# KatherLab/STAMP

Hardware: AMD Instinct MI355X
Metric: tiles/sec encoded (224x224, ViT-L/14) (higher is better)
Workload: dtype f16

## Files before the change

include/amdstamp.h:

```cpp
#ifndef AMDSTAMP_H
#define AMDSTAMP_H

#include <stddef.h>
#include <stdint.h>

#ifdef __cplusplus
extern "C" {
#endif

#define AMDS_VERSION_MAJOR 0
#define AMDS_VERSION_MINOR 2

typedef enum {
    AMDS_OK = 0,
    AMDS_ERR_INVALID = -1,
    AMDS_ERR_WORKSPACE = -2,
    AMDS_ERR_HIP = -3,
    AMDS_ERR_NODEVICE = -4,
    AMDS_ERR_RANGE = -5
} amds_status;

typedef enum { AMDS_F16 = 0, AMDS_BF16 = 1, AMDS_F32 = 2 } amds_dtype;

typedef enum {
    AMDS_EPI_BIAS = 0,
    AMDS_EPI_BIAS_GELU = 1,
    AMDS_EPI_BIAS_RELU = 2,
    AMDS_EPI_RESIDUAL = 3,
    AMDS_EPI_BIAS_F32 = 4,
    AMDS_EPI_SWIGLU = 5,
    AMDS_EPI_PATCH = 6,
    AMDS_EPI_BIAS_GELU_F32 = 7,
    AMDS_EPI_BIAS_RELU_F32 = 8
} amds_epilogue;


int amds_version(void);
const char* amds_last_error(void);
int amds_device_info(int device, char* name_host, int n, int* cu_count_host, size_t* hbm_bytes_host);

typedef struct amds_ctx amds_ctx;
amds_ctx* amds_create(int device);
void amds_destroy(amds_ctx* ctx);
int amds_ctx_device(const amds_ctx* ctx);

int amds_profile_enable(amds_ctx* ctx, int on);
int amds_profile_reset(amds_ctx* ctx);
int amds_profile_read(amds_ctx* ctx, int kind, double* total_ms_host, long* launches_host, double* total_work_host);


int amds_cast_pad(const float* src, int ld_src, void* dst, int ld_dst, int rows, int cols,
                  int dtype, void* stream);

int amds_layernorm(const float* x, long x_row_stride, const float* gamma, const float* beta,
                   void* y, long y_row_stride, int rows, int cols, float eps, int out_dtype,
                   void* stream);

int amds_gemm(const void* A, long lda, const void* W, long ldw, int M, int N, int K,
              int dtype, int epi, void* out, long ldo, const float* bias, const float* scale,
              const float* pos, int np, int T, int P, float acc_scale, void* stream);

int amds_quick_gelu_inplace(void* u, long ld, long rows, int cols, int dtype, void* stream);

int amds_gemm_rowstream(const void* A, long lda, const float* ln_gamma, const float* ln_beta, float ln_eps,
                        const void* W, long ldw, int M, int N, int K, int dtype, int epi, void* out, long ldo,
                        const float* bias, void* stream);

int amds_swin_mlp96(float* x, int M, const void* fc1_w, const float* fc1_b, const void* fc2_w, const float* fc2_b,
                    const float* ln_gamma, const float* ln_beta, float ln_eps, int dtype, void* stream);

int amds_swin_mlp192_pack(const void* fc1_w, const void* fc2_w, void* packed, int dtype, void* stream);
int amds_swin_mlp192(float* x, int M, const void* packed_w, const float* fc1_b, const float* fc2_b, const float* ln_gamma,
                     const float* ln_beta, float ln_eps, int dtype, void* stream);

int amds_gemm_ex(int cfg, const void* A, long lda, const void* W, long ldw, int M, int N, int K,
                 int dtype, int epi, void* out, long ldo, const float* bias, const float* scale,
                 const float* pos, int np, int T, int P, float acc_scale, void* stream);
long amds_gemm_persist_launches(void);

int amds_gemm_fp8(const void* A8, long lda, const void* W8, long ldw, int M, int N, int K, int epi, void* out, long ldo, const float* bias,
                  const float* colscale, const float* rowscale, void* stream);
int amds_quantize_rows_e4m3(const void* x, long ldx, void* q, long ldq, float* scale, int rows, int cols, int in_dtype, void* stream);
int amds_layernorm_quant_e4m3(const float* x, long ldx, const float* gamma, const float* beta, float eps, void* q, long ldq, float* scale,
                              float* rownorm, int rows, int cols, void* stream);
int amds_row_bound_scale(const float* rownorm, float c0, float c1, float* us, int rows, void* stream);
int amds_gemm_fp8_out8(const void* A8, long lda, const void* W8, long ldw, int M, int N, int K, int epi, void* out8, long ldo8,
                       const float* out_rowscale, const float* bias, const float* colscale, const float* rowscale, void* stream);

int amds_gemm_lnfold(const void* A, long lda, const void* W, long ldw, int M, int N, int K, int dtype, int epi, void* out,
                     long ldo, const float* bias, const float* scale, void* xh, float* rowpart, const float* rowstat,
                     const float* colsum, void* stream);

int amds_gemm_lnfold_planes(const void* A, long lda, const void* W, long ldw, int M, int N, int K, void* hi, void* lo, long ld,
                            const float* bias, const float* scale, float* rowpart, void* stream);
int amds_ln_stats_split(const float* x, long ldx, int M, int D, float eps, void* hi, void* lo, long ld, float* rowstat, void* stream);
int amds_planes_to_f32(const void* hi, const void* lo, long ld, long row_stride, float* out, long ldo, long rows, int D, void* stream);

int amds_ln_rowstat(const float* rowpart, int M, int NP, int D, float eps, float* rowstat, void* stream);
int amds_ln_rowstat_diag(const float* rowpart, int M, int NP, int D, float eps, float* rowstat, int* diag, int dtype, void* stream);
int amds_ln_stats_cast(const float* x, long ldx, int M, int D, float eps, void* xh, long ldxh, float* rowstat, int dtype, void* stream);

int amds_pack_swiglu_rows(const float* src, float* dst, int H, int cols, void* stream);

int amds_attention_vit(const void* qkv, void* out, int B, int T, int H, int dtype, void* stream);

int amds_attention_vit_hd(const void* qkv, void* out, int B, int T, int H, int head_dim, int dtype, void* stream);

int amds_attention(const void* qkv, void* out, int B, int T, int H, int dtype, void* stream);
int amds_attention_row(const void* q, long ldq, const void* qkv, void* out, long ldo, int B, int T, int H, int dtype, void* stream);
int amds_attention_row_fwd_train(const void* qkv, void* out, float* lse, int B, int T, int H, int qrow, int dtype, float p, uint64_t seed,
                                 uint32_t stream_id, void* stream);
int amds_attention_row_alibi_fwd_train(const void* qkv, const float* coords, const float* inv_running_mean, const float* bias_scale, void* out, void* u, void* osm,
                                       float* lse, int B, int T, int H, int qrow, int dtype, void* stream);
int amds_attention_row_alibi_bwd_train(const void* qkv, const void* osm, const void* u, const void* dout, const float* lse, const float* coords, const float* bias_scale,
                                       const float* inv_running_mean, void* dqkv, float* dbs, int B, int T, int H, int qrow, int dtype, void* stream);
int amds_attention_row_bwd_train(const void* qkv, const void* out, const void* dout, const float* lse, void* dqkv, int B, int T, int H, int qrow,
                                 int dtype, float p, uint64_t seed, uint32_t stream_id, void* stream);
int amds_set_mil_cls_tail(amds_ctx* ctx, int on);
int amds_get_mil_cls_tail(amds_ctx* ctx);

int amds_attention_alibi(const void* qkv, const float* coords, const float* head_scale, void* out, int B, int T, int H,
                         int dtype, void* stream);

int amds_attention_masked(const void* qkv, const uint8_t* pad, void* out, int B, int T, int H, int mask_heads, int dtype, void* stream);
int amds_attention_alibi_masked(const void* qkv, const float* coords, const float* head_scale, const uint8_t* pad, void* out,
                                int B, int T, int H, int dtype, void* stream);


typedef struct {
    int img;
    int patch;
    int dim;
    int depth;
    int heads;
    int hidden;
    int n_prefix;
    int mlp_kind;
    int layerscale;
    int dtype;
    float ln_eps;
} amds_vit_cfg;

typedef struct {
    const float* ln1_w; const float* ln1_b;
    const void*  qkv_w; const float* qkv_b;
    const void*  proj_w; const float* proj_b;
    const float* ls1;
    const float* ln2_w; const float* ln2_b;
    const void*  fc1_w; const float* fc1_b;
    const void*  fc2_w; const float* fc2_b;
    const float* ls2;
    const float* qkv_colsum;
    const float* fc1_colsum;
} amds_vit_block;

typedef struct {
    const float* q_w;    const float* q_b;
    const float* proj_w; const float* proj_b;
    const float* fc1_w;  const float* fc1_b;
    const float* fc2_w;  const float* fc2_b;
} amds_vit_exact_block;

typedef struct {
    const void* qkv_w8;  const float* qkv_cs;
    const void* proj_w8; const float* proj_cs; const float* proj_b;
    const void* fc1_w8;  const float* fc1_cs;
    float fc1_wnorm_max; float fc1_babs_max;
    const void* fc2_w8;  const float* fc2_cs;  const float* fc2_b;
} amds_vit_fp8_block;

typedef struct {
    const void*  patch_w;
    const float* patch_b;
    const float* prefix;
    const float* pos_patch;
    const amds_vit_block* blocks_host;
    const float* norm_w; const float* norm_b;
    int patch_lo_shift;
    const amds_vit_exact_block* exact_host;
    int exact_hidden;
    const amds_vit_fp8_block* fp8_host;
    const float* pre_norm_w;
    const float* pre_norm_b;
    const amds_vit_exact_block* cls_tail;
} amds_vit_weights;

typedef struct {
    const float* norm1_w; const float* norm1_b;
    const float* qkv_w;   const float* qkv_b;
    const float* proj_w;  const float* proj_b;
    const float* ls1;
    const float* norm2_w; const float* norm2_b;
    const float* fc1_w;   const float* fc1_b;
    const float* fc2_w;   const float* fc2_b;
    const float* ls2;
} amds_vit_host_block;
typedef struct {
    const float* patch_w;
    const float* patch_b;
    const float* cls_token;
    const float* reg_token;
    const float* pos_embed;
    const amds_vit_host_block* blocks;
    const float* norm_w; const float* norm_b;
    int hidden;
    int no_embed_class;
    double mean[3]; double std[3];
} amds_vit_host_weights;
#define AMDS_PACK_LNFOLD      1
#define AMDS_PACK_PATCH_SPLIT 2
#define AMDS_PACK_EXACT       4
#define AMDS_PACK_CLS_TAIL    8
size_t amds_vit_pack_bytes(const amds_vit_cfg* cfg_host, const amds_vit_host_weights* src_host, int flags);
int amds_vit_pack(const amds_vit_cfg* cfg_host, const amds_vit_host_weights* src_host, int flags, void* dev_image, size_t bytes,
                  amds_vit_weights* out_w_host, amds_vit_block* out_blocks_host, amds_vit_exact_block* out_exact_host, void* stream);
int amds_vit_pack_host(const amds_vit_cfg* cfg_host, const amds_vit_host_weights* src_host, int flags, void* image_host, size_t bytes,
                       const void* target_base, amds_vit_weights* out_w_host, amds_vit_block* out_blocks_host,
                       amds_vit_exact_block* out_exact_host);

size_t amds_vit_workspace_bytes(const amds_vit_cfg* cfg_host, int batch);

size_t amds_vit_workspace_diag_offset(const amds_vit_cfg* cfg_host, int batch);

int amds_vit_forward(const amds_vit_cfg* cfg_host, const amds_vit_weights* w_host,
                     const uint8_t* tiles, void* feats_f16, int B, int chunk,
                     void* ws, size_t ws_bytes, void* stream);

int amds_check_finite(const void* x, long n, int dtype, int* count_dev, int* count_host, void* stream);

int amds_vit_forward_tokens(const amds_vit_cfg* cfg_host, const amds_vit_weights* w_host,
                            const uint8_t* tiles, void* feats_f16, float* tokens_f32, int B, int chunk,
                            void* ws, size_t ws_bytes, void* stream);

int amds_vit_forward_overlapped(amds_ctx* ctx, const amds_vit_cfg* cfg_host, const amds_vit_weights* w_host, const uint8_t* tiles,
                                void* feats_f16, int B, int chunk, void* ws, size_t ws_bytes, void* stream);

int amds_attention_cls_f32(const float* q, long ldq, const void* qkv, float* out, long ldo, int B, int T, int H, int head_dim,
                           int dtype, void* stream);
int amds_vit_cls_gather(const float* x, float* xc, int B, int T, int D, void* stream);
int amds_vit_cls_scatter(const float* xc, float* x, void* xh, float* rowstat, int B, int T, int D, float eps, int dtype, void* stream);
int amds_mlp_act_f32(float* u, long ld, int rows, int hidden, int kind, void* stream);

int amds_tile_im2col_u8(const uint8_t* tiles, void* out, int B, int img, int patch, int kp,
                        int dtype, void* stream);
int amds_tile_im2col_u8_ex(const uint8_t* tiles, void* out, int B, int img, int patch, int kp,
                           int dtype, int lo_shift, void* stream);

int amds_tile_normalize_u8(const uint8_t* hwc, float* chw, int B, int H, int W,
                           const float mean_host[3], const float std_host[3], void* stream);

int amds_tile_edge_fraction_u8(const uint8_t* tiles, float* frac, uint8_t* edges, uint8_t* gray, int B, int S, int low, int high,
                               void* stream);

typedef struct {
    int img;
    int embed;
    int n_stages;
    int depths[4];
    int heads[4];
    int dtype;
    float ln_eps;
} amds_swin_cfg;

typedef struct {
    const float* ln1_w; const float* ln1_b;
    const void*  qkv_w; const float* qkv_b;
    const float* bias_lane;
    const void*  proj_w; const float* proj_b;
    const float* ln2_w; const float* ln2_b;
    const void*  fc1_w; const float* fc1_b;
    const void*  fc2_w; const float* fc2_b;
    const void*  mlp_pack;
} amds_swin_block;

typedef struct {
    const float* ln_w; const float* ln_b;
    const void*  red_w;
} amds_swin_merge;

typedef struct {
    const float* stem;
    const amds_swin_block* blocks_host;
    int n_blocks;
    amds_swin_merge merges[3];
    const float* norm_w; const float* norm_b;
    const uint64_t* mask_bits;
} amds_swin_weights;

size_t amds_swin_workspace_bytes(const amds_swin_cfg* cfg_host, int batch);

int amds_swin_forward(const amds_swin_cfg* cfg_host, const amds_swin_weights* w_host, const uint8_t* tiles,
                      void* feats_f16, float* feats_f32, int B, int chunk, void* ws, size_t ws_bytes, void* stream);

int amds_swin_stem(const uint8_t* tiles, float* x, const float* params, int B, int img, int embed, float eps, void* stream);

int amds_window_attention(const void* qkv, long ldq, void* out, long ldo, const float* bias_lane, const uint64_t* mask_bits,
                          int B, int grid, int dim, int heads, int shift, int dtype, void* stream);

int amds_swin_attn96(float* x, const void* qkv_w, const float* qkv_b, const void* proj_w, const float* proj_b,
                     const float* ln_gamma, const float* ln_beta, const float* bias_lane, const uint64_t* mask_bits, int B,
                     int grid, int shift, float ln_eps, int dtype, void* stream);

int amds_patch_merge_ln(const float* x, void* y, const float* gamma, const float* beta, int B, int grid, int dim, float eps,
                        int dtype, void* stream);

int amds_layernorm_meanpool(const float* x, void* out_f16, float* out_f32, const float* gamma, const float* beta, int B,
                            int L, int dim, float eps, void* stream);

int amds_macenko_normalize_u8(const uint8_t* tiles, uint8_t* out, float* fit_out, int B, int H, int W, float Io, float alpha, float beta, void* stream);

size_t amds_supertiles_to_tiles_workspace_bytes(int n, int S, int k, int t);
int amds_supertiles_to_tiles_u8(const uint8_t* rgba, uint8_t* tiles, int n, int S, int k, int t, const int* bounds, const int* coef,
                                int ksize, void* ws, size_t ws_bytes, void* stream);

size_t amds_tile_resize_crop_workspace_bytes(int n, int S, int t);
int amds_tile_resize_crop_u8(const uint8_t* tiles, uint8_t* out, int n, int S, int O, int t, const int* bounds, const int* coef, int ksize, void* ws,
                             size_t ws_bytes, void* stream);

int amds_compact_rows_u8(const uint8_t* src, long row_bytes, const float* score, float cutoff, uint8_t* dst, int capacity_rows,
                         int* count_dev, int* slot_out, int n, void* stream);
int amds_compact_shift_u8(const uint8_t* src, uint8_t* dst, long row_bytes, int m, int max_rows, int* count_dev, void* stream);
// ... 495 lines not shown
```

stamp_amd/_lib.py:

```python
from __future__ import annotations

import ctypes as C
import os
from pathlib import Path

LIB_PATH = Path(__file__).resolve().parent / "lib" / "libamdstamp.so"

F16, BF16, F32 = 0, 1, 2
ERR_RANGE = -5
(EPI_BIAS, EPI_BIAS_GELU, EPI_BIAS_RELU, EPI_RESIDUAL, EPI_BIAS_F32, EPI_SWIGLU, EPI_PATCH,
 EPI_BIAS_GELU_F32, EPI_BIAS_RELU_F32) = range(9)


class VitCfg(C.Structure):
    _fields_ = [("img", C.c_int), ("patch", C.c_int), ("dim", C.c_int), ("depth", C.c_int),
                ("heads", C.c_int), ("hidden", C.c_int), ("n_prefix", C.c_int), ("mlp_kind", C.c_int),
                ("layerscale", C.c_int), ("dtype", C.c_int), ("ln_eps", C.c_float)]


class VitBlock(C.Structure):
    _fields_ = [(n, C.c_void_p) for n in (
        "ln1_w", "ln1_b", "qkv_w", "qkv_b", "proj_w", "proj_b", "ls1",
        "ln2_w", "ln2_b", "fc1_w", "fc1_b", "fc2_w", "fc2_b", "ls2", "qkv_colsum", "fc1_colsum")]

# ... 127 lines not shown
class BarspoonGrads(C.Structure):
    _fields_ = [("proj_w", C.c_void_p), ("proj_b", C.c_void_p), ("enc_layers_host", C.POINTER(MilVitLayerGrads)), ("class_tokens", C.c_void_p),
                ("dec_layers_host", C.POINTER(BarspoonDecLayerGrads)), ("head_w_host", C.POINTER(C.c_void_p)), ("head_b_host", C.POINTER(C.c_void_p))]


class TiconBlock(C.Structure):
    _fields_ = [(n, C.c_void_p) for n in ("ln1_w", "ln1_b", "v_w", "v_b", "proj_w", "proj_b", "ln2_w", "ln2_b", "fc1_w", "fc1_b", "fc2_w", "fc2_b")]


class TiconWeights(C.Structure):
    _fields_ = [("in_dim", C.c_int), ("dim", C.c_int), ("hidden", C.c_int), ("depth", C.c_int)] + \
               [(n, C.c_void_p) for n in ("in_fc1_w", "in_fc1_b", "in_fc2_w", "in_fc2_b", "in_norm_w", "in_norm_b")] + \
               [("blocks_host", C.POINTER(TiconBlock)), ("norm_w", C.c_void_p), ("norm_b", C.c_void_p)]


class SwinCfg(C.Structure):
    _fields_ = [("img", C.c_int), ("embed", C.c_int), ("n_stages", C.c_int), ("depths", C.c_int * 4),
                ("heads", C.c_int * 4), ("dtype", C.c_int), ("ln_eps", C.c_float)]


class SwinBlock(C.Structure):
    _fields_ = [(n, C.c_void_p) for n in (
        "ln1_w", "ln1_b", "qkv_w", "qkv_b", "bias_lane", "proj_w", "proj_b",
        "ln2_w", "ln2_b", "fc1_w", "fc1_b", "fc2_w", "fc2_b", "mlp_pack")]


class SwinMerge(C.Structure):
    _fields_ = [(n, C.c_void_p) for n in ("ln_w", "ln_b", "red_w")]


class SwinWeights(C.Structure):
    _fields_ = [("stem", C.c_void_p), ("blocks_host", C.POINTER(SwinBlock)), ("n_blocks", C.c_int),
                ("merges", SwinMerge * 3), ("norm_w", C.c_void_p), ("norm_b", C.c_void_p), ("mask_bits", C.c_void_p)]


class GapWeights(C.Structure):
    _fields_ = [(n, C.c_void_p) for n in ("fc_w", "fc_b", "a_w", "a_b", "b_w", "b_b", "c_w", "c_b", "packed")]


_vp, _i, _l, _f, _sz = C.c_void_p, C.c_int, C.c_long, C.c_float, C.c_size_t
_u64, _u32 = C.c_uint64, C.c_uint32

class TiconSlideCfg(C.Structure):
    _fields_ = [(n, C.c_int) for n in ("in_dim", "dim", "heads", "hidden", "depth", "dtype")]


class TiconSlideBlock(C.Structure):
    _fields_ = [(n, C.c_void_p) for n in ("ln1_w", "ln1_b", "in_w", "in_b", "proj_w", "proj_b", "g1", "ln2_w", "ln2_b", "fc1_w", "fc1_b", "fc2_w", "fc2_b", "g2")]


class TiconSlideWeights(C.Structure):
    _fields_ = [(n, C.c_void_p) for n in ("in_fc1_w", "in_fc1_b", "in_fc2_w", "in_fc2_b", "in_norm_w", "in_norm_b", "slopes")] + \
               [("blocks_host", C.POINTER(TiconSlideBlock)), ("norm_w", C.c_void_p), ("norm_b", C.c_void_p)]


PROTOTYPES = {
    "amds_version": (_i, []),
    "amds_last_error": (C.c_char_p, []),
    "amds_device_info": (_i, [_i, C.c_char_p, _i, C.POINTER(_i), C.POINTER(_sz)]),
    "amds_create": (_vp, [_i]),
    "amds_destroy": (None, [_vp]),
    "amds_ctx_device": (_i, [_vp]),
    "amds_profile_enable": (_i, [_vp, _i]),
    "amds_profile_reset": (_i, [_vp]),
    "amds_profile_read": (_i, [_vp, _i, C.POINTER(C.c_double), C.POINTER(C.c_long), C.POINTER(C.c_double)]),
    "amds_cast_pad": (_i, [_vp, _i, _vp, _i, _i, _i, _i, _vp]),
    "amds_layernorm": (_i, [_vp, _l, _vp, _vp, _vp, _l, _i, _i, _f, _i, _vp]),
    "amds_gemm": (_i, [_vp, _l, _vp, _l, _i, _i, _i, _i, _i, _vp, _l, _vp, _vp, _vp, _i, _i, _i, _f, _vp]),
    "amds_gemm_ex": (_i, [_i, _vp, _l, _vp, _l, _i, _i, _i, _i, _i, _vp, _l, _vp, _vp, _vp, _i, _i, _i, _f, _vp]),
    "amds_gemm_persist_launches": (_l, []),
    "amds_gemm_fp8": (_i, [_vp, _l, _vp, _l, _i, _i, _i, _i, _vp, _l, _vp, _vp, _vp, _vp]),
    "amds_layernorm_quant_e4m3": (_i, [_vp, _l, _vp, _vp, _f, _vp, _l, _vp, _vp, _i, _i, _vp]),
    "amds_row_bound_scale": (_i, [_vp, _f, _f, _vp, _i, _vp]),
    "amds_gemm_fp8_out8": (_i, [_vp, _l, _vp, _l, _i, _i, _i, _i, _vp, _l, _vp, _vp, _vp, _vp, _vp]),
    "amds_quantize_rows_e4m3": (_i, [_vp, _l, _vp, _l, _vp, _i, _i, _i, _vp]),
    "amds_gemm_lnfold": (_i, [_vp, _l, _vp, _l, _i, _i, _i, _i, _i, _vp, _l, _vp, _vp, _vp, _vp, _vp, _vp, _vp]),
    "amds_ln_rowstat": (_i, [_vp, _i, _i, _i, _f, _vp, _vp]),
    "amds_ln_rowstat_diag": (_i, [_vp, _i, _i, _i, _f, _vp, _vp, _i, _vp]),
    "amds_vit_workspace_diag_offset": (_sz, [_vp, _i]),
    "amds_check_finite": (_i, [_vp, _l, _i, _vp, _vp, _vp]),
    "amds_export_words": (_i, [_vp, _vp, _l, _i, _vp]),
    "amds_ln_stats_cast": (_i, [_vp, _l, _i, _i, _f, _vp, _l, _vp, _i, _vp]),
    "amds_gemm_lnfold_planes": (_i, [_vp, _l, _vp, _l, _i, _i, _i, _vp, _vp, _l, _vp, _vp, _vp, _vp]),
    "amds_ln_stats_split": (_i, [_vp, _l, _i, _i, _f, _vp, _vp, _l, _vp, _vp]),
    "amds_planes_to_f32": (_i, [_vp, _vp, _l, _l, _vp, _l, _l, _i, _vp]),
    "amds_gemm_rowstream": (_i, [_vp, _l, _vp, _vp, _f, _vp, _l, _i, _i, _i, _i, _i, _vp, _l, _vp, _vp]),
    "amds_swin_mlp96": (_i, [_vp, _i, _vp, _vp, _vp, _vp, _vp, _vp, _f, _i, _vp]),
    "amds_swin_mlp192_pack": (_i, [_vp, _vp, _vp, _i, _vp]),
    "amds_swin_mlp192": (_i, [_vp, _i, _vp, _vp, _vp, _vp, _vp, _f, _i, _vp]),
    "amds_pack_swiglu_rows": (_i, [_vp, _vp, _i, _i, _vp]),
    "amds_attention_vit": (_i, [_vp, _vp, _i, _i, _i, _i, _vp]),
    "amds_attention_row": (_i, [_vp, _l, _vp, _vp, _l, _i, _i, _i, _i, _vp]),
    "amds_attention_row_fwd_train": (_i, [_vp, _vp, _vp, _i, _i, _i, _i, _i, _f, C.c_uint64, C.c_uint32, _vp]),
    "amds_attention_row_bwd_train": (_i, [_vp, _vp, _vp, _vp, _vp, _i, _i, _i, _i, _i, _f, C.c_uint64, C.c_uint32, _vp]),
    "amds_set_mil_cls_tail": (_i, [_vp, _i]),
    "amds_get_mil_cls_tail": (_i, [_vp]),
    "amds_attention": (_i, [_vp, _vp, _i, _i, _i, _i, _vp]),
    "amds_attention_vit_hd": (_i, [_vp, _vp, _i, _i, _i, _i, _i, _vp]),
    "amds_attention_alibi": (_i, [_vp, _vp, _vp, _vp, _i, _i, _i, _i, _vp]),
    "amds_vit_workspace_bytes": (_sz, [C.POINTER(VitCfg), _i]),
    "amds_vit_forward": (_i, [C.POINTER(VitCfg), C.POINTER(VitWeights), _vp, _vp, _i, _i, _vp, _sz, _vp]),
    "amds_vit_forward_overlapped": (_i, [_vp, C.POINTER(VitCfg), C.POINTER(VitWeights), _vp, _vp, _i, _i, _vp, _sz, _vp]),
    "amds_vit_forward_tokens": (_i, [C.POINTER(VitCfg), C.POINTER(VitWeights), _vp, _vp, _vp, _i, _i, _vp, _sz, _vp]),
    "amds_swin_workspace_bytes": (_sz, [C.POINTER(SwinCfg), _i]),
    "amds_swin_forward": (_i, [C.POINTER(SwinCfg), C.POINTER(SwinWeights), _vp, _vp, _vp, _i, _i, _vp, _sz, _vp]),
    "amds_swin_stem": (_i, [_vp, _vp, _vp, _i, _i, _i, _f, _vp]),
    "amds_window_attention": (_i, [_vp, _l, _vp, _l, _vp, _vp, _i, _i, _i, _i, _i, _i, _vp]),
    "amds_swin_attn96": (_i, [_vp, _vp, _vp, _vp, _vp, _vp, _vp, _vp, _vp, _i, _i, _i, _f, _i, _vp]),
    "amds_patch_merge_ln": (_i, [_vp, _vp, _vp, _vp, _i, _i, _i, _f, _i, _vp]),
    "amds_layernorm_meanpool": (_i, [_vp, _vp, _vp, _vp, _vp, _i, _i, _i, _f, _vp]),
    "amds_tile_edge_fraction_u8": (_i, [_vp, _vp, _vp, _vp, _i, _i, _i, _i, _vp]),
    "amds_tile_im2col_u8": (_i, [_vp, _vp, _i, _i, _i, _i, _i, _vp]),
    "amds_tile_im2col_u8_ex": (_i, [_vp, _vp, _i, _i, _i, _i, _i, _i, _vp]),
    "amds_vit_pack_bytes": (_sz, [_vp, _vp, _i]),
    "amds_vit_pack": (_i, [_vp, _vp, _i, _vp, _sz, _vp, _vp, _vp, _vp]),
    "amds_vit_pack_host": (_i, [_vp, _vp, _i, _vp, _sz, _vp, _vp, _vp, _vp]),
    "amds_compact_shift_u8": (_i, [_vp, _vp, _l, _i, _i, _vp, _vp]),
    "amds_compact_rows_u8": (_i, [_vp, _l, _vp, _f, _vp, _i, _vp, _vp, _i, _vp]),
    "amds_attention_cls_f32": (_i, [_vp, _l, _vp, _vp, _l, _i, _i, _i, _i, _i, _vp]),
    "amds_vit_cls_gather": (_i, [_vp, _vp, _i, _i, _i, _vp]),
    "amds_vit_cls_scatter": (_i, [_vp, _vp, _vp, _vp, _i, _i, _i, _f, _i, _vp]),
    "amds_mlp_act_f32": (_i, [_vp, _l, _i, _i, _i, _vp]),
    "amds_tile_normalize_u8": (_i, [_vp, _vp, _i, _i, _i, C.POINTER(_f), C.POINTER(_f), _vp]),
    "amds_macenko_normalize_u8": (_i, [_vp, _vp, _vp, _i, _i, _i, _f, _f, _f, _vp]),
    "amds_supertiles_to_tiles_workspace_bytes": (_sz, [_i, _i, _i, _i]),
    "amds_supertiles_to_tiles_u8": (_i, [_vp, _vp, _i, _i, _i, _i, _vp, _vp, _i, _vp, _sz, _vp]),
    "amds_gather_rows": (_i, [_vp, _l, _vp, _i, _vp, _l, _i, _i, _i, _i, _vp]),
    "amds_vary_precision": (_i, [_vp, _vp, _vp, _l, _i, _vp]),
    "amds_bag_batch_gather": (_i, [_vp, _l, _i, _vp, _vp, _vp, _l, _i, _vp, _i, _i, _i, _i, _u64, _u32, _vp]),
    "amds_bag_batch_shifts": (_i, [_vp, _i, _i, _i, _i, _u64, _u32, _vp]),
    "amds_mean_pool": (_i, [_vp, _vp, _i, _i, _i, _i, _vp]),
    "amds_linear_f32": (_i, [_vp, _vp, _vp, _vp, _i, _i, _i, _i, _vp]),
    "amds_mil_vit_workspace_bytes": (_sz, [_vp, _i, _i]),
    "amds_mil_vit_forward": (_i, [_vp, _vp, _vp, _i, _vp, _vp, _vp, _i, _i, _vp, _sz, _vp]),
    "amds_mil_vit_ragged_workspace_bytes": (_sz, [_vp, _i, _l, _i]),
    "amds_mil_vit_forward_ragged": (_i, [_vp, _vp, _vp, _i, _vp, _vp, _vp, _i, _l, _i, _vp, _sz, _vp]),
    "amds_mil_vit_ragged_max_shared_tiles": (_i, [_vp]),
    "amds_attention_varlen_workspace_bytes": (_sz, [_i, _l]),
    "amds_attention_varlen": (_i, [_vp, _vp, _vp, _i, _l, _i, _i, _i, _vp, _sz, _vp]),
    "amds_attention_varlen_rows": (_i, [_vp, _vp, _vp, _i, _l, _i, _i, _i, _vp, _sz, _vp]),
    "amds_attention_alibi_varlen": (_i, [_vp, _vp, _vp, _vp, _vp, _i, _l, _i, _i, _i, _vp, _sz, _vp]),
    "amds_attention_row_varlen": (_i, [_vp, _l, _vp, _vp, _vp, _l, _i, _l, _i, _i, _i, _vp, _sz, _vp]),
    "amds_barspoon_workspace_bytes": (_sz, [_vp, _i, _i]),
    "amds_barspoon_forward": (_i, [_vp, _vp, _vp, _i, _vp, _vp, _i, _i, _vp, _sz, _vp]),
    "amds_barspoon_ragged_workspace_bytes": (_sz, [_vp, _i, _l, _i]),
    "amds_barspoon_forward_ragged": (_i, [_vp, _vp, _vp, _i, _vp, _vp, _vp, _i, _l, _i, _vp, _sz, _vp]),
    "amds_barspoon_ragged_max_shared_tiles": (_i, [_vp]),
    "amds_barspoon_train_saved_bytes": (_sz, [_vp, _i, _i]),
    "amds_barspoon_train_workspace_bytes": (_sz, [_vp, _i, _i, _i]),
    "amds_barspoon_train_forward": (_i, [_vp, _vp, _vp, _i, _vp, _vp, _vp, _i, _i, _vp, _sz, _vp]),
    "amds_barspoon_train_backward": (_i, [_vp, _vp, _vp, _vp, _i, _i, _vp, _sz, _vp, _i, _vp, _sz, _vp]),
    "amds_cross_attention_fwd_train": (_i, [_vp, _vp, _vp, _vp, _i, _i, _i, _i, _i, _i, _f, _u64, _u32, _vp]),
    "amds_cross_attention_bwd_workspace_bytes": (_sz, [_i, _i, _i, _i]),
    "amds_cross_attention_bwd_train": (_i, [_vp, _vp, _vp, _vp, _vp, _vp, _vp, _l, _i, _i, _i, _i, _i, _i, _f, _u64, _u32, _vp, _sz, _vp]),
    "amds_ticon_tile_workspace_bytes": (_sz, [_vp, _i]),
    "amds_ticon_tile_forward": (_i, [_vp, _vp, _i, _vp, _i, _i, _vp, _sz, _vp]),
    "amds_attention_distbias": (_i, [_vp, _vp, _vp, _vp, _i, _i, _i, _i, _vp]),
    "amds_ticon_slide_workspace_bytes": (_sz, [_vp, _i, _i]),
    "amds_ticon_slide_forward": (_i, [_vp, _vp, _vp, _i, _vp, _vp, _i, _i, _i, _vp, _sz, _vp]),
    "amds_tile_resize_crop_workspace_bytes": (_sz, [_i, _i, _i]),
    "amds_tile_resize_crop_u8": (_i, [_vp, _vp, _i, _i, _i, _i, _vp, _vp, _i, _vp, _sz, _vp]),
    "amds_proj_head_l2norm_workspace_bytes": (_sz, [_i, _i, _i]),
    "amds_proj_head_l2norm": (_i, [_vp, _i, _vp, _vp, _vp, _vp, _vp, _i, _i, _i, _vp, _sz, _vp]),
    "amds_quick_gelu_inplace": (_i, [_vp, _l, _l, _i, _i, _vp]),
    "amds_transmil_workspace_bytes": (_sz, [_vp, _i, _i]),
    "amds_transmil_train_saved_bytes": (_sz, [_vp, _i, _i]),
    "amds_transmil_train_workspace_bytes": (_sz, [_vp, _i, _i]),
    "amds_transmil_train_forward": (_i, [_vp, _vp, _vp, _i, _f, C.c_uint64, _vp, _i, _i, _vp, _sz, _vp]),
    "amds_transmil_train_backward": (_i, [_vp, _vp, _vp, _f, C.c_uint64, _i, _i, _vp, _sz, _vp, _vp, _vp, _sz, _vp]),
    "amds_nystrom_attn_saved_bytes": (_sz, [_i, _i, _i]),
    "amds_nystrom_attn_workspace_bytes": (_sz, [_i, _i, _i]),
    "amds_nystrom_attn_fwd": (_i, [_vp, _i, _vp, _vp, _i, _i, _f, C.c_uint64, C.c_uint32, _vp, _sz, _vp]),
    "amds_nystrom_attn_bwd": (_i, [_vp, _i, _vp, _vp, _vp, _i, _i, _f, C.c_uint64, C.c_uint32, _vp, _sz, _vp, _sz, _vp]),
    "amds_transmil_forward": (_i, [_vp, _vp, _vp, _i, _vp, _i, _i, _vp, _sz, _vp]),
    "amds_transmil_ragged_plan": (_i, [_vp, _i, _vp, _vp]),
    "amds_transmil_ragged_workspace_bytes": (_sz, [_vp, _i, _vp]),
    "amds_transmil_forward_ragged": (_i, [_vp, _vp, _vp, _i, _vp, _vp, _vp, _i, _vp, _sz, _vp]),
    "amds_mil_vit_train_saved_bytes": (_sz, [_vp, _i, _i]),
    "amds_mil_vit_train_workspace_bytes": (_sz, [_vp, _i, _i, _i]),
    "amds_mil_vit_train_forward": (_i, [_vp, _vp, _vp, _i, _vp, _vp, _vp, _i, _i, _vp, _sz, _vp]),
    "amds_mil_vit_train_backward": (_i, [_vp, _vp, _vp, _vp, _i, _i, _vp, _sz, _vp, _vp, _i, _vp, _sz, _vp]),
    "amds_mil_vit_gradcam_workspace_bytes": (_sz, [_vp, _i, _i]),
    "amds_mil_vit_gradcam": (_i, [_vp, _vp, _vp, _i, _i, _vp, _sz, _f, _vp, _vp, _sz, _vp]),
    "amds_softmax_over_tiles": (_i, [_vp, _vp, _i, _l, _vp]),
    "amds_scatter_grid": (_i, [_vp, _vp, _vp, _vp, _l, _i, _i, _i, _vp]),
    "amds_concordance_workspace_bytes": (_sz, [_l, _i]),
    "amds_concordance_counts": (_i, [_vp, _l, _l, _vp, _l, _vp, _l, _vp, _l, _l, _i, _vp, _vp, _sz, _vp]),
    "amds_bgemm_f32": (_i, [_vp, _i, _l, _l, _vp, _i, _l, _l, _i, _vp, _i, _l, _l, _i, _i, _i, _i, _i, _f, _f, _vp, _i, _vp]),
    "amds_bgemm_f32_dual": (_i, [_vp, _i, _l, _l, _vp, _i, _l, _l, _i, _vp, _vp, _i, _l, _l, _i, _i, _i, _i, _i, _f, _f, _f, _f, _vp]),
    "amds_softmax_rows": (_i, [_vp, _l, _i, _vp]),
    "amds_landmark_mean": (_i, [_vp, _l, _l, _i, _vp, _i, _i, _i, _i, _i, _f, _vp]),
    "amds_pinv_init": (_i, [_vp, _vp, _i, _i, _vp, _vp]),
    "amds_pinv_init_grouped": (_i, [_vp, _vp, _i, _i, _i, _vp, _vp]),
    "amds_dwconv_seq_row": (_i, [_vp, _l, _l, _i, _vp, _vp, _l, _l, _i, _i, _i, _i, _i, _i, _vp]),
    "amds_dwconv_seq": (_i, [_vp, _l, _l, _i, _vp, _vp, _l, _l, _i, _i, _i, _i, _i, _i, _vp]),
    "amds_ppeg": (_i, [_vp, _vp, _vp, _vp, _vp, _vp, _vp, _vp, _i, _i, _i, _i, _vp]),
    "amds_softmax_rows_bwd": (_i, [_vp, _vp, _l, _i, _vp]),
    "amds_landmark_mean_bwd": (_i, [_vp, _vp, _l, _l, _i, _i, _i, _i, _i, _i, _f, _i, _vp]),
    "amds_dwconv_seq_wgrad_workspace_bytes": (_sz, [_i, _i, _i]),
    "amds_dwconv_seq_wgrad": (_i, [_vp, _l, _l, _i, _vp, _l, _l, _i, _vp, _i, _i, _i, _i, _i, _vp, _sz, _vp]),
    "amds_ppeg_wgrad_workspace_bytes": (_sz, [_i, _i]),
    "amds_ppeg_wgrad": (_i, [_vp, _vp, _vp, _i, _i, _i, _i, _vp, _sz, _vp]),
# ... 119 lines not shown
```

stamp_amd/csrc/api.hip:

```cpp
#include "gemm_kernel.h"
#include <stdlib.h>
#include <atomic>
#include <mutex>

namespace amds {

static thread_local char g_err[512] = "";

void set_error(const char* fmt, ...) {
    va_list ap;
    va_start(ap, fmt);
    vsnprintf(g_err, sizeof(g_err), fmt, ap);
    va_end(ap);
}

int hip_fail(hipError_t e, const char* what) {
    set_error("HIP error %d (%s) in %s", (int)e, hipGetErrorString(e), what);
    return AMDS_ERR_HIP;
}

}
struct amds_ctx {
    int device = -1;
    int refs = 0;
// ... 289 lines not shown
        const char* e = getenv("AMDS_GEMM_CFG");
        bcfg = (e && *e && atoi(e) == 8) ? 8 : 12;
    }
    if (dtype == AMDS_F16) return gemm_dispatch<f16>(bcfg, epi, A, lda, W, ldw, M, N, K, ep, st);
    if (dtype == AMDS_BF16) return gemm_dispatch<bf16>(bcfg, epi, A, lda, W, ldw, M, N, K, ep, st);
    set_error("amds_gemm_batched: bad dtype %d", dtype);
    return AMDS_ERR_INVALID;
}

extern "C" int amds_wgrad_tn(const void* dy, long ld_dy, const void* x, long ld_x, long tokens, int N, int K, int split_k, int dtype, float* part,
                             void* stream) {
    AMDS_REQUIRE(dy && x && part, "amds_wgrad_tn: null pointer");
    AMDS_REQUIRE(tokens > 0 && N > 0 && K > 0 && split_k > 0 && split_k <= 65535, "amds_wgrad_tn: bad shape");
    AMDS_REQUIRE(N % 256 == 0 && K % 256 == 0, "amds_wgrad_tn: needs N %% 256 == 0 and K %% 256 == 0 (N=%d K=%d)", N, K);
    AMDS_REQUIRE(ld_dy % 8 == 0 && ld_x % 8 == 0 && ld_dy >= N && ld_x >= K, "amds_wgrad_tn: bad pitches");
    AMDS_REQUIRE(((uintptr_t)dy & 15) == 0 && ((uintptr_t)x & 15) == 0 && ((uintptr_t)part & 15) == 0, "amds_wgrad_tn: pointers must be 16-byte aligned");
    const long unit = 64L * split_k;
    const long chunk = (tokens + unit - 1) / unit * 64;
    AMDS_REQUIRE((chunk + 63) * std::max(ld_dy, ld_x) * 2 < (1L << 31), "amds_wgrad_tn: one split's operand span is beyond the 2 GB a buffer descriptor addresses (raise split_k)");
    EpiArgs ep;
    ep.out = part; ep.ldo = K; ep.bias = nullptr; ep.scale = nullptr; ep.pos = nullptr; ep.np = ep.T = ep.P = 0; ep.acc_scale = 1.0f;
    ep.bsA = chunk * ld_dy; ep.bsW = chunk * ld_x; ep.bsOut = (long)N * K; ep.nbatch = split_k; ep.ktot = tokens;
    hipStream_t st = (hipStream_t)stream;
    ProfScope prof(PROF_GEMM, 2.0 * tokens * (double)N * K, st);
    if (dtype == AMDS_F16) return gemm_dispatch<f16>(15, AMDS_EPI_BIAS_F32, dy, ld_dy, x, ld_x, N, K, (int)chunk, ep, st);
    if (dtype == AMDS_BF16) return gemm_dispatch<bf16>(15, AMDS_EPI_BIAS_F32, dy, ld_dy, x, ld_x, N, K, (int)chunk, ep, st);
    set_error("amds_wgrad_tn: bad dtype %d", dtype);
    return AMDS_ERR_INVALID;
}

extern "C" int amds_gemm_lnfold(const void* A, long lda, const void* W, long ldw, int M, int N, int K, int dtype, int epi, void* out,
                                long ldo, const float* bias, const float* scale, void* xh, float* rowpart, const float* rowstat,
                                const float* colsum, void* stream) {
    AMDS_REQUIRE(A && W && out, "amds_gemm_lnfold: null pointer");
    AMDS_REQUIRE(M >= 0 && N > 0 && K > 0 && K % 64 == 0 && N % 256 == 0, "amds_gemm_lnfold: needs K %% 64 == 0 and N %% 256 == 0 (M=%d N=%d K=%d)", M, N, K);
    AMDS_REQUIRE(lda % 8 == 0 && ldw % 8 == 0 && lda >= K && ldw >= K && ldo % 4 == 0, "amds_gemm_lnfold: bad pitches");
    AMDS_REQUIRE(((uintptr_t)A & 15) == 0 && ((uintptr_t)W & 15) == 0 && ((uintptr_t)out & 15) == 0 && ((uintptr_t)xh & 15) == 0,
                 "amds_gemm_lnfold: pointers must be 16-byte aligned");
    const bool producer = xh || rowpart, consumer = rowstat || colsum;
    AMDS_REQUIRE(producer != consumer, "amds_gemm_lnfold: either (xh, rowpart) [RESIDUAL] or (rowstat, colsum) [BIAS / BIAS_GELU / SWIGLU]");
    if (producer) {
        AMDS_REQUIRE(epi == AMDS_EPI_RESIDUAL && xh && rowpart, "amds_gemm_lnfold: the producer form is the RESIDUAL epilogue with xh AND rowpart");
    } else {
        AMDS_REQUIRE((epi == AMDS_EPI_BIAS || epi == AMDS_EPI_BIAS_GELU || epi == AMDS_EPI_SWIGLU) && rowstat && colsum && bias,
                     "amds_gemm_lnfold: the consumer form is BIAS / BIAS_GELU / SWIGLU with rowstat, colsum AND bias");
    }
    if (M == 0) return AMDS_OK;
    EpiArgs ep;
    ep.out = out; ep.ldo = ldo; ep.bias = bias; ep.scale = scale; ep.pos = nullptr; ep.np = ep.T = ep.P = 0; ep.acc_scale = 1.0f;
    ep.xh = xh; ep.rowpart = rowpart; ep.rowstat = rowstat; ep.colsum = colsum;
    hipStream_t st = (hipStream_t)stream;
    ProfScope prof(PROF_GEMM, 2.0 * M * (double)N * K, st);
    if (dtype == AMDS_F16) return gemm_dispatch<f16>(12, epi, A, lda, W, ldw, M, N, K, ep, st);
    if (dtype == AMDS_BF16) return gemm_dispatch<bf16>(12, epi, A, lda, W, ldw, M, N, K, ep, st);
    set_error("amds_gemm_lnfold: bad dtype %d", dtype);
    return AMDS_ERR_INVALID;
}

#ifdef AMDS_GEMM_TRACE
static const float* g_gemm_trace_buffer = nullptr;
extern "C" void amds_gemm_trace_buffer(void* p) { g_gemm_trace_buffer = reinterpret_cast<const float*>(p); }
#endif

extern "C" int amds_gemm_lnfold_planes(const void* A, long lda, const void* W, long ldw, int M, int N, int K, void* hi, void* lo, long ld,
                                       const float* bias, const float* scale, float* rowpart, void* stream) {
    AMDS_REQUIRE(A && W && hi && lo && rowpart, "amds_gemm_lnfold_planes: null pointer");
    AMDS_REQUIRE(M >= 0 && N > 0 && K > 0 && K % 64 == 0 && N % 256 == 0, "amds_gemm_lnfold_planes: needs K %% 64 == 0 and N %% 256 == 0 (M=%d N=%d K=%d)", M, N, K);
    AMDS_REQUIRE(lda % 8 == 0 && ldw % 8 == 0 && lda >= K && ldw >= K && ld % 4 == 0 && ld >= N, "amds_gemm_lnfold_planes: bad pitches");
    AMDS_REQUIRE(((uintptr_t)A & 15) == 0 && ((uintptr_t)W & 15) == 0 && ((uintptr_t)hi & 15) == 0 && ((uintptr_t)lo & 15) == 0,
                 "amds_gemm_lnfold_planes: pointers must be 16-byte aligned");
    AMDS_REQUIRE(hi != lo && A != hi && A != lo, "amds_gemm_lnfold_planes: the planes are updated in place and must not alias each other or A");
    if (M == 0) return AMDS_OK;
    EpiArgs ep;
    ep.out = hi; ep.ldo = ld; ep.bias = bias; ep.scale = scale; ep.pos = nullptr; ep.np = ep.T = ep.P = 0; ep.acc_scale = 1.0f;
    ep.xh = hi; ep.xl = lo; ep.rowpart = rowpart;
#ifdef AMDS_GEMM_TRACE
    ep.pos = g_gemm_trace_buffer;
#endif
    hipStream_t st = (hipStream_t)stream;
    ProfScope prof(PROF_GEMM, 2.0 * M * (double)N * K, st);
    return gemm_dispatch<f16>(12, AMDS_EPI_RESIDUAL, A, lda, W, ldw, M, N, K, ep, st);
}

extern "C" long amds_gemm_persist_launches(void) { return g_gemm_persist_launches.load(std::memory_order_relaxed); }

extern "C" int amds_gemm_ex(int cfg, const void* A, long lda, const void* W, long ldw, int M, int N, int K, int dtype,
                            int epi, void* out, long ldo, const float* bias, const float* scale, const float* pos,
                            int np, int T, int P, float acc_scale, void* stream) {
    return gemm_impl(cfg, A, lda, W, ldw, M, N, K, dtype, epi, out, ldo, bias, scale, pos, np, T, P, acc_scale, stream);
}
```

stamp_amd/csrc/elementwise.hip:

```cpp
#include "launch.h"

namespace amds {

template <typename TO, int MAXV>
__global__ void __launch_bounds__(256) layernorm_kernel(const float* __restrict__ x, long xs,
                                                        const float* __restrict__ gamma,
                                                        const float* __restrict__ beta, TO* __restrict__ y,
                                                        long ys, int rows, int cols, float eps) {
    const int lane = threadIdx.x & 63;
    const int row = blockIdx.x * 4 + (threadIdx.x >> 6);
    if (row >= rows) return;
    const float* xr = x + (long)row * xs;
    const int nv = cols >> 2;
    f32x4 v[MAXV];
    float s = 0.f;
#pragma unroll
    for (int i = 0; i < MAXV; ++i) {
        const int c = i * 64 + lane;
        if (c < nv) {
            v[i] = *reinterpret_cast<const f32x4*>(xr + c * 4);
            s += (v[i][0] + v[i][1]) + (v[i][2] + v[i][3]);
        }
    }
    const float mean = wave_sum(s) / (float)cols;
// ... 241 lines not shown

struct Norm3 { float mean[3], inv_std[3]; };
__global__ void __launch_bounds__(256) tile_normalize_kernel(const uint8_t* __restrict__ hwc, float* __restrict__ chw,
                                                             long npix_total, int hw, Norm3 nm) {
    long q = (long)blockIdx.x * blockDim.x + threadIdx.x;
    const long nq = npix_total >> 2;
    const long stride = (long)gridDim.x * blockDim.x;
    for (; q < nq; q += stride) {
        const long p = q << 2;
        const long b = p / hw;
        const int off = (int)(p - b * hw);
        const uint32_t* s = reinterpret_cast<const uint32_t*>(hwc + p * 3);
        const uint32_t w0 = s[0], w1 = s[1], w2 = s[2];
        uint8_t px[12];
#pragma unroll
        for (int k = 0; k < 4; ++k) { px[k] = (w0 >> (8 * k)) & 255; px[4 + k] = (w1 >> (8 * k)) & 255; px[8 + k] = (w2 >> (8 * k)) & 255; }
#pragma unroll
        for (int c = 0; c < 3; ++c) {
            f32x4 o;
#pragma unroll
            for (int k = 0; k < 4; ++k) o[k] = ((float)px[k * 3 + c] / 255.0f - nm.mean[c]) * nm.inv_std[c];
            *reinterpret_cast<f32x4*>(chw + (b * 3 + c) * hw + off) = o;
        }
    }
}

constexpr int IM2COL_KMAX = 4096;
template <typename TO>
__global__ void __launch_bounds__(256) im2col_u8_kernel(const uint8_t* __restrict__ tiles, TO* __restrict__ out,
                                                        int img, int p, int kp, float lo_scale) {
    extern __shared__ __attribute__((aligned(16))) uint8_t srow[];
    const int g = img / p;
    const int b = blockIdx.x / g, py = blockIdx.x - b * g;
    const int nbytes = p * img * 3;
    const uint8_t* src = tiles + ((long)b * img + (long)py * p) * img * 3;
    for (int i = threadIdx.x * 16; i < nbytes; i += 256 * 16)
        *reinterpret_cast<u32x4*>(srow + i) = *reinterpret_cast<const u32x4*>(src + i);
    __shared__ int koff[IM2COL_KMAX];
    const int pp = p * p, k_real = 3 * pp;
    for (int k = threadIdx.x; k < kp; k += 256) {
        const int c = k / pp, r = k - c * pp, i = r / p, j = r - i * p;
        koff[k] = k < k_real ? (i * img + j) * 3 + c : -1;
    }
    __syncthreads();
    const int ld = lo_scale != 0.f ? 2 * kp : kp;
    const int chunks = ld >> 3, half = kp >> 3;
    TO* orow = out + ((long)b * g * g + (long)py * g) * ld;
    typedef TO vec8 __attribute__((ext_vector_type(8)));
    for (int w = threadIdx.x; w < g * chunks; w += 256) {
        const int px = w / chunks, ch = w - px * chunks;
        const int ch0 = ch >= half ? ch - half : ch;
        const float sc = ch >= half ? lo_scale : 1.0f;
        const uint8_t* pbase = srow + px * p * 3;
        vec8 o;
#pragma unroll
        for (int e = 0; e < 8; ++e) {
            const int off = koff[ch0 * 8 + e];
            o[e] = (TO)(off >= 0 ? (float)pbase[off] * sc : 0.f);
        }
        *reinterpret_cast<vec8*>(orow + (long)px * ld + ch * 8) = o;
    }
}

__global__ void prefix_init_kernel(const float* __restrict__ prefix, float* __restrict__ x, int B, int T, int P, int dim) {
    const long total = (long)B * P * (dim >> 2);
    long i = (long)blockIdx.x * blockDim.x + threadIdx.x;
    const long stride = (long)gridDim.x * blockDim.x;
    const int dv = dim >> 2;
    for (; i < total; i += stride) {
        const long bt = i / dv;
        const int c = (int)(i - bt * dv);
        const long b = bt / P;
        const int t = (int)(bt - b * P);
        *reinterpret_cast<f32x4*>(x + ((b * T + t) * (long)dim) + c * 4) =
            *reinterpret_cast<const f32x4*>(prefix + (long)t * dim + c * 4);
    }
}

int prefix_init(const float* prefix, float* x, int B, int T, int P, int dim, hipStream_t st) {
    const long total = (long)B * P * (dim / 4);
    const int grid = (int)min((long)2048, (total + 255) / 256);
    hipLaunchKernelGGL(prefix_init_kernel, dim3(grid), dim3(256), 0, st, prefix, x, B, T, P, dim);
    AMDS_LAUNCH_CHECK("prefix_init_kernel");
    return AMDS_OK;
}

template <typename T>
__global__ void __launch_bounds__(256) quick_gelu_inplace_kernel(T* __restrict__ u, long ld, long rows, int cols) {
    typedef T vec8 __attribute__((ext_vector_type(8)));
    const int c8 = cols >> 3;
    const long total = rows * c8;
    long i = (long)blockIdx.x * blockDim.x + threadIdx.x;
    const long stride = (long)gridDim.x * blockDim.x;
    for (; i < total; i += stride) {
        const long r = i / c8;
        const int c = (int)(i - r * c8);
        vec8* p = reinterpret_cast<vec8*>(u + r * ld) + c;
        vec8 v = *p;
#pragma unroll
        for (int e = 0; e < 8; ++e) {
            const float x = (float)v[e];
            v[e] = (T)(x * __builtin_amdgcn_rcpf(1.0f + __expf(-1.702f * x)));
        }
        *p = v;
    }
}

}

using namespace amds;

extern "C" int amds_layernorm(const float* x, long x_row_stride, const float* gamma, const float* beta, void* y,
                              long y_row_stride, int rows, int cols, float eps, int out_dtype, void* stream) {
    AMDS_REQUIRE(x && gamma && beta && y, "amds_layernorm: null pointer");
    AMDS_REQUIRE(rows >= 0 && cols > 0 && cols % 4 == 0 && cols <= 8192, "amds_layernorm: cols=%d must be a multiple of 4 and <= 8192", cols);
    AMDS_REQUIRE(x_row_stride % 4 == 0 && y_row_stride % 4 == 0, "amds_layernorm: row strides must be multiples of 4");
    if (rows == 0) return AMDS_OK;
    hipStream_t st = (hipStream_t)stream;
    ProfScope prof(PROF_LN, (double)rows * cols * (4 + (out_dtype == AMDS_F32 ? 4 : 2)), st);
    int rc = AMDS_ERR_INVALID;
    if (!dispatch_16_32(out_dtype, [&](auto t) { rc = launch_ln<AMDS_TAG_T(t)>(x, x_row_stride, gamma, beta, y, y_row_stride, rows, cols, eps, st); }))
        set_error("amds_layernorm: bad out_dtype %d", out_dtype);
    return rc;
}

extern "C" int amds_cast_pad(const float* src, int ld_src, void* dst, int ld_dst, int rows, int cols, int dtype,
                             void* stream) {
    AMDS_REQUIRE(src && dst, "amds_cast_pad: null pointer");
    AMDS_REQUIRE(rows >= 0 && cols >= 0 && ld_dst >= cols && ld_src >= cols, "amds_cast_pad: bad shape");
    const long total = (long)rows * ld_dst;
    if (total == 0) return AMDS_OK;
    const int grid = (int)min((long)4096, (total + 255) / 256);
    hipStream_t st = (hipStream_t)stream;
    const bool ok = dispatch_16_32(dtype, [&](auto t) {
        typedef AMDS_TAG_T(t) T;
        hipLaunchKernelGGL((cast_pad_kernel<T>), dim3(grid), dim3(256), 0, st, src, ld_src, (T*)dst, ld_dst, total, cols);
    });
    if (!ok) { set_error("amds_cast_pad: bad dtype %d", dtype); return AMDS_ERR_INVALID; }
    AMDS_LAUNCH_CHECK("cast_pad_kernel");
    return AMDS_OK;
}

extern "C" int amds_pack_swiglu_rows(const float* src, float* dst, int H, int cols, void* stream) {
    AMDS_REQUIRE(src && dst && src != dst, "amds_pack_swiglu_rows: null/aliased pointer");
    AMDS_REQUIRE(H > 0 && H % 32 == 0 && cols > 0, "amds_pack_swiglu_rows: H=%d must be a positive multiple of 32", H);
    const long total = 2L * H * cols;
    const int grid = (int)min((long)4096, (total + 255) / 256);
    hipLaunchKernelGGL(pack_swiglu_rows_kernel, dim3(grid), dim3(256), 0, (hipStream_t)stream, src, dst, H, cols);
    AMDS_LAUNCH_CHECK("pack_swiglu_rows_kernel");
    return AMDS_OK;
}

extern "C" int amds_tile_normalize_u8(const uint8_t* hwc, float* chw, int B, int H, int W, const float mean_host[3],
                                      const float std_host[3], void* stream) {
    AMDS_REQUIRE(hwc && chw && mean_host && std_host, "amds_tile_normalize_u8: null pointer");
    AMDS_REQUIRE(B >= 0 && H > 0 && W > 0 && (H * W) % 4 == 0, "amds_tile_normalize_u8: H*W must be a multiple of 4");
    if (B == 0) return AMDS_OK;
    Norm3 nm;
    for (int c = 0; c < 3; ++c) {
        AMDS_REQUIRE(std_host[c] != 0.f, "amds_tile_normalize_u8: std[%d] == 0", c);
        nm.mean[c] = mean_host[c];
        nm.inv_std[c] = 1.0f / std_host[c];
    }
    const long npix = (long)B * H * W;
    const int grid = (int)min((long)4096, (npix / 4 + 255) / 256);
    hipLaunchKernelGGL(tile_normalize_kernel, dim3(grid), dim3(256), 0, (hipStream_t)stream, hwc, chw, npix, H * W, nm);
// ... 164 lines not shown
```

stamp_amd/csrc/gemm_4w16.h:

```cpp
#pragma once
#include <algorithm>
#include <type_traits>
#include "gemm_kernel.h"

namespace amds {

__device__ __forceinline__ f32x4 agpr_read(const f32x4& a) {
    f32x4 v;
    asm("v_accvgpr_read_b32 %0, %1" : "=v"(v[0]) : "a"(a[0]));
    asm("v_accvgpr_read_b32 %0, %1" : "=v"(v[1]) : "a"(a[1]));
    asm("v_accvgpr_read_b32 %0, %1" : "=v"(v[2]) : "a"(a[2]));
    asm("v_accvgpr_read_b32 %0, %1" : "=v"(v[3]) : "a"(a[3]));
    return v;
}

template <int N> struct NextTilePieces : std::integral_constant<int, N> {};
template <typename C> struct is_next_tile : std::false_type {};
template <int N> struct is_next_tile<NextTilePieces<N>> : std::true_type {};

template <typename T, int EPI, int P3 = 6, int P0 = 6, bool SPREAD = true, int PRL = 0, int PRS = 0, bool STREAM = false, bool PERSIST = false, bool TN = false>
__global__ void __launch_bounds__(256) __attribute__((amdgpu_waves_per_eu(1, 1)))
gemm_4w16_kernel(const T* __restrict__ A, long lda, const T* __restrict__ W, long ldw, int M, int N, int K,
                 EpiArgs ep, int tiles_m, int tiles_n) {
    typedef typename Act<T>::vec8 vec8;
    typedef typename Act<T>::vec4 vec4;
    constexpr int BM = 256, BN = 256, BK = 64, NT = 256;
    constexpr int ROWB = BK * 2;
    constexpr int A_BYTES = BM * ROWB, STAGE = (BM + BN) * ROWB;
    constexpr int FI = 8, FJ = 8;
    constexpr int GROUP_M = 8;

    extern __shared__ __attribute__((aligned(16))) char smem[];
#ifdef AMDS_GEMM_TRACE
    unsigned long long tr_t[4] = {0, 0, 0, 0}, tr_rt0 = __builtin_amdgcn_s_memrealtime();
    int tr_round = 0;
#define AMDS_GEMM_STAMP(k)                             \
    do {                                               \
        __builtin_amdgcn_sched_barrier(0);             \
        tr_t[k] = __builtin_amdgcn_s_memtime();        \
        __builtin_amdgcn_sched_barrier(0);             \
    } while (0)
#define AMDS_GEMM_TRACE_WRITE()                                                                                                            \
    do {                                                                                                                                   \
        if (ep.pos != nullptr && threadIdx.x == 0) {                                                                                       \
            unsigned long long* rec = reinterpret_cast<unsigned long long*>(const_cast<float*>(ep.pos)) +                                  \
                                      ((long)blockIdx.x * ((ntiles + (int)gridDim.x - 1) / (int)gridDim.x) + tr_round) * 8;                \
            rec[0] = tr_t[0]; rec[1] = tr_t[1]; rec[2] = tr_t[2]; rec[3] = tr_t[3];                                                        \
            rec[4] = (unsigned long long)__builtin_amdgcn_s_getreg(63492) | ((unsigned long long)__builtin_amdgcn_s_getreg(63508) << 32);  \
            rec[5] = (unsigned long long)ti;                                                                                               \
            rec[6] = tr_rt0; rec[7] = __builtin_amdgcn_s_memrealtime();                                                                    \
        }                                                                                                                                  \
        ++tr_round;                                                                                                                        \
    } while (0)
    AMDS_GEMM_STAMP(0);
#else
#define AMDS_GEMM_STAMP(k) do { } while (0)
#define AMDS_GEMM_TRACE_WRITE() do { } while (0)
#endif

    const int tid = threadIdx.x;
    const int lane = tid & 63;
    const int wave = __builtin_amdgcn_readfirstlane(tid >> 6);
    const int wm = wave >> 1, wn = wave & 1;
    const int l15 = lane & 15, kb = lane >> 4;
    const int l31 = lane & 31, hi = lane >> 5;

    static_assert(!PERSIST || (STREAM && !TN && P3 >= 0 && PRL + PRS == 0 &&
                               (EPI == AMDS_EPI_BIAS || EPI == AMDS_EPI_BIAS_GELU || EPI == AMDS_EPI_BIAS_RELU || EPI == AMDS_EPI_RESIDUAL)),
                  "gemm_4w16: the persistent form is a streamed epilogue on SCHED 0");
    int tm, tn;
    auto tile_of = [&](int bid, int nwg, int& tm_, int& tn_) {
        const int xcd = bid & 7, q = nwg >> 3, r = nwg & 7;
        const int t = (xcd < r ? xcd * (q + 1) : r * (q + 1) + (xcd - r) * q) + (bid >> 3);
        const int group = GROUP_M * tiles_n;
        const int g = t / group, first_m = g * GROUP_M;
        const int gm = min(tiles_m - first_m, GROUP_M);
        const int rr = t - g * group;
        tm_ = first_m + rr % gm;
        tn_ = rr / gm;
    };
    const int ntiles = PERSIST ? tiles_m * tiles_n : (int)gridDim.x;
    int ti = blockIdx.x;
    tile_of(ti, ntiles, tm, tn);
    int m0 = tm * BM, n0 = tn * BN;
    int par = 0;
    if (ep.nbatch > 1) {
        const long by = blockIdx.y;
        A += by * ep.bsA;
        W += by * ep.bsW;
        constexpr bool F32O = (EPI == AMDS_EPI_RESIDUAL || EPI == AMDS_EPI_BIAS_F32 || EPI == AMDS_EPI_BIAS_GELU_F32 || EPI == AMDS_EPI_BIAS_RELU_F32);
        if (F32O) ep.out = reinterpret_cast<float*>(ep.out) + by * ep.bsOut;
        else ep.out = reinterpret_cast<T*>(ep.out) + by * ep.bsOut;
    }

    int rows_a = min(BM, M - m0);
    const long tn_valid = TN ? (ep.ktot > 0 ? min((long)K, ep.ktot - (long)blockIdx.y * K) : (long)K) : 0;
    __amdgpu_buffer_rsrc_t rsrc_a = TN ? __builtin_amdgcn_make_buffer_rsrc(const_cast<T*>(A + m0), 0, tn_valid > 0 ? (int)(((tn_valid - 1) * lda + BM) * 2) : 0, 0x00020000)
                                             : __builtin_amdgcn_make_buffer_rsrc(const_cast<T*>(A + (long)m0 * lda), 0, (int)((((long)rows_a - 1) * lda + K) * 2), 0x00020000);
    __amdgpu_buffer_rsrc_t rsrc_w = TN ? __builtin_amdgcn_make_buffer_rsrc(const_cast<T*>(W + n0), 0, tn_valid > 0 ? (int)(((tn_valid - 1) * ldw + BN) * 2) : 0, 0x00020000)
                                             : __builtin_amdgcn_make_buffer_rsrc(const_cast<T*>(W + (long)n0 * ldw), 0, (int)(((long)(BN - 1) * ldw + K) * 2), 0x00020000);
    int voff[16];
#pragma unroll
    for (int it = 0; it < 16; ++it) {
        if constexpr (TN) {
            const int c = (it & 7) * NT + tid, row = c >> 5, pos = c & 31, g = (row & 3) | ((row >> 1) & 4);
            voff[it] = (int)(((long)row * (it < 8 ? lda : ldw) + (pos ^ (g << 1)) * 8) * 2);
        } else {
            const int c = (it & 7) * NT + tid, row = c >> 3, cp = c & 7, sc = cp ^ ((row >> 1) & 7);
            voff[it] = (int)(((long)row * (it < 8 ? lda : ldw) + sc * 8) * 2);
        }
    }
    auto issue_to = [&](const __amdgpu_buffer_rsrc_t& ra, const __amdgpu_buffer_rsrc_t& rw, char* st, int koff, int koff_w, int lo, int hi_) {
#pragma unroll
        for (int it = 0; it < 16; ++it)
            if (it >= lo && it < hi_) {
                if (it < 8) {
                    __builtin_amdgcn_raw_ptr_buffer_load_lds(ra, (lptr_t)(st + ((it & 7) * NT + wave * 64) * 16), 16, voff[it], koff, 0, 0);
                } else {
                    __builtin_amdgcn_raw_ptr_buffer_load_lds(rw, (lptr_t)(st + A_BYTES + ((it & 7) * NT + wave * 64) * 16), 16, voff[it], koff_w,
                                                             0, 0);
                }
            }
    };
    auto issue_pieces = [&](int kt, int lo, int hi_) {
        char* st = smem + ((PERSIST ? kt + par : kt) & 1) * STAGE;
        const int koff = TN ? kt * BK * (int)lda * 2 : kt * BK * 2;
        const int koff_w = TN ? kt * BK * (int)ldw * 2 : koff;
        issue_to(rsrc_a, rsrc_w, st, koff, koff_w, lo, hi_);
    };
    int m0n = m0, n0n = n0;
    bool has_next = false;
    __amdgpu_buffer_rsrc_t rsrc_an = rsrc_a, rsrc_wn = rsrc_w;
    auto issue_next = [&](int lo, int hi_) { issue_to(rsrc_an, rsrc_wn, smem + ((K / BK + par) & 1) * STAGE, 0, 0, lo, hi_); };

    const int swz = (l15 >> 1) & 7;
    const int a_off = (wm * 128 + l15) * ROWB;
    const int w_off = A_BYTES + (wn * 128 + l15) * ROWB;

    const bool lnf = ep.rowstat != nullptr;
    const bool bias_in_acc = ep.bias != nullptr && ep.acc_scale == 1.0f && !lnf;
    f32x4 acc[FI][FJ];
    {
        f32x4 b0[FJ];
#pragma unroll
        for (int j = 0; j < FJ; ++j) b0[j] = f32x4{0.f, 0.f, 0.f, 0.f};
        if (bias_in_acc) {
#pragma unroll
            for (int j = 0; j < FJ; ++j) b0[j] = *reinterpret_cast<const f32x4*>(ep.bias + n0 + wn * 128 + j * 16 + 4 * kb);
        }
        __builtin_amdgcn_sched_barrier(0);
        issue_pieces(0, 0, 16);
        if constexpr (P3 < 0) {
            if (K / BK > 1) issue_pieces(1, 0, 16);
        }
        __builtin_amdgcn_sched_barrier(0);
#pragma unroll
        for (int i = 0; i < FI; ++i)
#pragma unroll
            for (int j = 0; j < FJ; ++j) acc[i][j] = b0[j];
    }
#pragma unroll
    for (int i = 0; i < FI; ++i) {
        if (i == FI - 1)
            asm volatile("s_nop 7" : "+a"(acc[i][0]), "+a"(acc[i][1]), "+a"(acc[i][2]), "+a"(acc[i][3]), "+a"(acc[i][4]), "+a"(acc[i][5]),
                         "+a"(acc[i][6]), "+a"(acc[i][7]));
        else
            asm volatile("" : "+a"(acc[i][0]), "+a"(acc[i][1]), "+a"(acc[i][2]), "+a"(acc[i][3]), "+a"(acc[i][4]), "+a"(acc[i][5]),
                         "+a"(acc[i][6]), "+a"(acc[i][7]));
    }
    __builtin_amdgcn_sched_barrier(0);

    vec8 af[2][FI], wf[2][FJ];
    const int tn_g = (l15 >> 2) | ((kb & 1) << 2);
    const int tn_row = (kb * 8 + (l15 >> 2)) * 512 + (l15 & 1) * 8 + ((l15 >> 1) & 1) * 16;
    auto load_frags = [&](int kt, int ks, int s, int lo, int hi_) {
        const char* sb = smem + ((PERSIST ? kt + par : kt) & 1) * STAGE;
        if constexpr (TN) {
            const unsigned base = (unsigned)(size_t)(sb + tn_row + ks * 32 * 512);
#pragma unroll
            for (int q = 0; q < 16; ++q)
                if (q >= lo && q < hi_) {
                    const int qq = q & 7;
                    const unsigned pq = base + (q < 8 ? 0 : A_BYTES) + ((q < 8 ? wm : wn) * 16 + 2 * (qq ^ tn_g)) * 16;
                    u32x2 a0, a1;
                    asm volatile("ds_read_b64_tr_b16 %0, %1" : "=v"(a0) : "v"(pq) : "memory");
                    asm volatile("ds_read_b64_tr_b16 %0, %1 offset:2048" : "=v"(a1) : "v"(pq) : "memory");
                    const vec8 f = __builtin_bit_cast(vec8, u32x4{a0[0], a0[1], a1[0], a1[1]});
                    if (q < 8) af[s][qq] = f; else wf[s][qq] = f;
                }
        } else {
            const int co = ((ks * 4 + kb) ^ swz) << 4;
#pragma unroll
            for (int q = 0; q < 16; ++q)
                if (q >= lo && q < hi_) {
                    if (q < 8) af[s][q] = *reinterpret_cast<const vec8*>(sb + a_off + q * 16 * ROWB + co);
                    else wf[s][q - 8] = *reinterpret_cast<const vec8*>(sb + w_off + (q - 8) * 16 * ROWB + co);
                }
        }
    };
    auto unit = [&](int s, int ih, auto nr_c, int rkt, int rks, int rs, int rlo, auto nc_c, int ckt, int clo) {
        constexpr int NR = decltype(nr_c)::value, NC = decltype(nc_c)::value;
        constexpr bool NXT = is_next_tile<decltype(nc_c)>::value;
        constexpr int R_SPAN = SPREAD ? (NR >= 16 ? 16 : 32) : (NR > 0 ? NR : 1), C_LO = SPREAD ? (NR >= 16 ? 16 : 0) : NR,
                      C_SPAN = SPREAD ? 32 - C_LO : (NC > 0 ? NC : 1);
#pragma unroll
        for (int m = 0; m < 32; ++m) {
            Act<T>::mfma16_agpr(wf[s][m & 7], af[s][ih * 4 + (m >> 3)], acc[ih * 4 + (m >> 3)][m & 7]);
            if (NR > 0 && m < R_SPAN) {
                const int r0 = m * NR / R_SPAN, r1 = (m + 1) * NR / R_SPAN;
                if (r1 > r0) load_frags(rkt, rks, rs, rlo + r0, rlo + r1);
            }
            if (NC > 0 && m >= C_LO && m < C_LO + C_SPAN) {
                const int c0 = (m - C_LO) * NC / C_SPAN, c1 = (m - C_LO + 1) * NC / C_SPAN;
                if (c1 > c0) {
                    if constexpr (NXT) issue_next(clo + c0, clo + c1); else issue_pieces(ckt, clo + c0, clo + c1);
                }
            }
            __builtin_amdgcn_sched_barrier(0);
        }
    };
    typedef std::integral_constant<int, 0> I0;
    typedef std::integral_constant<int, 8> I8;
    typedef std::integral_constant<int, 16> I16;
// ... 119 lines not shown
                AMDS_BARRIER();
                unit(1, 1, I16{}, kt + 1, 0, 0, 0, I0{}, 0, 0);
            } else {
                unit(1, 0, I0{}, 0, 0, 0, 0, I0{}, 0, 0);
                unit(1, 1, I0{}, 0, 0, 0, 0, I0{}, 0, 0);
            }
        }
    };
    auto k_tile_last_prefetch = [&](int kt) {
        unit(0, 0, I8{}, kt, 1, 1, 0, NextTilePieces<8>{}, 0, 0);
        unit(0, 1, I8{}, kt, 1, 1, 8, NextTilePieces<8>{}, 0, 8);
        unit(1, 0, I0{}, 0, 0, 0, 0, I0{}, 0, 0);
        asm volatile("s_waitcnt lgkmcnt(0)" ::: "memory");
        __builtin_amdgcn_sched_barrier(0);
        __builtin_amdgcn_s_waitcnt(0x0F70);
        AMDS_BARRIER();
    };
next_tile:
    int kt = 0;
    for (; kt < nk - 2; ++kt) k_tile(kt, std::true_type{}, std::true_type{});
    if (nk >= 2) k_tile(kt++, std::true_type{}, std::false_type{});
    if constexpr (PERSIST) {
        has_next = ti + (int)gridDim.x < ntiles;
        int tmn, tnn;
        tile_of(has_next ? ti + (int)gridDim.x : ti, ntiles, tmn, tnn);
        m0n = tmn * BM;
        n0n = tnn * BN;
        const int rows_an = min(BM, M - m0n);
        rsrc_an = __builtin_amdgcn_make_buffer_rsrc(const_cast<T*>(A + (long)m0n * lda), 0, has_next ? (int)((((long)rows_an - 1) * lda + K) * 2) : 0, 0x00020000);
        rsrc_wn = __builtin_amdgcn_make_buffer_rsrc(const_cast<T*>(W + (long)n0n * ldw), 0, has_next ? (int)(((long)(BN - 1) * ldw + K) * 2) : 0, 0x00020000);
    }
    constexpr bool LNC = (EPI == AMDS_EPI_BIAS || EPI == AMDS_EPI_BIAS_GELU || EPI == AMDS_EPI_SWIGLU);
    f32x2 rs[LNC ? FI : 1];
    f32x4 cb[LNC ? FJ : 1], cs[LNC ? FJ : 1];
    auto load_lnc = [&]() {
        if constexpr (LNC) {
            if (lnf) {
#pragma unroll
                for (int i = 0; i < FI; ++i)
                    rs[i] = *reinterpret_cast<const f32x2*>(ep.rowstat + 2 * (long)min(m0 + wm * 128 + i * 16 + l15, M - 1));
#pragma unroll
                for (int j = 0; j < FJ; ++j) {
                    cb[j] = *reinterpret_cast<const f32x4*>(ep.bias + n0 + wn * 128 + j * 16 + 4 * kb);
                    cs[j] = *reinterpret_cast<const f32x4*>(ep.colsum + n0 + wn * 128 + j * 16 + 4 * kb);
                }
            }
        }
    };
    if constexpr (PERSIST) {
        k_tile_last_prefetch(kt);
        if constexpr (LNC) {
#pragma unroll
            for (int i = 0; i < FI; ++i) asm volatile("" : "=v"(rs[i]));
#pragma unroll
            for (int j = 0; j < FJ; ++j) asm volatile("" : "=v"(cb[j]), "=v"(cs[j]));
        }
        load_lnc();
        __builtin_amdgcn_sched_barrier(0);
        unit(1, 1, I0{}, 0, 0, 0, 0, I0{}, 0, 0);
    } else {
        load_lnc();
        k_tile(kt, std::false_type{}, std::false_type{});
    }
    AMDS_GEMM_STAMP(2);
    if constexpr (PRN > 0) {
        asm volatile("s_waitcnt vmcnt(0)" ::: "memory");
#pragma unroll
        for (int q = 0; q < (PRL > 0 ? PRL : 1); ++q) asm volatile("" ::"v"(pd[q]));
    }
    if constexpr (!PERSIST) AMDS_BARRIER();

#pragma unroll
    for (int i = 0; i < FI; ++i) {
        if (i == 0)
            asm volatile("s_nop 15\n\ts_nop 15" : "+a"(acc[i][0]), "+a"(acc[i][1]), "+a"(acc[i][2]), "+a"(acc[i][3]), "+a"(acc[i][4]),
                         "+a"(acc[i][5]), "+a"(acc[i][6]), "+a"(acc[i][7]));
        else
            asm volatile("" : "+a"(acc[i][0]), "+a"(acc[i][1]), "+a"(acc[i][2]), "+a"(acc[i][3]), "+a"(acc[i][4]), "+a"(acc[i][5]),
                         "+a"(acc[i][6]), "+a"(acc[i][7]));
    }
    __builtin_amdgcn_sched_barrier(0);

    constexpr bool F16OUT = (EPI == AMDS_EPI_BIAS || EPI == AMDS_EPI_BIAS_GELU || EPI == AMDS_EPI_BIAS_RELU);
    static_assert(epi_is_staged<EPI>() || EPI == AMDS_EPI_SWIGLU, "gemm_4w16: staged epilogues and SWIGLU");
    if constexpr (EPI == AMDS_EPI_SWIGLU) {
        const float as = ep.acc_scale;
#pragma unroll
        for (int i = 0; i < FI; ++i) {
            const int row = wm * 128 + i * 16 + l15;
#pragma unroll
            for (int q = 0; q < 2; ++q)
#pragma unroll
                for (int t = 0; t < 2; ++t) {
                    f32x4 gt = agpr_read(acc[i][4 * q + t]), vl = agpr_read(acc[i][4 * q + 2 + t]);
                    if (lnf) {
                        gt = gt * rs[i][0] + (cs[4 * q + t] * rs[i][1] + cb[4 * q + t]);
                        vl = vl * rs[i][0] + (cs[4 * q + 2 + t] * rs[i][1] + cb[4 * q + 2 + t]);
                    } else if (!bias_in_acc) {
                        const f32x4 bg = *reinterpret_cast<const f32x4*>(ep.bias + n0 + wn * 128 + (4 * q + t) * 16 + 4 * kb);
                        const f32x4 bv = *reinterpret_cast<const f32x4*>(ep.bias + n0 + wn * 128 + (4 * q + 2 + t) * 16 + 4 * kb);
                        gt = gt * as + bg;
                        vl = vl * as + bv;
                    }
                    f32x4 o;
                    {
                        const f32x2 o01 = silu_mul2(f32x2{gt[0], gt[1]}, f32x2{vl[0], vl[1]}), o23 = silu_mul2(f32x2{gt[2], gt[3]}, f32x2{vl[2], vl[3]});
                        o = f32x4{o01[0], o01[1], o23[0], o23[1]};
                    }
                    const int hcol = wn * 64 + q * 32 + t * 16 + 4 * kb;
                    const int chunk = hcol >> 3, half = ((hcol >> 2) & 1) * 8;
                    *reinterpret_cast<vec4*>(smem + row * 256 + ((chunk ^ (row & 15)) << 4) + half) = Act<T>::from_f32x4(o);
                }
        }
        __syncthreads();
        const int l15r = lane & 15, rsub = lane >> 4;
#pragma unroll 4
        for (int it = 0; it < 16; ++it) {
            const int row = wave * 64 + it * 4 + rsub;
            const u32x4 v = *reinterpret_cast<const u32x4*>(smem + row * 256 + l15r * 16);
            const int chunk = l15r ^ (row & 15);
            if (m0 + row < M)
                *reinterpret_cast<u32x4*>(reinterpret_cast<T*>(ep.out) + (long)(m0 + row) * ep.ldo + n0 / 2 + chunk * 8) = v;
        }
        return;
    }
    if constexpr (EPI == AMDS_EPI_RESIDUAL && STREAM) {
        static_assert(std::is_same<T, f16>::value && !TN && PRL + PRS == 0, "gemm_4w16: the streamed residual epilogue is the fp16 planes producer");
        __builtin_amdgcn_sched_barrier(0);
        __builtin_amdgcn_s_waitcnt(0x0F70);
        __builtin_amdgcn_sched_barrier(0);
        const int rows_o = min(BM, M - m0);
        int ldo2 = (int)ep.ldo * 2;
        if constexpr (PERSIST) asm volatile("" : "+s"(ldo2));
        const __amdgpu_buffer_rsrc_t rsrc_h = __builtin_amdgcn_make_buffer_rsrc(reinterpret_cast<T*>(ep.xh) + (long)m0 * ep.ldo + n0, 0,
                                                                                (int)((((long)rows_o - 1) * ep.ldo + BN) * 2), 0x00020000);
        const __amdgpu_buffer_rsrc_t rsrc_l = __builtin_amdgcn_make_buffer_rsrc(reinterpret_cast<T*>(ep.xl) + (long)m0 * ep.ldo + n0, 0,
                                                                                (int)((((long)rows_o - 1) * ep.ldo + BN) * 2), 0x00020000);
        char* slab = smem + (PERSIST ? ((nk - 1 + par) & 1) * STAGE : 0) + wave * 16384;
        float* part = reinterpret_cast<float*>(smem + 2 * STAGE);
        int wr_base = l15 * 512;
        int rd_base = hi * 512 + l31 * 16;
        if constexpr (PERSIST) asm volatile("" : "+v"(wr_base), "+v"(rd_base));
        int offp[8];
#pragma unroll
        for (int u = 0; u < 8; ++u) offp[u] = (wm * 128 + 2 * u + hi) * ldo2 + wn * 256 + ((l31 ^ (2 * u + hi)) << 3);
        const int np_part = N / 128;
        auto run = [&](auto has_scale_c) {
            constexpr bool HS = decltype(has_scale_c)::value;
            f32x4 sc[HS ? FJ : 1];
            if constexpr (HS) {
#pragma unroll
                for (int j = 0; j < FJ; ++j) sc[j] = *reinterpret_cast<const f32x4*>(ep.scale + n0 + wn * 128 + j * 16 + 4 * kb);
            }
            f32x4 b0n[PERSIST ? FJ : 1];
            u32x4 prev[3][8];
            auto load_prev = [&](int s) {
                int rowoff = s * 16 * ldo2;
                asm volatile("" : "+s"(rowoff));
#pragma unroll
                for (int u = 0; u < 8; ++u) {
                    const u32x2 ph = __builtin_bit_cast(u32x2, __builtin_amdgcn_raw_buffer_load_b64(rsrc_h, offp[u] + rowoff, 0, 0));
                    const u32x2 pl = __builtin_bit_cast(u32x2, __builtin_amdgcn_raw_buffer_load_b64(rsrc_l, offp[u] + rowoff, 0, 0));
                    prev[s % 3][u] = u32x4{ph[0], ph[1], pl[0], pl[1]};
                }
            };
            load_prev(0);
            load_prev(1);
            f32x4 v[8];
#pragma unroll
            for (int s = 0; s <= FI; ++s) {
                if (s < FI) {
                    char* wp = slab + (s & 1) * 8192 + wr_base;
#pragma unroll
                    for (int j = 0; j < FJ; ++j) {
                        f32x4 a = agpr_read(acc[s][j]);
                        if constexpr (HS) a *= sc[j];
                        *reinterpret_cast<f32x4*>(wp + (((j * 4 + kb) ^ l15) << 4)) = a;
                    }
                    if (s >= 1 && s + 1 < FI) load_prev(s + 1);
                    if constexpr (PERSIST) {
                        if (s == FI - 1) {
#pragma unroll
                            for (int j = 0; j < FJ; ++j) b0n[j] = f32x4{0.f, 0.f, 0.f, 0.f};
                            if (bias_in_acc) {
#pragma unroll
                                for (int j = 0; j < FJ; ++j) b0n[j] = *reinterpret_cast<const f32x4*>(ep.bias + n0n + wn * 128 + j * 16 + 4 * kb);
                            }
                        }
                    }
                }
                __builtin_amdgcn_sched_barrier(0);
                if (s > 0) {
                    const int t = s - 1;
                    int rowoff = t * 16 * ldo2;
                    asm volatile("" : "+s"(rowoff));
                    f32x2 ss[8];
#pragma unroll
                    for (int u = 0; u < 8; ++u) {
                        const u32x4 o = prev[t % 3][u];
                        const f32x4 old4 = f32x4{mix_add_hh<0, 0>(o[0], o[2]), mix_add_hh<1, 1>(o[0], o[2]), mix_add_hh<0, 0>(o[1], o[3]), mix_add_hh<1, 1>(o[1], o[3])};
                        v[u] += old4;
                        const vec4 c = Act<T>::from_f32x4(v[u]);
                        __builtin_amdgcn_raw_buffer_store_b64(__builtin_bit_cast(u32x2, c), rsrc_h, offp[u] + rowoff, 0, 0);
                        const u32x2 cu = __builtin_bit_cast(u32x2, c);
                        const f32x4 rest = f32x4{mix_sub_fh<0>(v[u][0], cu[0]), mix_sub_fh<1>(v[u][1], cu[0]), mix_sub_fh<0>(v[u][2], cu[1]), mix_sub_fh<1>(v[u][3], cu[1])};
                        const vec4 cl = Act<T>::from_f32x4(rest);
                        __builtin_amdgcn_raw_buffer_store_b64(__builtin_bit_cast(u32x2, cl), rsrc_l, offp[u] + rowoff, 0, 0);
                        ss[u] = f32x2{(v[u][0] + v[u][1]) + (v[u][2] + v[u][3]),
                                      fmaf(v[u][0], v[u][0], v[u][1] * v[u][1]) + fmaf(v[u][2], v[u][2], v[u][3] * v[u][3])};
                    }
                    const f32x2 tot = row16_sum8(ss, lane);
                    const int urow = ((lane >> 3) & 1) * 4 + ((lane >> 2) & 1) * 2 + (lane & 1);
                    const int prow = wm * 128 + t * 16 + 2 * urow + hi;
                    if ((lane & 2) == 0) *reinterpret_cast<f32x2*>(part + ((prow * 2 + ((lane >> 4) & 1)) * 2 + wn) * 2) = tot;
                }
                if (s < FI) {
                    __builtin_amdgcn_fence(__ATOMIC_ACQ_REL, "wavefront");
                    __builtin_amdgcn_wave_barrier();
                    const char* rp = slab + (s & 1) * 8192 + rd_base;
#pragma unroll
                    for (int u = 0; u < 8; ++u) v[u] = *reinterpret_cast<const f32x4*>(rp + u * 1024);
                    __builtin_amdgcn_wave_barrier();
                }
                __builtin_amdgcn_sched_barrier(0);
            }
            if constexpr (PERSIST) {
#pragma unroll
                for (int i = 0; i < FI; ++i)
#pragma unroll
                    for (int j = 0; j < FJ; ++j) acc[i][j] = b0n[PERSIST ? j : 0];
            }
        };
        if (ep.scale) run(std::true_type{}); else run(std::false_type{});
        if constexpr (PERSIST) {
#pragma unroll
            for (int i = 0; i < FI; ++i) {
                if (i == FI - 1)
                    asm volatile("s_nop 7" : "+a"(acc[i][0]), "+a"(acc[i][1]), "+a"(acc[i][2]), "+a"(acc[i][3]), "+a"(acc[i][4]), "+a"(acc[i][5]),
                                 "+a"(acc[i][6]), "+a"(acc[i][7]));
                else
                    asm volatile("" : "+a"(acc[i][0]), "+a"(acc[i][1]), "+a"(acc[i][2]), "+a"(acc[i][3]), "+a"(acc[i][4]), "+a"(acc[i][5]),
                                 "+a"(acc[i][6]), "+a"(acc[i][7]));
            }
        }
        asm volatile("s_waitcnt lgkmcnt(0)" ::: "memory");
        __builtin_amdgcn_sched_barrier(0);
        __builtin_amdgcn_s_barrier();
        __builtin_amdgcn_sched_barrier(0);
#pragma unroll
        for (int e = 0; e < 2; ++e) {
            const int idx = e * NT + tid, row = idx >> 1;
            const f32x4 p4 = *reinterpret_cast<const f32x4*>(part + idx * 4);
            if (m0 + row < M)
                *reinterpret_cast<f32x2*>(ep.rowpart + ((long)(m0 + row) * np_part + tn * 2 + (idx & 1)) * 2) = f32x2{p4[0] + p4[2], p4[1] + p4[3]};
        }
        if constexpr (PERSIST) {
            AMDS_GEMM_STAMP(3);
            AMDS_GEMM_TRACE_WRITE();
            if (!has_next) return;
            ti += (int)gridDim.x;
            tn = n0n / BN;
            m0 = m0n;
            n0 = n0n;
            rsrc_a = rsrc_an;
            rsrc_w = rsrc_wn;
            par = (par + nk) & 1;
            AMDS_GEMM_STAMP(0);
            AMDS_GEMM_STAMP(1);
            load_frags(0, 0, 0, 0, 16);
            if (nk > 1) issue_pieces(1, 0, Q3);
            __builtin_amdgcn_sched_barrier(0);
            goto next_tile;
        }
#ifdef AMDS_GEMM_TRACE
        asm volatile("s_waitcnt vmcnt(0)" ::: "memory");
#endif
        AMDS_GEMM_STAMP(3);
        AMDS_GEMM_TRACE_WRITE();
        return;
    }
    if constexpr (EPI == AMDS_EPI_RESIDUAL) {
        if (rmw_fast) {
            const int rows_o = min(BM, M - m0);
            rsrc_o = __builtin_amdgcn_make_buffer_rsrc(reinterpret_cast<float*>(ep.out) + (long)m0 * ep.ldo + n0, 0,
                                                       (int)((((long)rows_o - 1) * ep.ldo + BN) * 4), 0x00020000);
#pragma unroll
            for (int h = 0; h < 2; ++h)
#pragma unroll
                for (int u = 0; u < 8; ++u)
                    offu[h][u] = (wave * 64 + 2 * u + hi) * ldo4 + (((l31 >> 4) ^ h) << 9) + (((l31 & 15) ^ (2 * u + hi)) << 4);
            const __amdgpu_buffer_rsrc_t rsrc_h = __builtin_amdgcn_make_buffer_rsrc(
                ep.xh ? reinterpret_cast<T*>(ep.xh) + (long)m0 * ep.ldo + n0 : reinterpret_cast<T*>(ep.out), 0,
                ep.xh ? (int)((((long)rows_o - 1) * ep.ldo + BN) * 2) : 0, 0x00020000);
            const __amdgpu_buffer_rsrc_t rsrc_l = __builtin_amdgcn_make_buffer_rsrc(
                ep.xl ? reinterpret_cast<T*>(ep.xl) + (long)m0 * ep.ldo + n0 : reinterpret_cast<T*>(ep.out), 0,
                ep.xl ? (int)((((long)rows_o - 1) * ep.ldo + BN) * 2) : 0, 0x00020000);
            const int np_part = N / 128;
            auto run = [&](auto has_scale_c, auto lnp_c, auto pl_c) {
                constexpr bool HS = decltype(has_scale_c)::value, LNP = decltype(lnp_c)::value, PL = decltype(pl_c)::value;
                auto load_prev = [&](int pass, int b8) {
                    if constexpr (PL) {
                        int rowoff = b8 * 16 * ldo4 + pass * 256;
                        asm volatile("" : "+s"(rowoff));
#pragma unroll
                        for (int u = 0; u < 8; ++u) {
                            const int o = (offu[b8 & 1][u] + rowoff) >> 1;
                            const u32x2 ph = __builtin_bit_cast(u32x2, __builtin_amdgcn_raw_buffer_load_b64(rsrc_h, o, 0, 0));
                            const u32x2 pl = __builtin_bit_cast(u32x2, __builtin_amdgcn_raw_buffer_load_b64(rsrc_l, o, 0, 0));
                            old[b8][u] = __builtin_bit_cast(f32x4, u32x4{ph[0], ph[1], pl[0], pl[1]});
                        }
                    } else {
                        load_old(pass, b8);
                    }
                };
                f32x4 sc[4];
                auto load_scale = [&](int pass) {
                    if constexpr (HS) {
#pragma unroll
                        for (int jj = 0; jj < 4; ++jj)
                            sc[jj] = *reinterpret_cast<const f32x4*>(ep.scale + n0 + wn * 128 + (pass * 4 + jj) * 16 + 4 * kb);
                    }
                };
                load_scale(0);
#pragma unroll
                for (int b8 = 0; b8 < 4; ++b8) load_prev(0, b8);
#pragma unroll
                for (int pass = 0; pass < 2; ++pass) {
#pragma unroll
                    for (int i = 0; i < FI; ++i) {
                        const int row = wm * 128 + i * 16 + l15;
#pragma unroll
                        for (int jj = 0; jj < 4; ++jj) {
                            f32x4 v = agpr_read(acc[i][pass * 4 + jj]);
                            if constexpr (HS) v *= sc[jj];
                            const int chunk = wn * 16 + jj * 4 + kb;
                            *reinterpret_cast<f32x4*>(smem + row * 512 + ((chunk ^ (row & 31)) << 4)) = v;
                        }
                        __builtin_amdgcn_sched_barrier(0);
                    }
                    asm volatile("s_waitcnt lgkmcnt(0)" ::: "memory");
                    __builtin_amdgcn_sched_barrier(0);
                    __builtin_amdgcn_s_barrier();
                    __builtin_amdgcn_sched_barrier(0);
                    if (pass == 0) load_scale(1);
#pragma unroll
                    for (int b8 = 0; b8 < 4; ++b8) {
                        f32x4 v[8];
#pragma unroll
                        for (int u = 0; u < 8; ++u) {
                            const int row = wave * 64 + (b8 * 8 + u) * 2 + hi;
                            v[u] = *reinterpret_cast<const f32x4*>(smem + row * 512 + l31 * 16);
                        }
                        int rowoff = b8 * 16 * ldo4 + pass * 256;
                        asm volatile("" : "+s"(rowoff));
#pragma unroll
                        for (int u = 0; u < 8; ++u) {
                            if constexpr (PL) {
                                const u32x4 o = __builtin_bit_cast(u32x4, old[b8][u]);
                                const vec4 h4 = __builtin_bit_cast(vec4, u32x2{o[0], o[1]}), l4 = __builtin_bit_cast(vec4, u32x2{o[2], o[3]});
                                f32x4 old4;
                                if constexpr (std::is_same<T, f16>::value) {
                                    old4 = f32x4{mix_add_hh<0, 0>(o[0], o[2]), mix_add_hh<1, 1>(o[0], o[2]), mix_add_hh<0, 0>(o[1], o[3]), mix_add_hh<1, 1>(o[1], o[3])};
                                } else {
// ... 196 lines not shown
#pragma unroll
                for (int jj = 0; jj < JP; jj += 2) {
                    const int j = pass * JP + jj;
                    f32x4 v0 = agpr_read(acc[i][j]), v1 = agpr_read(acc[i][j + 1]);
                    epi_value_pair<EPI, FAST, true>(epv, cols.bias[jj], cols.scale[jj], cols.bias[jj + 1], cols.scale[jj + 1], v0, v1);
                    if constexpr (F16OUT) {
                        const vec4 o0 = Act<T>::from_f32x4(v0), o1 = Act<T>::from_f32x4(v1);
                        const int chunk = wn * 16 + j * 2 + (kb >> 1);
                        const int half = ((kb & 1) ^ ((l15 >> 3) & 1)) * 8;
                        *reinterpret_cast<vec4*>(smem + row * 512 + ((chunk ^ (row & 31)) << 4) + half) = o0;
                        *reinterpret_cast<vec4*>(smem + row * 512 + (((chunk + 2) ^ (row & 31)) << 4) + half) = o1;
                    } else {
                        const int chunk = wn * 16 + jj * 4 + kb;
                        *reinterpret_cast<f32x4*>(smem + row * 512 + ((chunk ^ (row & 31)) << 4)) = v0;
                        *reinterpret_cast<f32x4*>(smem + row * 512 + (((chunk + 4) ^ (row & 31)) << 4)) = v1;
                    }
                }
            }
        };
        auto values_ln = [&]() {
            if constexpr (LNC && F16OUT) {
#pragma unroll
                for (int i = 0; i < FI; ++i) {
                    const int row = wm * 128 + i * 16 + l15;
#pragma unroll
                    for (int j = 0; j < FJ; j += 2) {
                        f32x4 v0 = agpr_read(acc[i][j]), v1 = agpr_read(acc[i][j + 1]);
                        v0 = v0 * rs[i][0] + (cs[j] * rs[i][1] + cb[j]);
                        v1 = v1 * rs[i][0] + (cs[j + 1] * rs[i][1] + cb[j + 1]);
                        epi_value_pair<EPI, true, true>(epv, cb[j], cb[j], cb[j + 1], cb[j + 1], v0, v1);
                        const vec4 o0 = Act<T>::from_f32x4(v0), o1 = Act<T>::from_f32x4(v1);
                        const int chunk = wn * 16 + j * 2 + (kb >> 1);
                        const int half = ((kb & 1) ^ ((l15 >> 3) & 1)) * 8;
                        *reinterpret_cast<vec4*>(smem + row * 512 + ((chunk ^ (row & 31)) << 4) + half) = o0;
                        *reinterpret_cast<vec4*>(smem + row * 512 + (((chunk + 2) ^ (row & 31)) << 4) + half) = o1;
                    }
                }
            }
        };
        if (LNC && F16OUT && lnf) values_ln();
        else if (F16OUT && (bias_in_acc || (ep.bias == nullptr && ep.acc_scale == 1.0f))) values(std::true_type{}); else values(std::false_type{});
        __syncthreads();
#pragma unroll 1
        for (int b8 = 0; b8 < 4; ++b8) {
            if constexpr (F16OUT) {
                u32x4 v[8];
#pragma unroll
                for (int u = 0; u < 8; ++u) {
                    const int row = wave * 64 + (b8 * 8 + u) * 2 + hi;
                    v[u] = *reinterpret_cast<const u32x4*>(smem + row * 512 + l31 * 16);
                    if ((u >> 2) & 1) v[u] = u32x4{v[u][2], v[u][3], v[u][0], v[u][1]};
                }
#pragma unroll
                for (int u = 0; u < 8; ++u) {
                    const int row = wave * 64 + (b8 * 8 + u) * 2 + hi;
                    const int chunk = l31 ^ (row & 31);
                    if (m0 + row < M)
                        *reinterpret_cast<u32x4*>(reinterpret_cast<T*>(ep.out) + (long)(m0 + row) * ep.ldo + n0 + chunk * 8) = v[u];
                }
            } else {
                f32x4 v[8], o[8];
#pragma unroll
                for (int u = 0; u < 8; ++u) {
                    const int row = wave * 64 + (b8 * 8 + u) * 2 + hi;
                    const int chunk = l31 ^ (row & 31);
                    const int n = n0 + (chunk >> 4) * 128 + pass * 64 + (chunk & 15) * 4;
                    v[u] = *reinterpret_cast<const f32x4*>(smem + row * 512 + l31 * 16);
                    if constexpr (EPI == AMDS_EPI_RESIDUAL)
                        o[u] = *reinterpret_cast<const f32x4*>(reinterpret_cast<const float*>(ep.out) +
                                                               (long)min(m0 + row, M - 1) * ep.ldo + n);
                }
#pragma unroll
                for (int u = 0; u < 8; ++u) {
                    const int row = wave * 64 + (b8 * 8 + u) * 2 + hi;
                    const int chunk = l31 ^ (row & 31);
                    const int n = n0 + (chunk >> 4) * 128 + pass * 64 + (chunk & 15) * 4;
                    if constexpr (EPI == AMDS_EPI_RESIDUAL) v[u] += o[u];
                    if (m0 + row < M)
                        *reinterpret_cast<f32x4*>(reinterpret_cast<float*>(ep.out) + (long)(m0 + row) * ep.ldo + n) = v[u];
                }
            }
        }
    }
}

static inline int gemm_persist_grid(int tiles) {
    int g = device_cu_count() & ~7;
    const char* e = getenv("AMDS_GEMM_PERSIST_WGS");
    if (e && *e) g = std::min(g, atoi(e) & ~7);
    return std::min(tiles, std::max(g, 8));
}

template <typename T, int EPI, bool SPREAD = true, int P3 = 6, int P0 = 6, int PRL = 0, int PRS = 0, bool STREAM = false, bool PERSIST = false, bool TN = false>
static int launch_gemm_4w16(const void* A, long lda, const void* W, long ldw, int M, int N, int K, const EpiArgs& ep,
                            hipStream_t st) {
    if constexpr (!epi_is_staged<EPI>() && EPI != AMDS_EPI_SWIGLU) {
        return launch_gemm_4w64<T, EPI>(A, lda, W, ldw, M, N, K, ep, st);
    } else {
        constexpr bool STR = STREAM && (EPI == AMDS_EPI_BIAS || EPI == AMDS_EPI_BIAS_GELU || EPI == AMDS_EPI_BIAS_RELU);
        constexpr bool RSTR = STREAM && EPI == AMDS_EPI_RESIDUAL && std::is_same<T, f16>::value && !TN && P3 >= 0 && PRL + PRS == 0;
        constexpr int LDS = 2 * (256 + 256) * 128 + (RSTR ? 8192 : 0);
        if constexpr (RSTR) {
            if (!(ep.xh && ep.xl && ep.rowpart && ep.acc_scale == 1.0f && ep.rowstat == nullptr && ep.nbatch == 1 && ep.ldo * 512 < (1L << 31)))
                return launch_gemm_4w16<T, EPI, SPREAD, P3, P0, PRL, PRS, false, false, TN>(A, lda, W, ldw, M, N, K, ep, st);
        }
        if constexpr (STR) {
            if (ep.ldo * 512 >= (1L << 31)) return launch_gemm_4w16<T, EPI, SPREAD, P3, P0, PRL, PRS, false, false, TN>(A, lda, W, ldw, M, N, K, ep, st);
        }
        constexpr bool PER = PERSIST && (STR || RSTR) && !TN && P3 >= 0 && PRL + PRS == 0;
        if constexpr (PER) {
            if (ep.nbatch != 1) return launch_gemm_4w16<T, EPI, SPREAD, P3, P0, PRL, PRS, STREAM, false, TN>(A, lda, W, ldw, M, N, K, ep, st);
        }
        constexpr auto kern = gemm_4w16_kernel<T, EPI, P3, P0, SPREAD, PRL, PRS, STR || RSTR, PER, TN>;
        EpiArgs epp = ep;
        if constexpr (PRL + PRS > 0) {
            static char* scratch = nullptr;
            static size_t scratch_bytes = 0;
            const size_t need = (size_t)cdiv(M, 256) * (N / 256) * (K / 64) * 4096 * (PRL > PRS ? PRL : PRS);
            if (need > scratch_bytes) {
                if (scratch) AMDS_HIP(hipFree(scratch));
                AMDS_HIP(hipMalloc(reinterpret_cast<void**>(&scratch), need));
                scratch_bytes = need;
            }
            epp.pos = reinterpret_cast<const float*>(scratch);
        }
        AMDS_HIP(lds_opt_in<kern>(LDS));
        const int tiles_m = cdiv(M, 256), tiles_n = N / 256;
        int grid = tiles_m * tiles_n;
        if constexpr (PER) {
            grid = gemm_persist_grid(grid);
            g_gemm_persist_launches.fetch_add(1, std::memory_order_relaxed);
        }
        hipLaunchKernelGGL(kern, dim3(grid, ep.nbatch), dim3(256), LDS, st, reinterpret_cast<const T*>(A), lda,
                           reinterpret_cast<const T*>(W), ldw, M, N, K, epp, tiles_m, tiles_n);
        AMDS_LAUNCH_CHECK("gemm_4w16_kernel");
        return AMDS_OK;
    }
}

}
```

stamp_amd/csrc/gemm_f16.hip:

```cpp
#include "gemm_8p64.h"
#include "gemm_4w64.h"
#include "gemm_4w16.h"
namespace amds {
AMDS_GEMM_DISPATCH_IMPL(f16)
}
```

stamp_amd/csrc/gemm_kernel.h:

```cpp
#pragma once
#include <stdlib.h>
#include <atomic>
#include <type_traits>
#include "launch.h"

namespace amds {

struct EpiArgs {
    void* out;
    long ldo;
    const float* bias;
    const float* scale;
    const float* pos;
    int np, T, P;
    float acc_scale;
    long bsA = 0, bsW = 0, bsOut = 0;
    int nbatch = 1;
    void* xh = nullptr;
    void* xl = nullptr;
    float* rowpart = nullptr;
    const float* rowstat = nullptr;
    const float* colsum = nullptr;
    long ktot = 0;
};
// ... 333 lines not shown
    AMDS_LAUNCH_CHECK("gemm_tn_kernel");
    return AMDS_OK;
}

template <typename T, int EPI>
static int launch_gemm_8p64(const void* A, long lda, const void* W, long ldw, int M, int N, int K, const EpiArgs& ep,
                            hipStream_t st);
template <typename T, int EPI>
static int launch_gemm_4w64(const void* A, long lda, const void* W, long ldw, int M, int N, int K, const EpiArgs& ep,
                            hipStream_t st);
template <typename T, int EPI, bool SPREAD, int P3, int P0, int PRL, int PRS, bool STREAM, bool PERSIST, bool TN>
static int launch_gemm_4w16(const void* A, long lda, const void* W, long ldw, int M, int N, int K, const EpiArgs& ep,
                            hipStream_t st);

static inline bool gemm_epi_stream() {
    const char* e = getenv("AMDS_GEMM_EPI_STREAM");
    return !(e && *e && atoi(e) == 0);
}
static inline bool gemm_resid_stream() {
    const char* e = getenv("AMDS_GEMM_RESID_STREAM");
    return !(e && *e && atoi(e) == 0);
}
static inline bool gemm_resid_persist() {
    const char* e = getenv("AMDS_GEMM_RESID_PERSIST");
    return !(e && *e && atoi(e) == 0);
}
inline std::atomic<long> g_gemm_persist_launches{0};
static inline bool gemm_persist() {
    const char* e = getenv("AMDS_GEMM_PERSIST");
    return !(e && *e && atoi(e) == 0);
}

template <typename T, int EPI>
static int launch_gemm(int cfg, const void* A, long lda, const void* W, long ldw, int M, int N, int K,
                       const EpiArgs& ep, hipStream_t st) {
    if (cfg == 10 && N % 256 == 0 && ep.nbatch == 1) return launch_gemm_4w64<T, EPI>(A, lda, W, ldw, M, N, K, ep, st);
    if (cfg == 10) cfg = 8;
    if ((cfg == 12 || cfg == 13 || cfg == 14 || cfg == 16) && N % 256 == 0) {
        const bool stream = cfg != 14 && (EPI == AMDS_EPI_RESIDUAL ? gemm_resid_stream() : gemm_epi_stream());
        if (cfg == 13) {
            if (stream) return launch_gemm_4w16<T, EPI, true, -2, 0, 0, 0, true, false, false>(A, lda, W, ldw, M, N, K, ep, st);
            return launch_gemm_4w16<T, EPI, true, -2, 0, 0, 0, false, false, false>(A, lda, W, ldw, M, N, K, ep, st);
        }
        if constexpr (EPI == AMDS_EPI_BIAS || EPI == AMDS_EPI_BIAS_GELU || EPI == AMDS_EPI_BIAS_RELU || EPI == AMDS_EPI_RESIDUAL) {
            if (stream && (cfg == 16 || (gemm_persist() && (EPI != AMDS_EPI_RESIDUAL || gemm_resid_persist())))) return launch_gemm_4w16<T, EPI, true, 6, 6, 0, 0, true, true, false>(A, lda, W, ldw, M, N, K, ep, st);
        }
        if (stream) return launch_gemm_4w16<T, EPI, true, 6, 6, 0, 0, true, false, false>(A, lda, W, ldw, M, N, K, ep, st);
        return launch_gemm_4w16<T, EPI, true, 6, 6, 0, 0, false, false, false>(A, lda, W, ldw, M, N, K, ep, st);
    }
#ifdef AMDS_GEMM_PROBE
    if constexpr (EPI == AMDS_EPI_BIAS || EPI == AMDS_EPI_BIAS_GELU || EPI == AMDS_EPI_RESIDUAL) {
        if (cfg == 21 && N % 256 == 0) return launch_gemm_4w16<T, EPI, true, 6, 6, 0, 2, false, false, false>(A, lda, W, ldw, M, N, K, ep, st);
        if (cfg == 22 && N % 256 == 0) return launch_gemm_4w16<T, EPI, true, 6, 6, 1, 1, false, false, false>(A, lda, W, ldw, M, N, K, ep, st);
        if (cfg == 23 && N % 256 == 0) return launch_gemm_4w16<T, EPI, true, 6, 6, 4, 4, false, false, false>(A, lda, W, ldw, M, N, K, ep, st);
    }
#endif
    if constexpr (EPI == AMDS_EPI_BIAS_F32) {
        if (cfg == 15 && N % 256 == 0 && M % 256 == 0) return launch_gemm_4w16<T, EPI, true, 6, 6, 0, 0, false, false, true>(A, lda, W, ldw, M, N, K, ep, st);
    }
    if (cfg == 15) { set_error("amds_gemm: kernel 15 (token-major operands) takes the BIAS_F32 epilogue and M, N multiples of 256"); return AMDS_ERR_INVALID; }
    if (cfg == 12 || cfg == 13 || cfg == 14 || cfg == 16) cfg = 8;

    if (cfg == 8 && N % 256 == 0) return launch_gemm_8p64<T, EPI>(A, lda, W, ldw, M, N, K, ep, st);
    if (cfg == 8) cfg = 0;
    if (cfg == 0 && N % 128 != 0) cfg = 1;
    switch (cfg) {
        case 0: return launch_gemm_cfg<T, 128, 128, 2, 2, EPI>(A, lda, W, ldw, M, N, K, ep, st);
        case 1:
            if constexpr (EPI == AMDS_EPI_SWIGLU || EPI == AMDS_EPI_PATCH) {
                set_error("amds_gemm: the 128x96 tile has no SWIGLU / PATCH epilogue");
                return AMDS_ERR_INVALID;
            } else {
                if (N % 96 != 0) { set_error("amds_gemm: kernel 1 needs N %% 96 == 0 (N=%d)", N); return AMDS_ERR_INVALID; }
                return launch_gemm_cfg<T, 128, 96, 4, 1, EPI>(A, lda, W, ldw, M, N, K, ep, st);
            }
    }
    set_error("amds_gemm: unknown tile config %d", cfg);
    return AMDS_ERR_INVALID;
}

template <typename T>
int gemm_dispatch(int cfg, int epi, const void* A, long lda, const void* W, long ldw, int M, int N, int K,
                  const EpiArgs& ep, hipStream_t st);

#define AMDS_GEMM_DISPATCH_IMPL(T)                                                                        \
    template <>                                                                                           \
    int gemm_dispatch<T>(int cfg, int epi, const void* A, long lda, const void* W, long ldw, int M, int N, \
                         int K, const EpiArgs& ep, hipStream_t st) {                                      \
        switch (epi) {                                                                                    \
            case AMDS_EPI_BIAS: return launch_gemm<T, AMDS_EPI_BIAS>(cfg, A, lda, W, ldw, M, N, K, ep, st); \
            case AMDS_EPI_BIAS_GELU: return launch_gemm<T, AMDS_EPI_BIAS_GELU>(cfg, A, lda, W, ldw, M, N, K, ep, st); \
            case AMDS_EPI_BIAS_RELU: return launch_gemm<T, AMDS_EPI_BIAS_RELU>(cfg, A, lda, W, ldw, M, N, K, ep, st); \
            case AMDS_EPI_RESIDUAL: return launch_gemm<T, AMDS_EPI_RESIDUAL>(cfg, A, lda, W, ldw, M, N, K, ep, st); \
            case AMDS_EPI_BIAS_F32: return launch_gemm<T, AMDS_EPI_BIAS_F32>(cfg, A, lda, W, ldw, M, N, K, ep, st); \
            case AMDS_EPI_SWIGLU: return launch_gemm<T, AMDS_EPI_SWIGLU>(cfg, A, lda, W, ldw, M, N, K, ep, st); \
            case AMDS_EPI_PATCH: return launch_gemm<T, AMDS_EPI_PATCH>(cfg, A, lda, W, ldw, M, N, K, ep, st); \
            case AMDS_EPI_BIAS_GELU_F32: return launch_gemm<T, AMDS_EPI_BIAS_GELU_F32>(cfg, A, lda, W, ldw, M, N, K, ep, st); \
            case AMDS_EPI_BIAS_RELU_F32: return launch_gemm<T, AMDS_EPI_BIAS_RELU_F32>(cfg, A, lda, W, ldw, M, N, K, ep, st); \
        }                                                                                                 \
        set_error("amds_gemm: unknown epilogue %d", epi);                                                 \
        return AMDS_ERR_INVALID;                                                                          \
    }

}
```

stamp_amd/csrc/vit.hip:

```cpp
#include "common.h"

namespace amds {
int prefix_init(const float* prefix, float* x, int B, int T, int P, int dim, hipStream_t st);

struct VitPlan {
    int np, T, kp, dim, hidden;
    size_t off_x, off_h, off_qkv, off_mlp, off_h2, off_lo, off_rowpart, off_rowstat, off_xc, off_hc, off_qc, off_oc, off_uc, off_diag, off_q8, off_q8s, off_q8n, off_q8u, total;
};

static inline size_t align256(size_t v) { return (v + 255) & ~(size_t)255; }

static int make_plan(const amds_vit_cfg* c, int batch, VitPlan* p) {
    AMDS_REQUIRE(c != nullptr, "vit: null cfg");
    AMDS_REQUIRE(c->img > 0 && c->patch > 0 && c->img % c->patch == 0, "vit: img=%d not divisible by patch=%d", c->img, c->patch);
    AMDS_REQUIRE(c->dim % 128 == 0 && c->heads > 0 && (c->heads * 64 == c->dim || c->heads * 80 == c->dim),
                 "vit: dim=%d must be a multiple of 128 and heads*64 or heads*80", c->dim);
    AMDS_REQUIRE(c->hidden % 64 == 0 && c->hidden > 0, "vit: hidden=%d must be a multiple of 64 (zero-pad)", c->hidden);
    AMDS_REQUIRE(c->mlp_kind >= 0 && c->mlp_kind <= 2, "vit: bad mlp_kind");
    AMDS_REQUIRE(c->mlp_kind == 1 || c->hidden % 128 == 0, "vit: GELU hidden=%d must be a multiple of 128", c->hidden);
    AMDS_REQUIRE(c->dtype == AMDS_F16 || c->dtype == AMDS_BF16, "vit: bad act dtype");
    AMDS_REQUIRE(c->depth > 0 && c->n_prefix >= 0 && batch > 0, "vit: bad depth/prefix/batch");
    const int g = c->img / c->patch;
    p->np = g * g;
    p->T = p->np + c->n_prefix;
    AMDS_REQUIRE(p->T <= 288, "vit: %d tokens > 288 unsupported", p->T);
    p->kp = ((3 * c->patch * c->patch + 63) / 64) * 64;
    p->dim = c->dim;
    p->hidden = c->hidden;
    const size_t rows = (size_t)batch * p->T;
    size_t o = 0;
    p->off_x = o;   o += align256(rows * c->dim * 4);
    p->off_h = o;   o += align256(rows * c->dim * 2);
    p->off_qkv = o; o += align256(rows * 3 * c->dim * 2);
    const size_t mlp_b = rows * c->hidden * 2, pm_b = (size_t)batch * p->np * p->kp * 2 * 2;
    p->off_mlp = o; o += align256(mlp_b > pm_b ? mlp_b : pm_b);
    p->off_h2 = o;      o += align256(rows * c->dim * 2);
    p->off_lo = o;      o += align256(rows * c->dim * 2);
    p->off_rowpart = o; o += align256(rows * (size_t)(c->dim / 128) * 2 * 4);
    p->off_rowstat = o; o += align256(rows * 2 * 4);
    const size_t cls = (size_t)batch * c->dim * 4;
    p->off_xc = o; o += align256(cls);
    p->off_hc = o; o += align256(cls);
    p->off_qc = o; o += align256(cls);
    p->off_oc = o; o += align256(cls);
    p->off_uc = o; o += align256((size_t)batch * 2 * c->hidden * 4);
    p->off_diag = o; o += 256;
    p->off_q8 = o;  o += align256(rows * (size_t)(c->hidden > c->dim ? c->hidden : c->dim));
    p->off_q8s = o; o += align256(rows * 4);
    p->off_q8n = o; o += align256(rows * 4);
    p->off_q8u = o; o += align256(rows * 4);
    p->total = o;
    return AMDS_OK;
}

struct VitSide {
    hipStream_t side = nullptr;
    hipEvent_t ev_fork = nullptr, ev_join = nullptr;
};

static int vit_chunk(const amds_vit_cfg* c, const amds_vit_weights* w, const VitPlan& pl, const uint8_t* tiles,
                     void* feats_f16, float* tokens_f32, int Bc, char* ws, hipStream_t st, const VitSide& sd = VitSide()) {
    float* x = reinterpret_cast<float*>(ws + pl.off_x);
    char* h = ws + pl.off_h;
    char* qkv = ws + pl.off_qkv;
    char* mlp = ws + pl.off_mlp;
    char* h2 = ws + pl.off_h2;
    char* lo = ws + pl.off_lo;
    float* rowpart = reinterpret_cast<float*>(ws + pl.off_rowpart);
    float* rowstat = reinterpret_cast<float*>(ws + pl.off_rowstat);
    int* diag = reinterpret_cast<int*>(ws + pl.off_diag);
    const int D = c->dim, T = pl.T, M = Bc * T, dt = c->dtype, Hd = c->hidden, NP = D / 128;
    const int n_fc1 = c->mlp_kind == 1 ? 2 * Hd : Hd;
    int rc;
#define AMDS_TRY(call) do { rc = (call); if (rc != AMDS_OK) return rc; } while (0)
    static const int kcfg = (getenv("AMDS_GEMM_CFG") && *getenv("AMDS_GEMM_CFG")) ? -1 : 12;
    auto enc_gemm = [&](const void* A, long lda, const void* Wt, long ldw, int Mr, int N, int K, int epi, void* out, long ldo, const float* bias,
                        const float* scale, hipStream_t s) {
        return amds_gemm_ex(N % 256 == 0 ? kcfg : -1, A, lda, Wt, ldw, Mr, N, K, dt, epi, out, ldo, bias, scale, nullptr, 0, 0, 0, 1.0f, s);
    };
    const bool fold = w->blocks_host[0].qkv_colsum != nullptr;
    for (int l = 0; l < c->depth; ++l) {
        const amds_vit_block& b = w->blocks_host[l];
        AMDS_REQUIRE((b.qkv_colsum != nullptr) == fold && (b.fc1_colsum != nullptr) == fold, "vit: block %d: qkv_colsum / fc1_colsum must be set in all blocks or in none", l);
    }
    if (fold)
        AMDS_REQUIRE(D % 256 == 0 && n_fc1 % 256 == 0, "vit: the LayerNorm-folded path needs dim %% 256 == 0 and fc1 rows %% 256 == 0 (dim=%d, fc1 rows=%d)", D, n_fc1);
    AMDS_REQUIRE(c->mlp_kind != 2 || (!fold && !w->exact_host && !w->fp8_host), "vit: the quick-GELU MLP (CLIP) runs on the plain packing only (no LayerNorm fold, exact rows or fp8)");
    const amds_vit_exact_block* ex = w->exact_host;
    const int xh_ = w->exact_hidden, xf1 = c->mlp_kind == 1 ? 2 * xh_ : xh_, hd = D / c->heads;
    if (ex) {
        AMDS_REQUIRE(xh_ > 0 && xh_ <= Hd && xh_ % 4 == 0, "vit: exact_hidden=%d must be a multiple of 4 and <= hidden=%d", xh_, Hd);
        for (int l = 0; l < c->depth; ++l)
            AMDS_REQUIRE(ex[l].q_w && ex[l].q_b && ex[l].proj_w && ex[l].proj_b && ex[l].fc1_w && ex[l].fc1_b && ex[l].fc2_w && ex[l].fc2_b &&
                         w->blocks_host[l].ln1_w && w->blocks_host[l].ln1_b && w->blocks_host[l].ln2_w && w->blocks_host[l].ln2_b,
                         "vit: exact block %d: incomplete weights", l);
    }
    const bool tail_env = !(getenv("AMDS_VIT_CLS_TAIL") && atoi(getenv("AMDS_VIT_CLS_TAIL")) == 0);
    const amds_vit_exact_block* tl = (tail_env && tokens_f32 == nullptr && c->mlp_kind != 2) ? (ex ? &ex[c->depth - 1] : w->cls_tail) : nullptr;
    if (tl) {
        AMDS_REQUIRE(xh_ > 0 && xh_ <= Hd && xh_ % 4 == 0, "vit: exact_hidden=%d must be a multiple of 4 and <= hidden=%d", xh_, Hd);
        const amds_vit_block& lb = w->blocks_host[c->depth - 1];
        AMDS_REQUIRE(tl->q_w && tl->q_b && tl->proj_w && tl->proj_b && tl->fc1_w && tl->fc1_b && tl->fc2_w && tl->fc2_b && lb.ln1_w && lb.ln1_b && lb.ln2_w && lb.ln2_b,
                     "vit: cls_tail: incomplete weights");
    }
    const bool planes_env = !(getenv("AMDS_VIT_PLANES") && atoi(getenv("AMDS_VIT_PLANES")) == 0);
    const bool planes = planes_env && fold && !ex && dt == AMDS_F16;
    const amds_vit_fp8_block* f8 = w->fp8_host;
    if (f8) {
        AMDS_REQUIRE(!fold && !ex && dt == AMDS_F16, "vit: the fp8 path needs the plain packing (no LayerNorm fold, no exact rows) and fp16 activations");
        AMDS_REQUIRE(D % 256 == 0 && Hd % 256 == 0, "vit: the fp8 path needs dim %% 256 == 0 and hidden %% 256 == 0");
        for (int l = 0; l < c->depth; ++l)
            AMDS_REQUIRE(f8[l].qkv_w8 && f8[l].qkv_cs && f8[l].proj_w8 && f8[l].proj_cs && f8[l].proj_b && f8[l].fc1_w8 && f8[l].fc1_cs && f8[l].fc2_w8 && f8[l].fc2_cs && f8[l].fc2_b,
                         "vit: fp8 block %d: incomplete weights", l);
    }
    char* q8 = ws + pl.off_q8;
    float* q8s = reinterpret_cast<float*>(ws + pl.off_q8s);
    float* q8n = reinterpret_cast<float*>(ws + pl.off_q8n);
    float* q8u = reinterpret_cast<float*>(ws + pl.off_q8u);
    float* xc = reinterpret_cast<float*>(ws + pl.off_xc);
    float* hc = reinterpret_cast<float*>(ws + pl.off_hc);
    float* qc = reinterpret_cast<float*>(ws + pl.off_qc);
    float* oc = reinterpret_cast<float*>(ws + pl.off_oc);
    float* uc = reinterpret_cast<float*>(ws + pl.off_uc);

    const int kpe = w->patch_lo_shift > 0 ? 2 * pl.kp : pl.kp;
    AMDS_TRY(amds_tile_im2col_u8_ex(tiles, mlp, Bc, c->img, c->patch, pl.kp, dt, w->patch_lo_shift, st));
    if (c->n_prefix > 0) AMDS_TRY(prefix_init(w->prefix, x, Bc, T, c->n_prefix, D, st));
    AMDS_TRY(amds_gemm(mlp, kpe, w->patch_w, kpe, Bc * pl.np, D, kpe, dt, AMDS_EPI_PATCH, x, D, w->patch_b,
                       nullptr, w->pos_patch, pl.np, T, c->n_prefix, 1.0f / 255.0f, st));
    if (w->pre_norm_w) {
        AMDS_REQUIRE(w->pre_norm_b, "vit: pre_norm_b missing");
        AMDS_TRY(amds_layernorm(x, D, w->pre_norm_w, w->pre_norm_b, x, D, Bc * T, D, c->ln_eps, AMDS_F32, st));
    }

    auto block_units = [&](int tiles) {
        const long rt = ((long)tiles * T + 255) / 256;
        auto waves = [&](long tn) { return (rt * tn + 255) / 256; };
        const long kf = Hd / D > 0 ? Hd / D : 1;
        return waves(3 * D / 256) + waves(D / 256) + waves(n_fc1 / 256) + kf * waves(D / 256);
    };
    int n_tail = 0;
    if (sd.side != nullptr && D % 256 == 0 && n_fc1 % 256 == 0 && Bc >= 8) {
        long best = block_units(Bc);
        for (int t = 1; t <= 2; ++t) {
            const long u = block_units(Bc - t);
            if (u < best) { best = u; n_tail = t; }
        }
        if (n_tail > 0) n_tail = Bc / 8 < 4 ? (Bc / 8 > n_tail ? Bc / 8 : n_tail) : 4;
    }
    struct Part { int t0, nt; hipStream_t s; };
    const Part parts[2] = {{0, Bc - n_tail, st}, {Bc - n_tail, n_tail, sd.side}};
    const int nparts = n_tail > 0 ? 2 : 1;
    auto rows16 = [&](char* base, long r0, long pitch_elems) { return base + (size_t)r0 * pitch_elems * 2; };

    auto run_tiles = [&](const Part& q) -> int {
        const long r0 = (long)q.t0 * T;
        const int n = q.nt * T;
        hipStream_t s = q.s;
        float* xq = x + (size_t)r0 * D;
        float* rp = rowpart + (size_t)r0 * NP * 2;
        float* rs = rowstat + 2 * (size_t)r0;
        char *hq = rows16(h, r0, D), *h2q = rows16(h2, r0, D), *loq = rows16(lo, r0, D), *qkvq = rows16(qkv, r0, 3 * D), *mlpq = rows16(mlp, r0, Hd);
        const int epi1 = c->mlp_kind == 0 ? AMDS_EPI_BIAS_GELU : (c->mlp_kind == 1 ? AMDS_EPI_SWIGLU : AMDS_EPI_BIAS);
        float *xcq = xc + (size_t)q.t0 * D, *hcq = hc + (size_t)q.t0 * D, *qcq = qc + (size_t)q.t0 * D, *ocq = oc + (size_t)q.t0 * D;
        float* ucq = uc + (size_t)q.t0 * 2 * Hd;
        auto lin32 = [&](const float* A, int lda, const float* Wt, int K, float* Cm, int ldc, int N, const float* bias, int acc) {
            return bgemm_f32_exact(A, lda, 0, 0, Wt, K, 0, 0, 1, Cm, ldc, 0, 0, 1, 1, q.nt, N, K, 1.0f, 0.0f, bias, acc, s);
        };
        if (ex) AMDS_TRY(amds_vit_cls_gather(xq, xcq, q.nt, T, D, s));
        if (planes) AMDS_TRY(amds_ln_stats_split(xq, D, n, D, c->ln_eps, hq, loq, D, rs, s));
        else if (fold) AMDS_TRY(amds_ln_stats_cast(xq, D, n, D, c->ln_eps, hq, D, rs, dt, s));
        for (int l = 0; l < c->depth; ++l) {
            const amds_vit_block& b = w->blocks_host[l];
            const bool last = l + 1 == c->depth;
            const float* ls1 = c->layerscale ? b.ls1 : nullptr;
            const float* ls2 = c->layerscale ? b.ls2 : nullptr;
            if (last && tl) {
                const size_t wkv = (size_t)D * D;
                if (f8) {
                    char* a8 = q8 + (size_t)r0 * (Hd > D ? Hd : D);
                    float* as = q8s + r0;
                    AMDS_TRY(amds_layernorm_quant_e4m3(xq, D, b.ln1_w, b.ln1_b, c->ln_eps, a8, D, as, nullptr, n, D, s));
                    AMDS_TRY(amds_gemm_fp8(a8, D, (const char*)f8[l].qkv_w8 + wkv, D, n, 2 * D, D, AMDS_EPI_BIAS, qkvq + (size_t)D * 2, 3 * D, b.qkv_b + D,
                                           f8[l].qkv_cs + D, as, s));
                } else if (fold) {
                    AMDS_TRY(amds_gemm_lnfold(hq, D, (const char*)b.qkv_w + wkv * 2, D, n, 2 * D, D, dt, AMDS_EPI_BIAS, qkvq + (size_t)D * 2, 3 * D, b.qkv_b + D,
                                              nullptr, nullptr, nullptr, rs, b.qkv_colsum + D, s));
                } else {
                    AMDS_TRY(amds_layernorm(xq, D, b.ln1_w, b.ln1_b, hq, D, n, D, c->ln_eps, dt, s));
                    AMDS_TRY(amds_gemm_ex((3 * D) % 256 == 0 ? kcfg : -1, hq, D, (const char*)b.qkv_w + wkv * 2, D, n, 2 * D, D, dt, AMDS_EPI_BIAS, qkvq + (size_t)D * 2, 3 * D,
                                          b.qkv_b + D, nullptr, nullptr, 0, 0, 0, 1.0f, s));
                }
                if (planes) AMDS_TRY(amds_planes_to_f32(hq, loq, D, T, xcq, D, q.nt, D, s));
                else if (!ex) AMDS_TRY(amds_vit_cls_gather(xq, xcq, q.nt, T, D, s));
                AMDS_TRY(amds_layernorm(xcq, D, b.ln1_w, b.ln1_b, hcq, D, q.nt, D, c->ln_eps, AMDS_F32, s));
                AMDS_TRY(lin32(hcq, D, tl->q_w, D, qcq, D, D, tl->q_b, 0));
                AMDS_TRY(amds_attention_cls_f32(qcq, D, qkvq, ocq, D, q.nt, T, c->heads, hd, dt, s));
                AMDS_TRY(lin32(ocq, D, tl->proj_w, D, xcq, D, D, tl->proj_b, 1));
                AMDS_TRY(amds_layernorm(xcq, D, b.ln2_w, b.ln2_b, hcq, D, q.nt, D, c->ln_eps, AMDS_F32, s));
                AMDS_TRY(lin32(hcq, D, tl->fc1_w, D, ucq, xf1, xf1, tl->fc1_b, 0));
                AMDS_TRY(amds_mlp_act_f32(ucq, xf1, q.nt, xh_, c->mlp_kind, s));
                AMDS_TRY(lin32(ucq, xf1, tl->fc2_w, xh_, xcq, D, D, tl->fc2_b, 1));
                continue;
            }
            if (f8) {
                char* a8 = q8 + (size_t)r0 * (Hd > D ? Hd : D);
                float* as = q8s + r0;
                float *an = q8n + r0, *au = q8u + r0;
                char* u8 = mlp + (size_t)r0 * Hd;
                AMDS_TRY(amds_layernorm_quant_e4m3(xq, D, b.ln1_w, b.ln1_b, c->ln_eps, a8, D, as, nullptr, n, D, s));
                AMDS_TRY(amds_gemm_fp8(a8, D, f8[l].qkv_w8, D, n, 3 * D, D, AMDS_EPI_BIAS, qkvq, 3 * D, b.qkv_b, f8[l].qkv_cs, as, s));
                AMDS_TRY(amds_attention_vit_hd(qkvq, hq, q.nt, T, c->heads, D / c->heads, dt, s));
                AMDS_TRY(amds_quantize_rows_e4m3(hq, D, a8, D, as, n, D, AMDS_F16, s));
                AMDS_TRY(amds_gemm_fp8(a8, D, f8[l].proj_w8, D, n, D, D, AMDS_EPI_RESIDUAL, xq, D, f8[l].proj_b, f8[l].proj_cs, as, s));
                if (c->mlp_kind == 0) {
                    AMDS_TRY(amds_layernorm_quant_e4m3(xq, D, b.ln2_w, b.ln2_b, c->ln_eps, a8, D, as, an, n, D, s));
                    AMDS_TRY(amds_row_bound_scale(an, f8[l].fc1_wnorm_max, f8[l].fc1_babs_max, au, n, s));
                    AMDS_TRY(amds_gemm_fp8_out8(a8, D, f8[l].fc1_w8, D, n, Hd, D, AMDS_EPI_BIAS_GELU, u8, Hd, au, b.fc1_b, f8[l].fc1_cs, as, s));
                } else {
                    AMDS_TRY(amds_layernorm_quant_e4m3(xq, D, b.ln2_w, b.ln2_b, c->ln_eps, a8, D, as, nullptr, n, D, s));
                    AMDS_TRY(amds_gemm_fp8(a8, D, f8[l].fc1_w8, D, n, 2 * Hd, D, AMDS_EPI_SWIGLU, mlpq, Hd, b.fc1_b, f8[l].fc1_cs, as, s));
                    u8 = a8;
                    AMDS_TRY(amds_quantize_rows_e4m3(mlpq, Hd, u8, Hd, au, n, Hd, AMDS_F16, s));
                }
                AMDS_TRY(amds_gemm_fp8(u8, Hd, f8[l].fc2_w8, Hd, n, D, Hd, AMDS_EPI_RESIDUAL, xq, D, f8[l].fc2_b, f8[l].fc2_cs, au, s));
                continue;
            }
            if (planes) {
                AMDS_TRY(amds_gemm_lnfold(hq, D, b.qkv_w, D, n, 3 * D, D, dt, AMDS_EPI_BIAS, qkvq, 3 * D, b.qkv_b, nullptr, nullptr, nullptr, rs,
                                          b.qkv_colsum, s));
                AMDS_TRY(amds_attention_vit_hd(qkvq, h2q, q.nt, T, c->heads, D / c->heads, dt, s));
                AMDS_TRY(amds_gemm_lnfold_planes(h2q, D, b.proj_w, D, n, D, D, hq, loq, D, b.proj_b, ls1, rp, s));
                AMDS_TRY(amds_ln_rowstat_diag(rp, n, NP, D, c->ln_eps, rs, diag, dt, s));
                AMDS_TRY(amds_gemm_lnfold(hq, D, b.fc1_w, D, n, n_fc1, D, dt, epi1, mlpq, Hd, b.fc1_b, nullptr, nullptr, nullptr, rs, b.fc1_colsum, s));
                AMDS_TRY(amds_gemm_lnfold_planes(mlpq, Hd, b.fc2_w, Hd, n, D, Hd, hq, loq, D, b.fc2_b, ls2, rp, s));
                if (!last) AMDS_TRY(amds_ln_rowstat_diag(rp, n, NP, D, c->ln_eps, rs, diag, dt, s));
                continue;
            }
            if (fold) {
                AMDS_TRY(amds_gemm_lnfold(hq, D, b.qkv_w, D, n, 3 * D, D, dt, AMDS_EPI_BIAS, qkvq, 3 * D, b.qkv_b, nullptr, nullptr, nullptr, rs,
                                          b.qkv_colsum, s));
            } else {
                AMDS_TRY(amds_layernorm(xq, D, b.ln1_w, b.ln1_b, hq, D, n, D, c->ln_eps, dt, s));
                AMDS_TRY(enc_gemm(hq, D, b.qkv_w, D, n, 3 * D, D, AMDS_EPI_BIAS, qkvq, 3 * D, b.qkv_b, nullptr, s));
            }
            AMDS_TRY(amds_attention_vit_hd(qkvq, hq, q.nt, T, c->heads, D / c->heads, dt, s));
            if (ex) {
                AMDS_TRY(amds_layernorm(xcq, D, b.ln1_w, b.ln1_b, hcq, D, q.nt, D, c->ln_eps, AMDS_F32, s));
                AMDS_TRY(lin32(hcq, D, ex[l].q_w, D, qcq, D, D, ex[l].q_b, 0));
                AMDS_TRY(amds_attention_cls_f32(qcq, D, qkvq, ocq, D, q.nt, T, c->heads, hd, dt, s));
                AMDS_TRY(lin32(ocq, D, ex[l].proj_w, D, xcq, D, D, ex[l].proj_b, 1));
            }
            if (fold) {
                AMDS_TRY(amds_gemm_lnfold(hq, D, b.proj_w, D, n, D, D, dt, AMDS_EPI_RESIDUAL, xq, D, b.proj_b, ls1, h2q, rp, nullptr, nullptr, s));
                AMDS_TRY(amds_ln_rowstat_diag(rp, n, NP, D, c->ln_eps, rs, diag, dt, s));
                if (ex) AMDS_TRY(amds_vit_cls_scatter(xcq, xq, h2q, rs, q.nt, T, D, c->ln_eps, dt, s));
                AMDS_TRY(amds_gemm_lnfold(h2q, D, b.fc1_w, D, n, n_fc1, D, dt, epi1, mlpq, Hd, b.fc1_b, nullptr, nullptr, nullptr, rs, b.fc1_colsum, s));
                if (!last) {
                    AMDS_TRY(amds_gemm_lnfold(mlpq, Hd, b.fc2_w, Hd, n, D, Hd, dt, AMDS_EPI_RESIDUAL, xq, D, b.fc2_b, ls2, hq, rp, nullptr, nullptr, s));
                    AMDS_TRY(amds_ln_rowstat_diag(rp, n, NP, D, c->ln_eps, rs, diag, dt, s));
                } else {
                    AMDS_TRY(enc_gemm(mlpq, Hd, b.fc2_w, Hd, n, D, Hd, AMDS_EPI_RESIDUAL, xq, D, b.fc2_b, ls2, s));
                }
            } else {
                AMDS_TRY(enc_gemm(hq, D, b.proj_w, D, n, D, D, AMDS_EPI_RESIDUAL, xq, D, b.proj_b, ls1, s));
                if (ex) AMDS_TRY(amds_vit_cls_scatter(xcq, xq, nullptr, nullptr, q.nt, T, D, c->ln_eps, dt, s));
                AMDS_TRY(amds_layernorm(xq, D, b.ln2_w, b.ln2_b, hq, D, n, D, c->ln_eps, dt, s));
                AMDS_TRY(enc_gemm(hq, D, b.fc1_w, D, n, n_fc1, D, epi1, mlpq, Hd, b.fc1_b, nullptr, s));
                if (c->mlp_kind == 2) AMDS_TRY(amds_quick_gelu_inplace(mlpq, Hd, n, Hd, dt, s));
                AMDS_TRY(enc_gemm(mlpq, Hd, b.fc2_w, Hd, n, D, Hd, AMDS_EPI_RESIDUAL, xq, D, b.fc2_b, ls2, s));
            }
            if (ex) {
                AMDS_TRY(amds_layernorm(xcq, D, b.ln2_w, b.ln2_b, hcq, D, q.nt, D, c->ln_eps, AMDS_F32, s));
                AMDS_TRY(lin32(hcq, D, ex[l].fc1_w, D, ucq, xf1, xf1, ex[l].fc1_b, 0));
                AMDS_TRY(amds_mlp_act_f32(ucq, xf1, q.nt, xh_, c->mlp_kind, s));
                AMDS_TRY(lin32(ucq, xf1, ex[l].fc2_w, xh_, xcq, D, D, ex[l].fc2_b, 1));
                const bool copy16 = fold && !last;
                AMDS_TRY(amds_vit_cls_scatter(xcq, xq, copy16 ? hq : nullptr, copy16 ? rs : nullptr, q.nt, T, D, c->ln_eps, dt, s));
            }
        }
// ... 126 lines not shown
```

stamp_amd/ops.py:

```python
from __future__ import annotations

import ctypes as C

import torch

from . import _lib
from ._lib import BF16, F16, F32

_DT = {torch.float16: F16, torch.bfloat16: BF16, torch.float32: F32}


def _stream() -> int:
    return torch.cuda.current_stream().cuda_stream


def _dev(*ts: torch.Tensor) -> None:
    for t in ts:
        if t is not None and not t.is_cuda:
            raise RuntimeError("stamp_amd ops need tensors on the GPU (no CPU fallback)")


_SCRATCH: dict = {}


# ... 75 lines not shown


def gemm(a: torch.Tensor, w: torch.Tensor, epi: int, *, bias=None, scale=None, out=None, pos=None, np_=0, T=0, P=0,
         acc_scale: float = 1.0, cfg: int = -1, n_out: int | None = None) -> torch.Tensor:
    _dev(a, w, bias, scale, out, pos)
    M, K = a.shape
    N = w.shape[0]
    assert w.shape[1] == K and a.dtype == w.dtype
    dt = act_code(a.dtype)
    f32_out = epi in (_lib.EPI_RESIDUAL, _lib.EPI_BIAS_F32, _lib.EPI_PATCH, _lib.EPI_BIAS_GELU_F32, _lib.EPI_BIAS_RELU_F32)
    if out is None:
        cols = n_out if n_out is not None else (N // 2 if epi == _lib.EPI_SWIGLU else N)
        out = torch.empty(M, cols, dtype=torch.float32 if f32_out else a.dtype, device=a.device)
    ldo = out.stride(-2) if out.dim() >= 2 else out.shape[-1]
    _lib.check(_lib.lib().amds_gemm_ex(cfg, _p(a), a.stride(0), _p(w), w.stride(0), M, N, K, dt, epi, _p(out), ldo,
                                       _p(bias), _p(scale), _p(pos), np_, T, P, acc_scale, _stream()), "gemm")
    return out


def gemm_lnfold(a: torch.Tensor, w: torch.Tensor, epi: int, *, out=None, bias=None, scale=None, xh=None, rowpart=None, rowstat=None,
                colsum=None) -> torch.Tensor:
    _dev(a, w, out, bias, scale, xh, rowpart, rowstat, colsum)
    M, K = a.shape
    N = w.shape[0]
    assert w.shape[1] == K and a.dtype == w.dtype
    if out is None:
        assert epi != _lib.EPI_RESIDUAL
        out = torch.empty(M, N // 2 if epi == _lib.EPI_SWIGLU else N, dtype=a.dtype, device=a.device)
    if xh is not None:
        assert xh.dtype == a.dtype and xh.stride(0) == out.stride(0) and rowpart.shape == (M, N // 128, 2) and rowpart.is_contiguous()
    _lib.check(_lib.lib().amds_gemm_lnfold(_p(a), a.stride(0), _p(w), w.stride(0), M, N, K, act_code(a.dtype), epi, _p(out), out.stride(0),
                                           _p(bias), _p(scale), _p(xh), _p(rowpart), _p(rowstat), _p(colsum), _stream()), "gemm_lnfold")
    return out


def ln_rowstat(rowpart: torch.Tensor, D: int, eps: float) -> torch.Tensor:
    _dev(rowpart)
    assert rowpart.dtype == torch.float32 and rowpart.is_contiguous() and rowpart.dim() == 3 and rowpart.shape[2] == 2
    out = torch.empty(rowpart.shape[0], 2, dtype=torch.float32, device=rowpart.device)
    _lib.check(_lib.lib().amds_ln_rowstat(_p(rowpart), rowpart.shape[0], rowpart.shape[1], D, eps, _p(out), _stream()), "ln_rowstat")
    return out


def ln_stats_cast(x: torch.Tensor, eps: float, dtype: torch.dtype) -> tuple[torch.Tensor, torch.Tensor]:
    _dev(x)
    assert x.dtype == torch.float32 and x.dim() == 2 and x.stride(1) == 1
    M, D = x.shape
    xh = torch.empty(M, D, dtype=dtype, device=x.device)
    rs = torch.empty(M, 2, dtype=torch.float32, device=x.device)
    _lib.check(_lib.lib().amds_ln_stats_cast(_p(x), x.stride(0), M, D, eps, _p(xh), D, _p(rs), act_code(dtype), _stream()), "ln_stats_cast")
    return xh, rs


def ln_stats_split(x: torch.Tensor, eps: float) -> tuple[torch.Tensor, torch.Tensor, torch.Tensor]:
    _dev(x)
    assert x.dtype == torch.float32 and x.dim() == 2 and x.stride(1) == 1
    M, D = x.shape
    hi, lo = torch.empty(M, D, dtype=torch.float16, device=x.device), torch.empty(M, D, dtype=torch.float16, device=x.device)
    rs = torch.empty(M, 2, dtype=torch.float32, device=x.device)
    _lib.check(_lib.lib().amds_ln_stats_split(_p(x), x.stride(0), M, D, eps, _p(hi), _p(lo), D, _p(rs), _stream()), "ln_stats_split")
    return hi, lo, rs


def planes_to_f32(hi: torch.Tensor, lo: torch.Tensor, row_stride: int = 1) -> torch.Tensor:
    _dev(hi, lo)
    assert hi.dtype == lo.dtype == torch.float16 and hi.shape == lo.shape and hi.is_contiguous() and lo.is_contiguous()
    rows = (hi.shape[0] + row_stride - 1) // row_stride
    out = torch.empty(rows, hi.shape[1], dtype=torch.float32, device=hi.device)
    _lib.check(_lib.lib().amds_planes_to_f32(_p(hi), _p(lo), hi.stride(0), row_stride, _p(out), out.stride(0), rows, hi.shape[1], _stream()), "planes_to_f32")
    return out


def gemm_lnfold_planes(a: torch.Tensor, w: torch.Tensor, hi: torch.Tensor, lo: torch.Tensor, *, bias=None, scale=None) -> torch.Tensor:
    _dev(a, w, hi, lo, bias, scale)
    M, K = a.shape
    N = w.shape[0]
    assert a.dtype == w.dtype == hi.dtype == lo.dtype == torch.float16 and hi.shape == lo.shape == (M, N) and hi.stride(0) == lo.stride(0)
    rowpart = torch.empty(M, N // 128, 2, dtype=torch.float32, device=a.device)
    _lib.check(_lib.lib().amds_gemm_lnfold_planes(_p(a), a.stride(0), _p(w), w.stride(0), M, N, K, _p(hi), _p(lo), hi.stride(0), _p(bias), _p(scale),
                                                  _p(rowpart), _stream()), "gemm_lnfold_planes")
    return rowpart


def attention_vit(qkv: torch.Tensor, B: int, T: int, H: int, head_dim: int = 64) -> torch.Tensor:
    _dev(qkv)
    assert qkv.is_contiguous() and qkv.shape == (B * T, 3 * H * head_dim)
    out = torch.empty(B * T, H * head_dim, dtype=qkv.dtype, device=qkv.device)
    _lib.check(_lib.lib().amds_attention_vit_hd(_p(qkv), _p(out), B, T, H, head_dim, act_code(qkv.dtype), _stream()), "attention_vit")
    return out


def attention(qkv: torch.Tensor, B: int, T: int, H: int) -> torch.Tensor:
    _dev(qkv)
    assert qkv.is_contiguous() and qkv.shape == (B * T, 3 * H * 64)
    out = torch.empty(B * T, H * 64, dtype=qkv.dtype, device=qkv.device)
    _lib.check(_lib.lib().amds_attention(_p(qkv), _p(out), B, T, H, act_code(qkv.dtype), _stream()), "attention")
    return out


def set_mil_cls_tail(on: bool, device: int | None = None) -> bool:
    lib = _lib.lib()
    cx = _lib.ctx_of(device)
    prev = bool(lib.amds_get_mil_cls_tail(cx))
    _lib.check(lib.amds_set_mil_cls_tail(cx, 1 if on else 0), "set_mil_cls_tail")
    return prev


def attention_row(q: torch.Tensor, qkv: torch.Tensor, B: int, T: int, H: int) -> torch.Tensor:
    _dev(q, qkv)
    assert qkv.is_contiguous() and qkv.shape == (B * T, 3 * H * 64) and q.shape == (B, H * 64) and q.dtype == qkv.dtype and q.stride(1) == 1
    out = torch.empty(B, H * 64, dtype=qkv.dtype, device=qkv.device)
    _lib.check(_lib.lib().amds_attention_row(_p(q), q.stride(0), _p(qkv), _p(out), H * 64, B, T, H, act_code(qkv.dtype), _stream()), "attention_row")
    return out


def attention_alibi(qkv: torch.Tensor, coords: torch.Tensor, head_scale: torch.Tensor, B: int, T: int, H: int) -> torch.Tensor:
    _dev(qkv, coords, head_scale)
    assert qkv.is_contiguous() and qkv.shape == (B * T, 3 * H * 64)
    assert coords.dtype == torch.float32 and coords.is_contiguous() and coords.shape == (B, T, 2)
    assert head_scale.dtype == torch.float32 and head_scale.numel() == H
    out = torch.empty(B * T, H * 64, dtype=torch.bfloat16, device=qkv.device)
    _lib.check(_lib.lib().amds_attention_alibi(_p(qkv), _p(coords), _p(head_scale), _p(out), B, T, H, act_code(qkv.dtype),
                                               _stream()), "attention_alibi")
    return out


def quantize_rows_e4m3(x: torch.Tensor) -> tuple[torch.Tensor, torch.Tensor]:
    _dev(x)
    assert x.dim() == 2 and x.stride(1) == 1 and x.dtype in (torch.float16, torch.float32)
    rows, cols = x.shape
    q = torch.empty(rows, cols, dtype=torch.uint8, device=x.device)
    sc = torch.empty(rows, dtype=torch.float32, device=x.device)
    _lib.check(_lib.lib().amds_quantize_rows_e4m3(_p(x), x.stride(0), _p(q), cols, _p(sc), rows, cols, _DT[x.dtype], _stream()), "quantize_rows_e4m3")
    return q, sc


def layernorm_quant_e4m3(x: torch.Tensor, gamma: torch.Tensor, beta: torch.Tensor, eps: float, want_norm: bool = False):
    _dev(x, gamma, beta)
    assert x.dtype == torch.float32 and x.dim() == 2 and x.stride(1) == 1
    rows, cols = x.shape
    q = torch.empty(rows, cols, dtype=torch.uint8, device=x.device)
    sc = torch.empty(rows, dtype=torch.float32, device=x.device)
    nrm = torch.empty(rows, dtype=torch.float32, device=x.device) if want_norm else None
    _lib.check(_lib.lib().amds_layernorm_quant_e4m3(_p(x), x.stride(0), _p(gamma), _p(beta), eps, _p(q), cols, _p(sc), _p(nrm), rows, cols, _stream()), "layernorm_quant_e4m3")
    return (q, sc, nrm) if want_norm else (q, sc)


def row_bound_scale(rownorm: torch.Tensor, c0: float, c1: float) -> torch.Tensor:
    _dev(rownorm)
    us = torch.empty_like(rownorm)
    _lib.check(_lib.lib().amds_row_bound_scale(_p(rownorm), float(c0), float(c1), _p(us), rownorm.numel(), _stream()), "row_bound_scale")
    return us


def gemm_fp8_out8(a8: torch.Tensor, w8: torch.Tensor, epi: int, out_rowscale: torch.Tensor, *, rowscale=None, colscale=None, bias=None) -> torch.Tensor:
    _dev(a8, w8, out_rowscale, rowscale, colscale, bias)
    M, K = a8.shape
    N = w8.shape[0]
    out8 = torch.empty(M, N, dtype=torch.uint8, device=a8.device)
    _lib.check(_lib.lib().amds_gemm_fp8_out8(_p(a8), a8.stride(0), _p(w8), w8.stride(0), M, N, K, epi, _p(out8), N, _p(out_rowscale), _p(bias), _p(colscale), _p(rowscale),
                                             _stream()), "gemm_fp8_out8")
    return out8


def gemm_fp8(a8: torch.Tensor, w8: torch.Tensor, epi: int, *, rowscale=None, colscale=None, bias=None, out=None) -> torch.Tensor:
    _dev(a8, w8, rowscale, colscale, bias, out)
    assert a8.dtype == torch.uint8 and w8.dtype == torch.uint8 and a8.stride(1) == 1 and w8.stride(1) == 1
    M, K = a8.shape
    N = w8.shape[0]
    if epi == _lib.EPI_RESIDUAL:
        assert out is not None and out.dtype == torch.float32 and out.shape == (M, N)
    elif out is None:
        out = torch.empty(M, N // 2 if epi == _lib.EPI_SWIGLU else N, dtype=torch.float16, device=a8.device)
    _lib.check(_lib.lib().amds_gemm_fp8(_p(a8), a8.stride(0), _p(w8), w8.stride(0), M, N, K, epi, _p(out), out.stride(0), _p(bias), _p(colscale), _p(rowscale),
                                        _stream()), "gemm_fp8")
    return out


def attention_cls_f32(q: torch.Tensor, qkv: torch.Tensor, B: int, T: int, H: int, head_dim: int = 64) -> torch.Tensor:
    _dev(q, qkv)
    assert q.dtype == torch.float32 and q.is_contiguous() and qkv.is_contiguous() and q.shape == (B, H * head_dim)
    out = torch.empty(B, H * head_dim, dtype=torch.float32, device=q.device)
    _lib.check(_lib.lib().amds_attention_cls_f32(_p(q), H * head_dim, _p(qkv), _p(out), H * head_dim, B, T, H, head_dim, act_code(qkv.dtype), _stream()),
               "attention_cls_f32")
    return out


def vit_cls_gather(x: torch.Tensor, B: int, T: int) -> torch.Tensor:
    _dev(x)
    assert x.dtype == torch.float32 and x.is_contiguous()
    D = x.shape[-1]
    xc = torch.empty(B, D, dtype=torch.float32, device=x.device)
    _lib.check(_lib.lib().amds_vit_cls_gather(_p(x), _p(xc), B, T, D, _stream()), "vit_cls_gather")
    return xc


def vit_cls_scatter(xc: torch.Tensor, x: torch.Tensor, T: int, eps: float, xh: torch.Tensor | None = None, rowstat: torch.Tensor | None = None) -> None:
    _dev(xc, x, xh, rowstat)
    B, D = xc.shape
    code = act_code(xh.dtype) if xh is not None else F16
    _lib.check(_lib.lib().amds_vit_cls_scatter(_p(xc), _p(x), _p(xh), _p(rowstat), B, T, D, eps, code, _stream()), "vit_cls_scatter")


def mlp_act_f32(u: torch.Tensor, hidden: int, kind: int) -> None:
    _dev(u)
    assert u.dtype == torch.float32 and u.is_contiguous() and u.dim() == 2
    _lib.check(_lib.lib().amds_mlp_act_f32(_p(u), u.shape[1], u.shape[0], hidden, kind, _stream()), "mlp_act_f32")


def pack_swiglu_rows(w: torch.Tensor) -> torch.Tensor:
    _dev(w)
    w2 = w.contiguous().float().reshape(w.shape[0], -1)
    H, cols = w2.shape[0] // 2, w2.shape[1]
    dst = torch.empty_like(w2)
    _lib.check(_lib.lib().amds_pack_swiglu_rows(_p(w2), _p(dst), H, cols, _stream()), "pack_swiglu_rows")
    return dst.reshape(w.shape)


def tile_im2col_u8(tiles: torch.Tensor, patch: int, kp: int, dtype: torch.dtype, lo_shift: int = 0) -> torch.Tensor:
    _dev(tiles)
    assert tiles.dtype == torch.uint8 and tiles.is_contiguous() and tiles.shape[-1] == 3
    B, img = tiles.shape[0], tiles.shape[1]
    g = img // patch
    out = torch.empty(B * g * g, kp * (2 if lo_shift else 1), dtype=dtype, device=tiles.device)
    _lib.check(_lib.lib().amds_tile_im2col_u8_ex(_p(tiles), _p(out), B, img, patch, kp, act_code(dtype), int(lo_shift), _stream()), "im2col")
    return out


def tile_normalize_u8(tiles: torch.Tensor, mean, std) -> torch.Tensor:
    _dev(tiles)
    assert tiles.dtype == torch.uint8 and tiles.is_contiguous() and tiles.shape[-1] == 3
    B, H, W, _ = tiles.shape
    out = torch.empty(B, 3, H, W, dtype=torch.float32, device=tiles.device)
    m = (C.c_float * 3)(*[float(v) for v in mean])
    s = (C.c_float * 3)(*[float(v) for v in std])
    _lib.check(_lib.lib().amds_tile_normalize_u8(_p(tiles), _p(out), B, H, W, m, s, _stream()), "tile_normalize")
    return out


_GAP_KEYS = ("fc_w", "fc_b", "a_w", "a_b", "b_w", "b_b", "c_w", "c_b")
_gap_ws: dict = {}


def _gap_workspace(device: torch.device, nbytes: int) -> torch.Tensor:
    key = (device.index, torch.cuda.current_stream(device).cuda_stream)
    ws = _gap_ws.get(key)
    if ws is None or ws.numel() < nbytes:
        ws = _gap_ws[key] = torch.empty(max(nbytes, 1 << 16), dtype=torch.uint8, device=device)
    return ws


_gap_packed: dict = {}


def _gap_weights(weights: dict[str, torch.Tensor], pack: bool = True):
    for k in _GAP_KEYS:
        assert weights[k].dtype == torch.float32 and weights[k].is_contiguous(), k
    gw = _lib.GapWeights(**{k: _p(weights[k]) for k in _GAP_KEYS})
    F, L, D = weights["fc_w"].shape[1], weights["fc_w"].shape[0], weights["a_w"].shape[0]
    n = _lib.lib().amds_gated_attn_packed_floats(F, L, D) if pack else 0
    if n:
        big = [weights[k] for k in ("fc_w", "a_w", "b_w")]
        key = tuple(t.data_ptr() for t in big)
        ver = tuple(t._version for t in big)
        hit = _gap_packed.get(key)
        if hit is None or hit[0] != ver:
            pk = torch.empty(n, dtype=torch.float32, device=big[0].device)
            _lib.check(_lib.lib().amds_gated_attn_pack(C.byref(gw), _p(pk), F, L, D, _stream()), "gated_attn_pack")
            if len(_gap_packed) > 16:
                _gap_packed.clear()
            hit = _gap_packed[key] = (ver, pk, big)
        gw.packed = _p(hit[1])
    return gw


GAP_MODES = {"auto": 0, "slab": 1, "split": 2}

# ... 242 lines not shown
```

Measured before the change: 6426.

## Stream CLS-only last-layer attention from LN-folded planes and fuse patch embed into planes

Adds a CLS-only attention kernel for the last block. It computes the query-key scores by projecting q through Wk (r = q·Wk) and reading the normalized hidden planes directly, which avoids computing the full K/V projection for all tokens in the final layer. Values are recovered as a softmax-weighted sum of the hidden rows multiplied by Wv, using colsum and rowstat corrections for the LayerNorm fold. A second kernel fuses the patch-embedding GEMM epilogue so it writes hi/lo fp16 planes and per-row partial statistics directly, removing the separate f32 write and the stats-split pass. Both paths are on by default behind env switches; the reordered arithmetic may change numerics slightly.

```diff
diff --git a/include/amdstamp.h b/include/amdstamp.h
--- a/include/amdstamp.h
+++ b/include/amdstamp.h
@@ -93,6 +93,8 @@
 
 int amds_gemm_lnfold_planes(const void* A, long lda, const void* W, long ldw, int M, int N, int K, void* hi, void* lo, long ld,
                             const float* bias, const float* scale, float* rowpart, void* stream);
+int amds_gemm_patch_planes(const void* A, long lda, const void* W, long ldw, int M, int N, int K, void* hi, void* lo, long ld,
+                           const float* bias, const float* pos, int np, int T, int P, float acc_scale, float* rowpart, void* stream);
 int amds_ln_stats_split(const float* x, long ldx, int M, int D, float eps, void* hi, void* lo, long ld, float* rowstat, void* stream);
 int amds_planes_to_f32(const void* hi, const void* lo, long ld, long row_stride, float* out, long ldo, long rows, int D, void* stream);
 
@@ -237,6 +239,10 @@
 
 int amds_attention_cls_f32(const float* q, long ldq, const void* qkv, float* out, long ldo, int B, int T, int H, int head_dim,
                            int dtype, void* stream);
+size_t amds_attention_cls_stream_scratch_bytes(int nt, int H, int D);
+int amds_attention_cls_stream(const float* q, long ldq, const void* hi, long ld, const float* rowstat, const void* wk, const void* wv,
+                              const float* colsum_k, const float* colsum_v, const float* bias_v, void* scratch, float* out, long ldo, int nt, int T,
+                              int H, void* stream);
 int amds_vit_cls_gather(const float* x, float* xc, int B, int T, int D, void* stream);
 int amds_vit_cls_scatter(const float* xc, float* x, void* xh, float* rowstat, int B, int T, int D, float eps, int dtype, void* stream);
 int amds_mlp_act_f32(float* u, long ld, int rows, int hidden, int kind, void* stream);
diff --git a/stamp_amd/_lib.py b/stamp_amd/_lib.py
--- a/stamp_amd/_lib.py
+++ b/stamp_amd/_lib.py
@@ -233,6 +233,7 @@
     "amds_export_words": (_i, [_vp, _vp, _l, _i, _vp]),
     "amds_ln_stats_cast": (_i, [_vp, _l, _i, _i, _f, _vp, _l, _vp, _i, _vp]),
     "amds_gemm_lnfold_planes": (_i, [_vp, _l, _vp, _l, _i, _i, _i, _vp, _vp, _l, _vp, _vp, _vp, _vp]),
+    "amds_gemm_patch_planes": (_i, [_vp, _l, _vp, _l, _i, _i, _i, _vp, _vp, _l, _vp, _vp, _i, _i, _i, _f, _vp, _vp]),
     "amds_ln_stats_split": (_i, [_vp, _l, _i, _i, _f, _vp, _vp, _l, _vp, _vp]),
     "amds_planes_to_f32": (_i, [_vp, _vp, _l, _l, _vp, _l, _l, _i, _vp]),
     "amds_gemm_rowstream": (_i, [_vp, _l, _vp, _vp, _f, _vp, _l, _i, _i, _i, _i, _i, _vp, _l, _vp, _vp]),
@@ -269,6 +270,8 @@
     "amds_compact_shift_u8": (_i, [_vp, _vp, _l, _i, _i, _vp, _vp]),
     "amds_compact_rows_u8": (_i, [_vp, _l, _vp, _f, _vp, _i, _vp, _vp, _i, _vp]),
     "amds_attention_cls_f32": (_i, [_vp, _l, _vp, _vp, _l, _i, _i, _i, _i, _i, _vp]),
+    "amds_attention_cls_stream_scratch_bytes": (_sz, [_i, _i, _i]),
+    "amds_attention_cls_stream": (_i, [_vp, _l, _vp, _l, _vp, _vp, _vp, _vp, _vp, _vp, _vp, _vp, _l, _i, _i, _i, _vp]),
     "amds_vit_cls_gather": (_i, [_vp, _vp, _i, _i, _i, _vp]),
     "amds_vit_cls_scatter": (_i, [_vp, _vp, _vp, _vp, _i, _i, _i, _f, _i, _vp]),
     "amds_mlp_act_f32": (_i, [_vp, _l, _i, _i, _i, _vp]),
diff --git a/stamp_amd/csrc/api.hip b/stamp_amd/csrc/api.hip
--- a/stamp_amd/csrc/api.hip
+++ b/stamp_amd/csrc/api.hip
@@ -395,6 +395,25 @@
     return gemm_dispatch<f16>(12, AMDS_EPI_RESIDUAL, A, lda, W, ldw, M, N, K, ep, st);
 }
 
+extern "C" int amds_gemm_patch_planes(const void* A, long lda, const void* W, long ldw, int M, int N, int K, void* hi, void* lo, long ld,
+                                      const float* bias, const float* pos, int np, int T, int P, float acc_scale, float* rowpart, void* stream) {
+    AMDS_REQUIRE(A && W && hi && lo && rowpart && bias && pos, "amds_gemm_patch_planes: null pointer");
+    AMDS_REQUIRE(M >= 0 && N > 0 && K > 0 && K % 64 == 0 && N % 256 == 0, "amds_gemm_patch_planes: needs K %% 64 == 0 and N %% 256 == 0 (M=%d N=%d K=%d)", M, N, K);
+    AMDS_REQUIRE(np > 0 && np % 256 == 0 && M % np == 0 && P >= 0 && T >= np + P, "amds_gemm_patch_planes: needs np %% 256 == 0, M %% np == 0, T >= np + P (M=%d np=%d T=%d P=%d)",
+                 M, np, T, P);
+    AMDS_REQUIRE(lda % 8 == 0 && ldw % 8 == 0 && lda >= K && ldw >= K && ld % 4 == 0 && ld >= N && ld * 1024 < (1L << 31), "amds_gemm_patch_planes: bad pitches");
+    AMDS_REQUIRE(((uintptr_t)A & 15) == 0 && ((uintptr_t)W & 15) == 0 && ((uintptr_t)hi & 15) == 0 && ((uintptr_t)lo & 15) == 0 && ((uintptr_t)pos & 15) == 0 &&
+                 ((uintptr_t)bias & 15) == 0, "amds_gemm_patch_planes: pointers must be 16-byte aligned");
+    AMDS_REQUIRE(hi != lo && A != hi && A != lo, "amds_gemm_patch_planes: the planes must not alias each other or A");
+    if (M == 0) return AMDS_OK;
+    EpiArgs ep;
+    ep.out = hi; ep.ldo = ld; ep.bias = bias; ep.scale = nullptr; ep.pos = pos; ep.np = np; ep.T = T; ep.P = P; ep.acc_scale = acc_scale;
+    ep.xh = hi; ep.xl = lo; ep.rowpart = rowpart;
+    hipStream_t st = (hipStream_t)stream;
+    ProfScope prof(PROF_GEMM, 2.0 * M * (double)N * K, st);
+    return gemm_patch_planes_f16(A, lda, W, ldw, M, N, K, ep, st);
+}
+
 extern "C" long amds_gemm_persist_launches(void) { return g_gemm_persist_launches.load(std::memory_order_relaxed); }
 
 extern "C" int amds_gemm_ex(int cfg, const void* A, long lda, const void* W, long ldw, int M, int N, int K, int dtype,
diff --git a/stamp_amd/csrc/attention_cls_stream.hip b/stamp_amd/csrc/attention_cls_stream.hip
--- /dev/null
+++ b/stamp_amd/csrc/attention_cls_stream.hip
@@ -0,0 +1,261 @@
+#include "common.h"
+#include "launch.h"
+
+namespace amds {
+
+constexpr int CS_TMAX = 288;
+constexpr int CS_CK = 32;
+
+__device__ __forceinline__ f32x4 cs_mfma(float a, float b, f32x4 c) { return __builtin_amdgcn_mfma_f32_16x16x4f32(a, b, c, 0, 0, 0); }
+
+__global__ void __launch_bounds__(256) cls_stream_r_kernel(const float* __restrict__ q, long ldq, const f16* __restrict__ wk, float* __restrict__ r, int nt, int H,
+                                                           int D) {
+    const int t0 = blockIdx.x * 16, h = blockIdx.y;
+    const int wave = threadIdx.x >> 6, lane = threadIdx.x & 63, l15 = lane & 15, g = lane >> 4;
+    const float* qa = q + (long)min(t0 + l15, nt - 1) * ldq + h * 64;
+    for (int sp = wave; sp < D / 128; sp += 4) {
+        const f16* wb = wk + (long)(h * 64) * D + sp * 128 + 8 * l15;
+        f32x4 acc[8];
+#pragma unroll
+        for (int e = 0; e < 8; ++e) acc[e] = f32x4{0.f, 0.f, 0.f, 0.f};
+#pragma unroll 4
+        for (int s = 0; s < 16; ++s) {
+            const int d = 4 * s + g;
+            const float a = qa[d];
+            const f16x8 b = *reinterpret_cast<const f16x8*>(wb + (long)d * D);
+#pragma unroll
+            for (int e = 0; e < 8; ++e) acc[e] = cs_mfma(a, (float)b[e], acc[e]);
+        }
+#pragma unroll
+        for (int rr = 0; rr < 4; ++rr) {
+            const int t = t0 + 4 * g + rr;
+            if (t < nt) {
+                float* dst = r + ((long)t * H + h) * D + sp * 128 + 8 * l15;
+                *reinterpret_cast<f32x4*>(dst) = f32x4{acc[0][rr], acc[1][rr], acc[2][rr], acc[3][rr]};
+                *reinterpret_cast<f32x4*>(dst + 4) = f32x4{acc[4][rr], acc[5][rr], acc[6][rr], acc[7][rr]};
+            }
+        }
+    }
+}
+
+static inline size_t cs_attn_lds_bytes(int D) { return (size_t)CS_CK * (2 * D + 16) + (4 * 16 * 32 + 16 * 33 + 48) * 4; }
+
+__global__ void __launch_bounds__(256) cls_stream_attn_kernel(const float* __restrict__ q, long ldq, const f16* __restrict__ hi, long ld,
+                                                              const float* __restrict__ rowstat, const float* __restrict__ colsum_k,
+                                                              const float* __restrict__ r, float* __restrict__ u, float* __restrict__ tt, int T, int H, int D,
+                                                              float scale) {
+    extern __shared__ __attribute__((aligned(16))) char smem[];
+    const int pitch = 2 * D + 16;
+    char* ck = smem;
+    float* Sp = reinterpret_cast<float*>(smem + CS_CK * pitch);
+    float* Pc = Sp + 4 * 16 * 32;
+    float* al = Pc + 16 * 33;
+    float* cc = al + 16;
+    float* lf = cc + 16;
+    const int tile = blockIdx.x, tid = threadIdx.x;
+    const int wave = tid >> 6, lane = tid & 63, l15 = lane & 15, g = lane >> 4;
+    const f16* hit = hi + (long)tile * T * ld;
+    const float* rst = rowstat + 2 * (long)tile * T;
+    const int rowp = D >> 3, npc = D >> 6;
+    u32x4 pf[16];
+    auto fetch = [&](int k0) {
+#pragma unroll
+        for (int p = 0; p < 16; ++p)
+            if (p < npc) {
+                const int x = p * 256 + tid, row = x / rowp, c16 = x - row * rowp;
+                pf[p] = *reinterpret_cast<const u32x4*>(hit + (long)min(k0 + row, T - 1) * ld + c16 * 8);
+            }
+    };
+    auto stage = [&]() {
+#pragma unroll
+        for (int p = 0; p < 16; ++p)
+            if (p < npc) {
+                const int x = p * 256 + tid, row = x / rowp, c16 = x - row * rowp;
+                *reinterpret_cast<u32x4*>(ck + row * pitch + c16 * 16) = pf[p];
+            }
+    };
+    fetch(0);
+#pragma unroll
+    for (int i4 = 0; i4 < 4; ++i4) {
+        const int i = wave * 4 + i4, ih = min(i, H - 1);
+        const float v = wave_sum(q[(long)tile * ldq + ih * 64 + lane] * colsum_k[ih * 64 + lane]);
+        if (lane == 0) cc[i] = v;
+    }
+    const int nc4 = D >> 7;
+    f32x4 ra0[8], ra1[8];
+    {
+        const float* ra = r + ((long)tile * H + min(l15, H - 1)) * D + 8 * g;
+#pragma unroll
+        for (int c4 = 0; c4 < 8; ++c4) {
+            ra0[c4] = ra1[c4] = f32x4{0.f, 0.f, 0.f, 0.f};
+            if (c4 < nc4) {
+                ra0[c4] = *reinterpret_cast<const f32x4*>(ra + 32 * (wave * nc4 + c4));
+                ra1[c4] = *reinterpret_cast<const f32x4*>(ra + 32 * (wave * nc4 + c4) + 4);
+            }
+        }
+    }
+    const int nsp = D >> 7;
+    f32x4 acc[2][8];
+#pragma unroll
+    for (int s2 = 0; s2 < 2; ++s2)
+#pragma unroll
+        for (int e = 0; e < 8; ++e) acc[s2][e] = f32x4{0.f, 0.f, 0.f, 0.f};
+    float m_run[2] = {-INFINITY, -INFINITY}, l_run[2] = {0.f, 0.f}, t_run[2] = {0.f, 0.f};
+    stage();
+    __syncthreads();
+#pragma unroll 1
+    for (int k0 = 0; k0 < T; k0 += CS_CK) {
+        const bool more = k0 + CS_CK < T;
+        if (more) fetch(k0 + CS_CK);
+        {
+            f32x4 s1[2] = {f32x4{0.f, 0.f, 0.f, 0.f}, f32x4{0.f, 0.f, 0.f, 0.f}};
+#pragma unroll
+            for (int c4 = 0; c4 < 8; ++c4)
+                if (c4 < nc4) {
+                    const int c = wave * nc4 + c4;
+#pragma unroll
+                    for (int kb = 0; kb < 2; ++kb) {
+                        const f16x8 b = *reinterpret_cast<const f16x8*>(ck + (kb * 16 + l15) * pitch + (32 * c + 8 * g) * 2);
+#pragma unroll
+                        for (int e = 0; e < 8; ++e) s1[kb] = cs_mfma(e < 4 ? ra0[c4][e & 3] : ra1[c4][e & 3], (float)b[e], s1[kb]);
+                    }
+                }
+#pragma unroll
+            for (int kb = 0; kb < 2; ++kb)
+#pragma unroll
+                for (int rr = 0; rr < 4; ++rr) Sp[(wave * 16 + 4 * g + rr) * 32 + kb * 16 + l15] = s1[kb][rr];
+        }
+        __syncthreads();
+#pragma unroll
+        for (int st = 0; st < 2; ++st) {
+            const int i = wave * 4 + 2 * st + (lane >> 5), j = lane & 31, key = k0 + j, kc = min(key, T - 1);
+            const float s = ((Sp[i * 32 + j] + Sp[(16 + i) * 32 + j]) + Sp[(32 + i) * 32 + j]) + Sp[(48 + i) * 32 + j];
+            const float rstd = rst[2 * kc], nmr = rst[2 * kc + 1];
+            const float sc = key < T ? scale * (rstd * s + nmr * cc[i]) : -INFINITY;
+            float cm = sc;
+#pragma unroll
+            for (int x = 1; x < 32; x <<= 1) cm = fmaxf(cm, __shfl_xor(cm, x, 64));
+            const float mn = fmaxf(m_run[st], cm);
+            const float alpha = expf(m_run[st] - mn);
+            const float p = key < T ? expf(sc - mn) : 0.f;
+            float ps = p, pt = p * nmr;
+#pragma unroll
+            for (int x = 1; x < 32; x <<= 1) {
+                ps += __shfl_xor(ps, x, 64);
+                pt += __shfl_xor(pt, x, 64);
+            }
+            l_run[st] = l_run[st] * alpha + ps;
+            t_run[st] = t_run[st] * alpha + pt;
+            m_run[st] = mn;
+            Pc[i * 33 + j] = p * rstd;
+            if (j == 0) al[i] = alpha;
+        }
+        __syncthreads();
+        {
+            const f32x4 a4 = f32x4{al[4 * g], al[4 * g + 1], al[4 * g + 2], al[4 * g + 3]};
+#pragma unroll
+            for (int s2 = 0; s2 < 2; ++s2)
+#pragma unroll
+                for (int e = 0; e < 8; ++e) acc[s2][e] *= a4;
+#pragma unroll
+            for (int s = 0; s < CS_CK / 4; ++s) {
+                const float a = Pc[l15 * 33 + 4 * s + g];
+#pragma unroll
+                for (int s2 = 0; s2 < 2; ++s2) {
+                    if (wave + 4 * s2 < nsp) {
+                        const f16x8 b = *reinterpret_cast<const f16x8*>(ck + (4 * s + g) * pitch + ((wave + 4 * s2) * 128 + 8 * l15) * 2);
+#pragma unroll
+                        for (int e = 0; e < 8; ++e) acc[s2][e] = cs_mfma(a, (float)b[e], acc[s2][e]);
+                    }
+                }
+            }
+        }
+        __syncthreads();
+        if (more) {
+            stage();
+            __syncthreads();
+        }
+    }
+#pragma unroll
+    for (int st = 0; st < 2; ++st) {
+        const int i = wave * 4 + 2 * st + (lane >> 5);
+        if ((lane & 31) == 0) {
+            const float inv = 1.0f / l_run[st];
+            lf[i] = inv;
+            if (i < H) tt[(long)tile * H + i] = t_run[st] * inv;
+        }
+    }
+    __syncthreads();
+    const f32x4 inv4 = f32x4{lf[4 * g], lf[4 * g + 1], lf[4 * g + 2], lf[4 * g + 3]};
+#pragma unroll
+    for (int s2 = 0; s2 < 2; ++s2) {
+        if (wave + 4 * s2 < nsp) {
+#pragma unroll
+            for (int rr = 0; rr < 4; ++rr) {
+                const int i = 4 * g + rr;
+                if (i < H) {
+                    float* dst = u + ((long)tile * H + i) * D + (wave + 4 * s2) * 128 + 8 * l15;
+                    *reinterpret_cast<f32x4*>(dst) = f32x4{acc[s2][0][rr], acc[s2][1][rr], acc[s2][2][rr], acc[s2][3][rr]} * inv4[rr];
+                    *reinterpret_cast<f32x4*>(dst + 4) = f32x4{acc[s2][4][rr], acc[s2][5][rr], acc[s2][6][rr], acc[s2][7][rr]} * inv4[rr];
+                }
+            }
+        }
+    }
+}
+
+__global__ void __launch_bounds__(256) cls_stream_o_kernel(const float* __restrict__ u, const float* __restrict__ tt, const f16* __restrict__ wv,
+                                                           const float* __restrict__ colsum_v, const float* __restrict__ bias_v, float* __restrict__ out, long ldo,
+                                                           int nt, int H, int D) {
+    const int t0 = blockIdx.x * 16, h = blockIdx.y;
+    const int wave = threadIdx.x >> 6, lane = threadIdx.x & 63, l15 = lane & 15, g = lane >> 4;
+    const float* ua = u + ((long)min(t0 + l15, nt - 1) * H + h) * D + 8 * g;
+    const f16* wb = wv + (long)(h * 64 + wave * 16 + l15) * D + 8 * g;
+    f32x4 acc = f32x4{0.f, 0.f, 0.f, 0.f};
+#pragma unroll 4
+    for (int c = 0; c < D / 32; ++c) {
+        const f32x4 a0 = *reinterpret_cast<const f32x4*>(ua + 32 * c), a1 = *reinterpret_cast<const f32x4*>(ua + 32 * c + 4);
+        const f16x8 b = *reinterpret_cast<const f16x8*>(wb + 32 * c);
+#pragma unroll
+        for (int e = 0; e < 8; ++e) acc = cs_mfma(e < 4 ? a0[e & 3] : a1[e & 3], (float)b[e], acc);
+    }
+    const int col = h * 64 + wave * 16 + l15;
+    const float cs = colsum_v[col], bv = bias_v[col];
+#pragma unroll
+    for (int rr = 0; rr < 4; ++rr) {
+        const int t = t0 + 4 * g + rr;
+        if (t < nt) out[(long)t * ldo + col] = acc[rr] + (tt[(long)t * H + h] * cs + bv);
+    }
+}
+
+}
+
+using namespace amds;
+
+extern "C" size_t amds_attention_cls_stream_scratch_bytes(int nt, int H, int D) { return (size_t)nt * H * (2 * (size_t)D + 1) * 4; }
+
+extern "C" int amds_attention_cls_stream(const float* q, long ldq, const void* hi, long ld, const float* rowstat, const void* wk, const void* wv,
+                                         const float* colsum_k, const float* colsum_v, const float* bias_v, void* scratch, float* out, long ldo, int nt,
+                                         int T, int H, void* stream) {
+    AMDS_REQUIRE(q && hi && rowstat && wk && wv && colsum_k && colsum_v && bias_v && scratch && out, "amds_attention_cls_stream: null pointer");
+    AMDS_REQUIRE(nt >= 0 && nt <= 65535 * 16 && T > 0 && T <= CS_TMAX && H > 0 && H <= 16 && H % 2 == 0,
+                 "amds_attention_cls_stream: bad nt=%d T=%d heads=%d (T <= %d, heads even and <= 16, head_dim 64)", nt, T, H, CS_TMAX);
+    const int D = H * 64;
+    AMDS_REQUIRE(ldq >= D && ldo >= D && ld >= D && ld % 8 == 0 && ldq % 4 == 0, "amds_attention_cls_stream: bad pitches");
+    AMDS_REQUIRE(((uintptr_t)hi & 15) == 0 && ((uintptr_t)wk & 15) == 0 && ((uintptr_t)wv & 15) == 0 && ((uintptr_t)scratch & 15) == 0 && ((uintptr_t)q & 15) == 0,
+                 "amds_attention_cls_stream: pointers must be 16-byte aligned");
+    if (nt == 0) return AMDS_OK;
+    hipStream_t st = (hipStream_t)stream;
+    float* r = reinterpret_cast<float*>(scratch);
+    float* u = r + (size_t)nt * H * D;
+    float* tt = u + (size_t)nt * H * D;
+    const dim3 gh(cdiv(nt, 16), H);
+    hipLaunchKernelGGL(cls_stream_r_kernel, gh, dim3(256), 0, st, q, ldq, (const f16*)wk, r, nt, H, D);
+    AMDS_LAUNCH_CHECK("cls_stream_r_kernel");
+    const int lds = (int)cs_attn_lds_bytes(1024);
+    AMDS_HIP(lds_opt_in<cls_stream_attn_kernel>(lds));
+    hipLaunchKernelGGL(cls_stream_attn_kernel, dim3(nt), dim3(256), cs_attn_lds_bytes(D), st, q, ldq, (const f16*)hi, ld, rowstat, colsum_k, r, u, tt, T, H, D, 0.125f);
+    AMDS_LAUNCH_CHECK("cls_stream_attn_kernel");
+    hipLaunchKernelGGL(cls_stream_o_kernel, gh, dim3(256), 0, st, u, tt, (const f16*)wv, colsum_v, bias_v, out, ldo, nt, H, D);
+    AMDS_LAUNCH_CHECK("cls_stream_o_kernel");
+    return AMDS_OK;
+}
diff --git a/stamp_amd/csrc/elementwise.hip b/stamp_amd/csrc/elementwise.hip
--- a/stamp_amd/csrc/elementwise.hip
+++ b/stamp_amd/csrc/elementwise.hip
@@ -347,6 +347,39 @@
     const int grid = (int)min((long)2048, (total + 255) / 256);
     hipLaunchKernelGGL(prefix_init_kernel, dim3(grid), dim3(256), 0, st, prefix, x, B, T, P, dim);
     AMDS_LAUNCH_CHECK("prefix_init_kernel");
+    return AMDS_OK;
+}
+
+__global__ void __launch_bounds__(64) prefix_init_planes_kernel(const float* __restrict__ prefix, f16* __restrict__ hi, f16* __restrict__ lo, long ld,
+                                                                float* __restrict__ rowpart, int T, int P, int dim) {
+    const int b = blockIdx.x / P, t = blockIdx.x - b * P, lane = threadIdx.x;
+    const long row = (long)b * T + t;
+    const float* src = prefix + (long)t * dim;
+    const int np = dim >> 7;
+    for (int q = 0; q < np; ++q) {
+        const int c0 = (q >> 1) * 256 + (q & 1) * 64 + lane, c1 = c0 + 128;
+        const float x0 = src[c0], x1 = src[c1];
+        const f16 h0 = (f16)x0, h1 = (f16)x1;
+        hi[row * ld + c0] = h0;
+        hi[row * ld + c1] = h1;
+        lo[row * ld + c0] = (f16)(x0 - (float)h0);
+        lo[row * ld + c1] = (f16)(x1 - (float)h1);
+        float s0 = x0, s1 = x1, q0 = x0 * x0, q1 = x1 * x1;
+#pragma unroll
+        for (int m = 32; m >= 1; m >>= 1) {
+            s0 += __shfl_xor(s0, m);
+            s1 += __shfl_xor(s1, m);
+            q0 += __shfl_xor(q0, m);
+            q1 += __shfl_xor(q1, m);
+        }
+        if (lane == 0) *reinterpret_cast<f32x2*>(rowpart + (row * np + q) * 2) = f32x2{s0 + s1, q0 + q1};
+    }
+}
+
+int prefix_init_planes(const float* prefix, void* hi, void* lo, long ld, float* rowpart, int B, int T, int P, int dim, hipStream_t st) {
+    AMDS_REQUIRE(dim % 256 == 0 && ld >= dim, "prefix_init_planes: dim=%d must be a multiple of 256", dim);
+    hipLaunchKernelGGL(prefix_init_planes_kernel, dim3(B * P), dim3(64), 0, st, prefix, (f16*)hi, (f16*)lo, ld, rowpart, T, P, dim);
+    AMDS_LAUNCH_CHECK("prefix_init_planes_kernel");
     return AMDS_OK;
 }
 
diff --git a/stamp_amd/csrc/gemm_4w16.h b/stamp_amd/csrc/gemm_4w16.h
--- a/stamp_amd/csrc/gemm_4w16.h
+++ b/stamp_amd/csrc/gemm_4w16.h
@@ -66,7 +66,7 @@
     const int l31 = lane & 31, hi = lane >> 5;
 
     static_assert(!PERSIST || (STREAM && !TN && P3 >= 0 && PRL + PRS == 0 &&
-                               (EPI == AMDS_EPI_BIAS || EPI == AMDS_EPI_BIAS_GELU || EPI == AMDS_EPI_BIAS_RELU || EPI == AMDS_EPI_RESIDUAL)),
+                               (EPI == AMDS_EPI_BIAS || EPI == AMDS_EPI_BIAS_GELU || EPI == AMDS_EPI_BIAS_RELU || EPI == AMDS_EPI_RESIDUAL || EPI == AMDS_EPI_PATCH)),
                   "gemm_4w16: the persistent form is a streamed epilogue on SCHED 0");
     int tm, tn;
     auto tile_of = [&](int bid, int nwg, int& tm_, int& tn_) {
@@ -138,7 +138,7 @@
     const int w_off = A_BYTES + (wn * 128 + l15) * ROWB;
 
     const bool lnf = ep.rowstat != nullptr;
-    const bool bias_in_acc = ep.bias != nullptr && ep.acc_scale == 1.0f && !lnf;
+    const bool bias_in_acc = EPI != AMDS_EPI_PATCH && ep.bias != nullptr && ep.acc_scale == 1.0f && !lnf;
     f32x4 acc[FI][FJ];
     {
         f32x4 b0[FJ];
@@ -424,7 +424,8 @@
     __builtin_amdgcn_sched_barrier(0);
 
     constexpr bool F16OUT = (EPI == AMDS_EPI_BIAS || EPI == AMDS_EPI_BIAS_GELU || EPI == AMDS_EPI_BIAS_RELU);
-    static_assert(epi_is_staged<EPI>() || EPI == AMDS_EPI_SWIGLU, "gemm_4w16: staged epilogues and SWIGLU");
+    static_assert(epi_is_staged<EPI>() || EPI == AMDS_EPI_SWIGLU || (EPI == AMDS_EPI_PATCH && STREAM && PERSIST),
+                  "gemm_4w16: staged epilogues, SWIGLU and the PATCH form of the streamed planes producer");
     if constexpr (EPI == AMDS_EPI_SWIGLU) {
         const float as = ep.acc_scale;
 #pragma unroll
@@ -466,18 +467,25 @@
         }
         return;
     }
-    if constexpr (EPI == AMDS_EPI_RESIDUAL && STREAM) {
+    if constexpr ((EPI == AMDS_EPI_RESIDUAL || EPI == AMDS_EPI_PATCH) && STREAM) {
         static_assert(std::is_same<T, f16>::value && !TN && PRL + PRS == 0, "gemm_4w16: the streamed residual epilogue is the fp16 planes producer");
+        constexpr bool PATCHP = EPI == AMDS_EPI_PATCH;
+        static_assert(!PATCHP || PERSIST, "gemm_4w16: the PATCH planes producer has the persistent form only");
         __builtin_amdgcn_sched_barrier(0);
         __builtin_amdgcn_s_waitcnt(0x0F70);
         __builtin_amdgcn_sched_barrier(0);
         const int rows_o = min(BM, M - m0);
         int ldo2 = (int)ep.ldo * 2;
         if constexpr (PERSIST) asm volatile("" : "+s"(ldo2));
-        const __amdgpu_buffer_rsrc_t rsrc_h = __builtin_amdgcn_make_buffer_rsrc(reinterpret_cast<T*>(ep.xh) + (long)m0 * ep.ldo + n0, 0,
+        const int p0 = PATCHP ? m0 % ep.np : 0;
+        const long rowd = PATCHP ? (long)(m0 / ep.np) * ep.T + ep.P + p0 - m0 : 0L;
+        const __amdgpu_buffer_rsrc_t rsrc_h = __builtin_amdgcn_make_buffer_rsrc(reinterpret_cast<T*>(ep.xh) + ((long)m0 + rowd) * ep.ldo + n0, 0,
                                                                                 (int)((((long)rows_o - 1) * ep.ldo + BN) * 2), 0x00020000);
-        const __amdgpu_buffer_rsrc_t rsrc_l = __builtin_amdgcn_make_buffer_rsrc(reinterpret_cast<T*>(ep.xl) + (long)m0 * ep.ldo + n0, 0,
+        const __amdgpu_buffer_rsrc_t rsrc_l = __builtin_amdgcn_make_buffer_rsrc(reinterpret_cast<T*>(ep.xl) + ((long)m0 + rowd) * ep.ldo + n0, 0,
                                                                                 (int)((((long)rows_o - 1) * ep.ldo + BN) * 2), 0x00020000);
+        __amdgpu_buffer_rsrc_t rsrc_p = rsrc_h;
+        if constexpr (PATCHP)
+            rsrc_p = __builtin_amdgcn_make_buffer_rsrc(const_cast<float*>(ep.pos) + (long)p0 * ep.ldo + n0, 0, (int)((((long)rows_o - 1) * ep.ldo + BN) * 4), 0x00020000);
         char* slab = smem + (PERSIST ? ((nk - 1 + par) & 1) * STAGE : 0) + wave * 16384;
         float* part = reinterpret_cast<float*>(smem + 2 * STAGE);
         int wr_base = l15 * 512;
@@ -489,11 +497,12 @@
         const int np_part = N / 128;
         auto run = [&](auto has_scale_c) {
             constexpr bool HS = decltype(has_scale_c)::value;
-            f32x4 sc[HS ? FJ : 1];
-            if constexpr (HS) {
-#pragma unroll
-                for (int j = 0; j < FJ; ++j) sc[j] = *reinterpret_cast<const f32x4*>(ep.scale + n0 + wn * 128 + j * 16 + 4 * kb);
-            }
+            f32x4 sc[HS || PATCHP ? FJ : 1];
+            if constexpr (HS || PATCHP) {
+#pragma unroll
+                for (int j = 0; j < FJ; ++j) sc[j] = *reinterpret_cast<const f32x4*>((PATCHP ? ep.bias : ep.scale) + n0 + wn * 128 + j * 16 + 4 * kb);
+            }
+            const float as = ep.acc_scale;
             f32x4 b0n[PERSIST ? FJ : 1];
             u32x4 prev[3][8];
             auto load_prev = [&](int s) {
@@ -501,9 +510,13 @@
                 asm volatile("" : "+s"(rowoff));
 #pragma unroll
                 for (int u = 0; u < 8; ++u) {
-                    const u32x2 ph = __builtin_bit_cast(u32x2, __builtin_amdgcn_raw_buffer_load_b64(rsrc_h, offp[u] + rowoff, 0, 0));
-                    const u32x2 pl = __builtin_bit_cast(u32x2, __builtin_amdgcn_raw_buffer_load_b64(rsrc_l, offp[u] + rowoff, 0, 0));
-                    prev[s % 3][u] = u32x4{ph[0], ph[1], pl[0], pl[1]};
+                    if constexpr (PATCHP) {
+                        prev[s % 3][u] = __builtin_bit_cast(u32x4, __builtin_amdgcn_raw_buffer_load_b128(rsrc_p, 2 * (offp[u] + rowoff), 0, 0));
+                    } else {
+                        const u32x2 ph = __builtin_bit_cast(u32x2, __builtin_amdgcn_raw_buffer_load_b64(rsrc_h, offp[u] + rowoff, 0, 0));
+                        const u32x2 pl = __builtin_bit_cast(u32x2, __builtin_amdgcn_raw_buffer_load_b64(rsrc_l, offp[u] + rowoff, 0, 0));
+                        prev[s % 3][u] = u32x4{ph[0], ph[1], pl[0], pl[1]};
+                    }
                 }
             };
             load_prev(0);
@@ -516,7 +529,8 @@
 #pragma unroll
                     for (int j = 0; j < FJ; ++j) {
                         f32x4 a = agpr_read(acc[s][j]);
-                        if constexpr (HS) a *= sc[j];
+                        if constexpr (PATCHP) a = a * as + sc[j];
+                        else if constexpr (HS) a *= sc[j];
                         *reinterpret_cast<f32x4*>(wp + (((j * 4 + kb) ^ l15) << 4)) = a;
                     }
                     if (s >= 1 && s + 1 < FI) load_prev(s + 1);
@@ -524,7 +538,7 @@
                         if (s == FI - 1) {
 #pragma unroll
                             for (int j = 0; j < FJ; ++j) b0n[j] = f32x4{0.f, 0.f, 0.f, 0.f};
-                            if (bias_in_acc) {
+                            if (!PATCHP && bias_in_acc) {
 #pragma unroll
                                 for (int j = 0; j < FJ; ++j) b0n[j] = *reinterpret_cast<const f32x4*>(ep.bias + n0n + wn * 128 + j * 16 + 4 * kb);
                             }
@@ -540,7 +554,8 @@
 #pragma unroll
                     for (int u = 0; u < 8; ++u) {
                         const u32x4 o = prev[t % 3][u];
-                        const f32x4 old4 = f32x4{mix_add_hh<0, 0>(o[0], o[2]), mix_add_hh<1, 1>(o[0], o[2]), mix_add_hh<0, 0>(o[1], o[3]), mix_add_hh<1, 1>(o[1], o[3])};
+                        const f32x4 old4 = PATCHP ? __builtin_bit_cast(f32x4, o)
+                                                  : f32x4{mix_add_hh<0, 0>(o[0], o[2]), mix_add_hh<1, 1>(o[0], o[2]), mix_add_hh<0, 0>(o[1], o[3]), mix_add_hh<1, 1>(o[1], o[3])};
                         v[u] += old4;
                         const vec4 c = Act<T>::from_f32x4(v[u]);
                         __builtin_amdgcn_raw_buffer_store_b64(__builtin_bit_cast(u32x2, c), rsrc_h, offp[u] + rowoff, 0, 0);
@@ -573,7 +588,7 @@
                     for (int j = 0; j < FJ; ++j) acc[i][j] = b0n[PERSIST ? j : 0];
             }
         };
-        if (ep.scale) run(std::true_type{}); else run(std::false_type{});
+        if (!PATCHP && ep.scale) run(std::true_type{}); else run(std::false_type{});
         if constexpr (PERSIST) {
 #pragma unroll
             for (int i = 0; i < FI; ++i) {
@@ -594,7 +609,7 @@
             const int idx = e * NT + tid, row = idx >> 1;
             const f32x4 p4 = *reinterpret_cast<const f32x4*>(part + idx * 4);
             if (m0 + row < M)
-                *reinterpret_cast<f32x2*>(ep.rowpart + ((long)(m0 + row) * np_part + tn * 2 + (idx & 1)) * 2) = f32x2{p4[0] + p4[2], p4[1] + p4[3]};
+                *reinterpret_cast<f32x2*>(ep.rowpart + (((long)(m0 + row) + rowd) * np_part + tn * 2 + (idx & 1)) * 2) = f32x2{p4[0] + p4[2], p4[1] + p4[3]};
         }
         if constexpr (PERSIST) {
             AMDS_GEMM_STAMP(3);
@@ -621,6 +636,7 @@
         AMDS_GEMM_TRACE_WRITE();
         return;
     }
+    if constexpr (EPI != AMDS_EPI_PATCH) {
     if constexpr (EPI == AMDS_EPI_RESIDUAL) {
         if (rmw_fast) {
             const int rows_o = min(BM, M - m0);
@@ -983,6 +999,7 @@
             }
         }
     }
+    }
 }
 
 static inline int gemm_persist_grid(int tiles) {
@@ -1039,4 +1056,18 @@
     }
 }
 
+template <typename T>
+static int launch_gemm_patch_planes(const void* A, long lda, const void* W, long ldw, int M, int N, int K, const EpiArgs& ep, hipStream_t st) {
+    constexpr int LDS = 2 * (256 + 256) * 128 + 8192;
+    constexpr auto kern = gemm_4w16_kernel<T, AMDS_EPI_PATCH, 6, 6, true, 0, 0, true, true, false>;
+    AMDS_HIP(lds_opt_in<kern>(LDS));
+    const int tiles_m = M / 256, tiles_n = N / 256;
+    const int grid = gemm_persist_grid(tiles_m * tiles_n);
+    g_gemm_persist_launches.fetch_add(1, std::memory_order_relaxed);
+    hipLaunchKernelGGL(kern, dim3(grid, 1), dim3(256), LDS, st, reinterpret_cast<const T*>(A), lda, reinterpret_cast<const T*>(W), ldw, M, N, K, ep, tiles_m,
+                       tiles_n);
+    AMDS_LAUNCH_CHECK("gemm_4w16_kernel (patch planes)");
+    return AMDS_OK;
 }
+
+}
diff --git a/stamp_amd/csrc/gemm_f16.hip b/stamp_amd/csrc/gemm_f16.hip
--- a/stamp_amd/csrc/gemm_f16.hip
+++ b/stamp_amd/csrc/gemm_f16.hip
@@ -3,4 +3,7 @@
 #include "gemm_4w16.h"
 namespace amds {
 AMDS_GEMM_DISPATCH_IMPL(f16)
+int gemm_patch_planes_f16(const void* A, long lda, const void* W, long ldw, int M, int N, int K, const EpiArgs& ep, hipStream_t st) {
+    return launch_gemm_patch_planes<f16>(A, lda, W, ldw, M, N, K, ep, st);
 }
+}
diff --git a/stamp_amd/csrc/gemm_kernel.h b/stamp_amd/csrc/gemm_kernel.h
--- a/stamp_amd/csrc/gemm_kernel.h
+++ b/stamp_amd/csrc/gemm_kernel.h
@@ -439,6 +439,7 @@
 template <typename T>
 int gemm_dispatch(int cfg, int epi, const void* A, long lda, const void* W, long ldw, int M, int N, int K,
                   const EpiArgs& ep, hipStream_t st);
+int gemm_patch_planes_f16(const void* A, long lda, const void* W, long ldw, int M, int N, int K, const EpiArgs& ep, hipStream_t st);
 
 #define AMDS_GEMM_DISPATCH_IMPL(T)                                                                        \
     template <>                                                                                           \
diff --git a/stamp_amd/csrc/vit.hip b/stamp_amd/csrc/vit.hip
--- a/stamp_amd/csrc/vit.hip
+++ b/stamp_amd/csrc/vit.hip
@@ -2,6 +2,7 @@
 
 namespace amds {
 int prefix_init(const float* prefix, float* x, int B, int T, int P, int dim, hipStream_t st);
+int prefix_init_planes(const float* prefix, void* hi, void* lo, long ld, float* rowpart, int B, int T, int P, int dim, hipStream_t st);
 
 struct VitPlan {
     int np, T, kp, dim, hidden;
@@ -105,6 +106,8 @@
     }
     const bool planes_env = !(getenv("AMDS_VIT_PLANES") && atoi(getenv("AMDS_VIT_PLANES")) == 0);
     const bool planes = planes_env && fold && !ex && dt == AMDS_F16;
+    const bool tail_kv_env = !(getenv("AMDS_VIT_TAIL_KV") && atoi(getenv("AMDS_VIT_TAIL_KV")) == 0);
+    const bool tail_kv = planes && tl != nullptr && tail_kv_env && hd == 64 && c->heads <= 16 && c->heads % 2 == 0 && !w->fp8_host;
     const amds_vit_fp8_block* f8 = w->fp8_host;
     if (f8) {
         AMDS_REQUIRE(!fold && !ex && dt == AMDS_F16, "vit: the fp8 path needs the plain packing (no LayerNorm fold, no exact rows) and fp16 activations");
@@ -125,9 +128,17 @@
 
     const int kpe = w->patch_lo_shift > 0 ? 2 * pl.kp : pl.kp;
     AMDS_TRY(amds_tile_im2col_u8_ex(tiles, mlp, Bc, c->img, c->patch, pl.kp, dt, w->patch_lo_shift, st));
-    if (c->n_prefix > 0) AMDS_TRY(prefix_init(w->prefix, x, Bc, T, c->n_prefix, D, st));
-    AMDS_TRY(amds_gemm(mlp, kpe, w->patch_w, kpe, Bc * pl.np, D, kpe, dt, AMDS_EPI_PATCH, x, D, w->patch_b,
-                       nullptr, w->pos_patch, pl.np, T, c->n_prefix, 1.0f / 255.0f, st));
+    const bool patch_planes_env = !(getenv("AMDS_VIT_PATCH_PLANES") && atoi(getenv("AMDS_VIT_PATCH_PLANES")) == 0);
+    const bool patch_planes = planes && patch_planes_env && pl.np % 256 == 0 && D % 256 == 0 && !w->pre_norm_w;
+    if (patch_planes) {
+        if (c->n_prefix > 0) AMDS_TRY(prefix_init_planes(w->prefix, h, lo, D, rowpart, Bc, T, c->n_prefix, D, st));
+        AMDS_TRY(amds_gemm_patch_planes(mlp, kpe, w->patch_w, kpe, Bc * pl.np, D, kpe, h, lo, D, w->patch_b, w->pos_patch, pl.np, T, c->n_prefix,
+                                        1.0f / 255.0f, rowpart, st));
+    } else {
+        if (c->n_prefix > 0) AMDS_TRY(prefix_init(w->prefix, x, Bc, T, c->n_prefix, D, st));
+        AMDS_TRY(amds_gemm(mlp, kpe, w->patch_w, kpe, Bc * pl.np, D, kpe, dt, AMDS_EPI_PATCH, x, D, w->patch_b,
+                           nullptr, w->pos_patch, pl.np, T, c->n_prefix, 1.0f / 255.0f, st));
+    }
     if (w->pre_norm_w) {
         AMDS_REQUIRE(w->pre_norm_b, "vit: pre_norm_b missing");
         AMDS_TRY(amds_layernorm(x, D, w->pre_norm_w, w->pre_norm_b, x, D, Bc * T, D, c->ln_eps, AMDS_F32, st));
@@ -168,7 +179,8 @@
             return bgemm_f32_exact(A, lda, 0, 0, Wt, K, 0, 0, 1, Cm, ldc, 0, 0, 1, 1, q.nt, N, K, 1.0f, 0.0f, bias, acc, s);
         };
         if (ex) AMDS_TRY(amds_vit_cls_gather(xq, xcq, q.nt, T, D, s));
-        if (planes) AMDS_TRY(amds_ln_stats_split(xq, D, n, D, c->ln_eps, hq, loq, D, rs, s));
+        if (patch_planes) AMDS_TRY(amds_ln_rowstat_diag(rp, n, NP, D, c->ln_eps, rs, diag, dt, s));
+        else if (planes) AMDS_TRY(amds_ln_stats_split(xq, D, n, D, c->ln_eps, hq, loq, D, rs, s));
         else if (fold) AMDS_TRY(amds_ln_stats_cast(xq, D, n, D, c->ln_eps, hq, D, rs, dt, s));
         for (int l = 0; l < c->depth; ++l) {
             const amds_vit_block& b = w->blocks_host[l];
@@ -177,7 +189,8 @@
             const float* ls2 = c->layerscale ? b.ls2 : nullptr;
             if (last && tl) {
                 const size_t wkv = (size_t)D * D;
-                if (f8) {
+                if (tail_kv) {
+                } else if (f8) {
                     char* a8 = q8 + (size_t)r0 * (Hd > D ? Hd : D);
                     float* as = q8s + r0;
                     AMDS_TRY(amds_layernorm_quant_e4m3(xq, D, b.ln1_w, b.ln1_b, c->ln_eps, a8, D, as, nullptr, n, D, s));
@@ -195,7 +208,10 @@
                 else if (!ex) AMDS_TRY(amds_vit_cls_gather(xq, xcq, q.nt, T, D, s));
                 AMDS_TRY(amds_layernorm(xcq, D, b.ln1_w, b.ln1_b, hcq, D, q.nt, D, c->ln_eps, AMDS_F32, s));
                 AMDS_TRY(lin32(hcq, D, tl->q_w, D, qcq, D, D, tl->q_b, 0));
-                AMDS_TRY(amds_attention_cls_f32(qcq, D, qkvq, ocq, D, q.nt, T, c->heads, hd, dt, s));
+                if (tail_kv)
+                    AMDS_TRY(amds_attention_cls_stream(qcq, D, hq, D, rs, (const char*)b.qkv_w + wkv * 2, (const char*)b.qkv_w + 2 * wkv * 2, b.qkv_colsum + D,
+                                                       b.qkv_colsum + 2 * D, b.qkv_b + 2 * D, qkvq, ocq, D, q.nt, T, c->heads, s));
+                else AMDS_TRY(amds_attention_cls_f32(qcq, D, qkvq, ocq, D, q.nt, T, c->heads, hd, dt, s));
                 AMDS_TRY(lin32(ocq, D, tl->proj_w, D, xcq, D, D, tl->proj_b, 1));
                 AMDS_TRY(amds_layernorm(xcq, D, b.ln2_w, b.ln2_b, hcq, D, q.nt, D, c->ln_eps, AMDS_F32, s));
                 AMDS_TRY(lin32(hcq, D, tl->fc1_w, D, ucq, xf1, xf1, tl->fc1_b, 0));
diff --git a/stamp_amd/ops.py b/stamp_amd/ops.py
--- a/stamp_amd/ops.py
+++ b/stamp_amd/ops.py
@@ -181,6 +181,18 @@
     return rowpart
 
 
+def gemm_patch_planes(a: torch.Tensor, w: torch.Tensor, hi: torch.Tensor, lo: torch.Tensor, rowpart: torch.Tensor, *, bias: torch.Tensor,
+                      pos: torch.Tensor, tokens: int, n_prefix: int, acc_scale: float = 1.0 / 255.0) -> None:
+    _dev(a, w, hi, lo, rowpart, bias, pos)
+    M, K = a.shape
+    N, n_patches = w.shape[0], pos.shape[0]
+    assert a.dtype == w.dtype == hi.dtype == lo.dtype == torch.float16 and rowpart.dtype == bias.dtype == pos.dtype == torch.float32
+    assert hi.shape == lo.shape and hi.shape[1] == N and hi.stride(0) == lo.stride(0) == pos.stride(0) and pos.shape[1] == N and M % n_patches == 0
+    assert hi.shape[0] >= (M // n_patches) * tokens and rowpart.is_contiguous() and rowpart.shape == (hi.shape[0], N // 128, 2)
+    _lib.check(_lib.lib().amds_gemm_patch_planes(_p(a), a.stride(0), _p(w), w.stride(0), M, N, K, _p(hi), _p(lo), hi.stride(0), _p(bias), _p(pos), n_patches,
+                                                 tokens, n_prefix, acc_scale, _p(rowpart), _stream()), "gemm_patch_planes")
+
+
 def attention_vit(qkv: torch.Tensor, B: int, T: int, H: int, head_dim: int = 64) -> torch.Tensor:
     _dev(qkv)
     assert qkv.is_contiguous() and qkv.shape == (B * T, 3 * H * head_dim)
@@ -292,6 +304,19 @@
     xc = torch.empty(B, D, dtype=torch.float32, device=x.device)
     _lib.check(_lib.lib().amds_vit_cls_gather(_p(x), _p(xc), B, T, D, _stream()), "vit_cls_gather")
     return xc
+
+
+def attention_cls_stream(q: torch.Tensor, hi: torch.Tensor, rowstat: torch.Tensor, wk: torch.Tensor, wv: torch.Tensor, colsum_k: torch.Tensor,
+                         colsum_v: torch.Tensor, bias_v: torch.Tensor, T: int, H: int) -> torch.Tensor:
+    _dev(q, hi, rowstat, wk, wv, colsum_k, colsum_v, bias_v)
+    nt, D = q.shape
+    assert D == 64 * H and hi.shape == (nt * T, D) and hi.dtype == wk.dtype == wv.dtype == torch.float16 and wk.shape == wv.shape == (D, D)
+    assert all(t.is_contiguous() for t in (q, hi, rowstat, wk, wv, colsum_k, colsum_v, bias_v)) and rowstat.shape == (nt * T, 2)
+    ws = torch.empty(_lib.lib().amds_attention_cls_stream_scratch_bytes(nt, H, D), dtype=torch.uint8, device=q.device)
+    out = torch.empty(nt, D, dtype=torch.float32, device=q.device)
+    _lib.check(_lib.lib().amds_attention_cls_stream(_p(q), D, _p(hi), D, _p(rowstat), _p(wk), _p(wv), _p(colsum_k), _p(colsum_v), _p(bias_v), _p(ws), _p(out),
+                                                    D, nt, T, H, _stream()), "attention_cls_stream")
+    return out
 
 
 def vit_cls_scatter(xc: torch.Tensor, x: torch.Tensor, T: int, eps: float, xh: torch.Tensor | None = None, rowstat: torch.Tensor | None = None) -> None:
```

Result: no change. 6477, median of 6 (+0.8%).
